# fhgyuanshen/HybridGL

Hardware: AMD Instinct MI355X
Metric: images/sec (whole node) (higher is better)
Workload: dtype f32 via fp16x3 split MFMA (fp32 accumulate)

## Files before the change

### hybridgl_amd/_lib.py

```python
import ctypes as C
import os

_HERE = os.path.dirname(os.path.abspath(__file__))
LIB_PATH = os.path.join(_HERE, "libhybridgl.so")

c_float_p = C.POINTER(C.c_float)
c_u8_p = C.POINTER(C.c_uint8)
c_i32_p = C.POINTER(C.c_int32)
c_i64_p = C.POINTER(C.c_int64)


class HybridGLError(RuntimeError):
    pass


class HglSentence(C.Structure):
    _fields_ = [("sentence_row", C.c_int), ("noun_phrase_row", C.c_int), ("other_row0", C.c_int), ("n_other", C.c_int),
                ("dirflag", C.c_int), ("relaword", C.c_int), ("has_other_nouns", C.c_int), ("black", C.c_float),
                ("imgattn", C.c_void_p), ("target", C.c_void_p)]


class HglGroupRef(C.Structure):
    _fields_ = [("hybrid", C.c_void_p), ("text", C.c_void_p), ("T", C.c_int), ("boxes", C.c_void_p), ("masks", C.c_void_p),
                ("N", C.c_int), ("H", C.c_int), ("W", C.c_int), ("sentences", C.POINTER(HglSentence)), ("S", C.c_int),
# ... 104 lines not shown
    "hgl_clip_text_workspace_bytes": (_SZ, [C.POINTER(HglClipTextW), _I]),
    "hgl_clip_encode_text": (_I, [C.POINTER(HglClipTextW), _VP, _I, _VP, _VP, _SZ, _VP]),
    "hgl_clip_encode_text_prefix": (_I, [C.POINTER(HglClipTextW), _VP, _I, _I, _VP, _VP, _SZ, _VP]),
    "hgl_clip_encode_text_ex": (_I, [C.POINTER(HglClipTextW), _VP, _I, _I, _VP, _VP, _I, _I, _VP, _VP, _SZ, _VP]),
    "hgl_gem_workspace_bytes": (_SZ, [C.POINTER(HglClipVisionW)]),
    "hgl_gem_image_features": (_I, [C.POINTER(HglClipVisionW), _VP, _I, _I, _F, _VP, _VP, _VP, _SZ, _VP]),
    "hgl_gem_batch_workspace_bytes": (_SZ, [C.POINTER(HglClipVisionW), _I]),
    "hgl_gem_image_features_batch": (_I, [C.POINTER(HglClipVisionW), _VP, _I, _I, _I, _F, _VP, _VP, _VP, _SZ, _VP]),
    "hgl_gem_heatmap_workspace_bytes": (_SZ, [_I, _I, _I]),
    "hgl_gem_heatmap": (_I, [_VP, _I, _I, _VP, _I, _I, _I, _VP, _VP, _SZ, _VP]),
    "hgl_resize_bilinear_aa": (_I, [_VP, _I, _I, _I, _VP, _I, _I, _VP]),
    "hgl_resize_bilinear": (_I, [_VP, _I, _I, _I, _VP, _I, _I, _VP]),
    "hgl_mask_resize": (_I, [_VP, _I, _I, _I, _I, _VP, _VP]),
    "hgl_calculate_score": (_I, [_VP, _VP, _I, _I, _I, _F, _VP, _VP]),
    "hgl_coherence_workspace_bytes": (_SZ, [_I, _I, _I]),
    "hgl_coherence_scores": (_I, [_VP, _VP, _I, _I, _I, _I, _F, _VP, _VP, _SZ, _VP]),
    "hgl_iou": (_I, [_VP, _VP, _LL, _VP, _VP]),
    "hgl_iou_select": (_I, [_VP, _VP, _I, _VP, _LL, _VP, _VP]),
    "hgl_score_sentence_workspace_bytes": (_SZ, [_I, _I]),
    "hgl_score_sentence": (_I, [_VP, _VP, _VP, _VP, _I, _F, _VP, _VP, _I, _I, _F, _I, _I, _F, _I, _I,
                                _VP, _VP, _VP, _VP, _SZ, _VP]),
    "hgl_synthesize_views": (_I, [_VP, _VP, _VP, _VP, _I, _I, _I, _I, _VP, _VP, _VP]),
    "hgl_resize_pil_bilinear_workspace_bytes": (_SZ, [_I, _I, _I]),
    "hgl_resize_pil_bilinear": (_I, [_VP, _I, _I, _I, _I, _I, _VP, _VP, _I, _VP, _VP, _I, _VP, _VP, _SZ, _VP]),
    "hgl_sam_encode_workspace_bytes": (_SZ, [C.POINTER(HglSamEncoderW)]),
    "hgl_sam_encode": (_I, [C.POINTER(HglSamEncoderW), _VP, _I, _I, _VP, _VP, _SZ, _VP]),
    "hgl_sam_encode_batch_workspace_bytes": (_SZ, [C.POINTER(HglSamEncoderW), _I]),
    "hgl_sam_encode_batch": (_I, [C.POINTER(HglSamEncoderW), C.POINTER(C.c_void_p), C.POINTER(C.c_int), C.POINTER(C.c_int), _I,
                                  _VP, _VP, _SZ, _VP]),
    "hgl_sam_dense_pe": (_I, [C.POINTER(HglSamDecoderW), _VP, _VP, _VP]),
    "hgl_sam_decode_workspace_bytes": (_SZ, [C.POINTER(HglSamDecoderW), _I]),
    "hgl_sam_decode_points": (_I, [C.POINTER(HglSamDecoderW), _VP, _VP, _I, _VP, _VP, _VP, _SZ, _VP]),
    "hgl_sam_decode_points_gated": (_I, [C.POINTER(HglSamDecoderW), _VP, _VP, _I, C.c_float, _VP, _VP, _VP, _SZ, _VP]),
    "hgl_sam_decode_prompts": (_I, [C.POINTER(HglSamDecoderW), _VP, _VP, _VP, _I, _VP, _I, _I, _VP, _VP, _VP, _SZ, _VP]),
    "hgl_sam_embed_masks": (_I, [C.POINTER(HglSamDecoderW), _VP, _I, _VP, _VP]),
    "hgl_sam_decoder_fusion": (_I, [_I]),
    "hgl_attention_presplit": (_I, [_I]),
    "hgl_attention_presplit_f32": (_I, [_VP, _I, _I, _I, _I, _I, _VP, _I, C.c_float, _I, _VP, _I, _I, _VP, C.c_size_t, _VP]),
    "hgl_sam_postprocess_workspace_bytes": (_SZ, [_I]),
    "hgl_sam_postprocess": (_I, [_VP, _VP, _I, _I, _I, _I, _I, _I, _I, _I, _F, _F, _F, _F, _VP, _VP, _VP, _VP, _VP,
                                 _VP, _SZ, _VP]),
    "hgl_nms": (_I, [_VP, _VP, _VP, _I, _F, _VP, _VP, _VP]),
    "hgl_nms_large_workspace_bytes": (_SZ, [_I]),
    "hgl_nms_large": (_I, [_VP, _VP, _VP, _I, _F, _VP, _VP, _VP, _SZ, _VP]),
    "hgl_box_near_crop_edge": (_I, [_VP, _I, C.POINTER(C.c_int32), C.POINTER(C.c_int32), _F, _VP, _VP]),
    "hgl_remove_small_regions_workspace_bytes": (_SZ, [_I, _I, _I]),
    "hgl_remove_small_regions": (_I, [_VP, _I, _I, _I, _I, _I, _VP, _VP, _VP, _SZ, _VP]),
    "hgl_remove_small_regions_boxes": (_I, [_VP, _I, _I, _I, _I, _I, _VP, _VP, _VP, _VP, _SZ, _VP]),
    "hgl_mask_boxes": (_I, [_VP, _I, _I, _I, _VP, _VP]),
    "hgl_gather_masks": (_I, [_VP, _VP, _VP, _I, _LL, _VP, _VP]),
    "hgl_gen_dir_mask": (_I, [_I, _I, _I, _VP, _VP]),
    "hgl_relation_boxes": (_I, [_VP, _VP, _VP, _VP, _I, _I, _VP, _VP]),
    "hgl_gaussian_blur_u8_workspace_bytes": (_SZ, [_I, _I, _I]),
    "hgl_gaussian_blur_u8": (_I, [_VP, _I, _I, _I, C.POINTER(C.c_double), _I, _VP, _VP, _SZ, _VP]),
    "hgl_cv_gaussian_kernel_q8": (_I, [_I, C.c_double, C.POINTER(C.c_uint16)]),
    "hgl_gaussian_blur_u8_q8": (_I, [_VP, _I, _I, _I, C.POINTER(C.c_uint16), C.POINTER(C.c_uint16), _I, _VP, _VP, _SZ, _VP]),
    "hgl_score_ref_workspace_bytes": (_SZ, [_I, _I, _I, _I, _I]),
    "hgl_score_ref": (_I, [_VP, _VP, _I, _VP, _VP, _I, _I, _I, _I, C.POINTER(HglSentence), _I, C.c_float, C.c_float, _I, _I, C.c_float,
                           _VP, _VP, _VP, _VP, _VP, _VP, _VP, _SZ, _VP]),
    "hgl_score_group_workspace_bytes": (_SZ, [C.POINTER(HglGroupRef), _I, _I]),
    "hgl_score_group": (_I, [C.POINTER(HglGroupRef), _I, _I, C.c_float, C.c_float, C.c_float, _VP, _VP, _SZ, _VP]),
    "hgl_u8_to_chw_lut": (_I, [_VP, _I, _I, _I, _VP, _VP, _VP]),
    "hgl_gt_mask_from_polygons": (_I, [_VP, _VP, _I, _I, _I, _VP, _VP]),
    "hgl_gt_mask_from_rle_counts": (_I, [_VP, _I, _I, _I, _VP, _VP]),
    "hgl_gt_mask_from_rle_string": (_I, [C.c_char_p, _I, _I, _VP, _VP]),
    "hgl_rle_encode_mask": (_I, [_VP, _I, _I, _VP, _LL, C.POINTER(C.c_longlong)]),
    "hgl_rle_to_string": (_I, [_VP, _LL, C.c_char_p, _SZ, C.POINTER(C.c_size_t)]),
}

_lib = None
ABI_VERSION = 7


def load():

# ... 26 lines not shown
```

### hybridgl_amd/csrc/attention.hip

```cpp
#include "hgl_common.h"
#include <stdlib.h>

typedef float f32x2 __attribute__((ext_vector_type(2)));

namespace {

constexpr int KV_CHUNK = 64;
constexpr int NEG_BIG_BITS = 0xff800000;

struct AttnArgs {
  const float *q, *k, *v;
  float* out;
  int B, H, Sq, Sk;
  int ldq, ldk, ldv, ldo;
  long long sqb, skb, svb, sob;
  float scale;
  int mask_kind;
  const uint8_t* keep;
  int keep_b0, keep_n;
  const float *rel_h, *rel_w;
  int kh, kw;
  const float *tab_h, *tab_w;
  const _Float16 *tabh_hi = nullptr, *tabh_lo = nullptr, *tabw_hi = nullptr, *tabw_lo = nullptr;
  _Float16 *out_hi, *out_lo;
// ... 1270 lines not shown
        for (int e = 0; e < 4; ++e) o[c][e] += sc[j] * vv[e];
      }
    }
  }
  const long long oo = b * a.sob + (long long)qi * a.ldo + hh * HD;
#pragma unroll
  for (int c = 0; c < 4; ++c) {
    f32x4 r;
#pragma unroll
    for (int e = 0; e < 4; ++e) r[e] = o[c][e] * inv;
    if (a.out) {
      *(f32x4*)(a.out + oo + 4 * c) = r;
    } else {
      h16x4 hi, lo;
#pragma unroll
      for (int e = 0; e < 4; ++e) {
        _Float16 a2, c2;
        hgl_split_hi_lo(r[e], a2, c2);
        hi[e] = a2;
        lo[e] = c2;
      }
      *(h16x4*)(a.out_hi + oo + 4 * c) = hi;
      if (a.out_lo) *(h16x4*)(a.out_lo + oo + 4 * c) = lo;
    }
  }
}

struct FewQArgs {
  const float *q, *k, *v;
  float* out;
  int B, H, Sq, Sk, ldq, ldk, ldv, ldo;
  long long sqb, skb, svb, sob;
  float scale;
};

constexpr int FEWQ_MAX = 8;

__global__ __launch_bounds__(256) void attn_fewq_kernel(FewQArgs a) {
  constexpr int HD = 16;
  __shared__ __attribute__((aligned(16))) float q_s[FEWQ_MAX * HD];
  __shared__ float part[4][FEWQ_MAX][HD + 2];
  int bh;
  {
    const int bid = blockIdx.x, n = gridDim.x;
    const int per = a.H * 8;
    const int full = (n / per) * per;
    if (bid < full) {
      const int grp = bid / per, r = bid - grp * per;
      const int xcd = r & 7, j = r >> 3;
      bh = (grp * 8 + xcd) * a.H + j;
    } else {
      bh = bid;
    }
  }
  const int b = bh / a.H, hh = bh - b * a.H;
  const int t = threadIdx.x, lane = t & 63, wave = t >> 6;
  if (t < a.Sq * HD) q_s[t] = a.q[b * a.sqb + (long long)(t / HD) * a.ldq + hh * HD + (t % HD)] * a.scale;
  else if (t < FEWQ_MAX * HD) q_s[t] = 0.f;
  __syncthreads();
  float m[FEWQ_MAX], l[FEWQ_MAX];
  f32x4 o[FEWQ_MAX][4];
#pragma unroll
  for (int qi = 0; qi < FEWQ_MAX; ++qi) {
    m[qi] = -3.0e38f; l[qi] = 0.f;
#pragma unroll
    for (int c = 0; c < 4; ++c) o[qi][c] = f32x4{0.f, 0.f, 0.f, 0.f};
// ... 64 lines not shown
      const float sc = expf(part[w2][qi][HD] - mm);
      ll += part[w2][qi][HD + 1] * sc;
      oo += part[w2][qi][d] * sc;
    }
    a.out[b * a.sob + (long long)qi * a.ldo + hh * HD + d] = oo / ll;
  }
}

constexpr int FQC_KEYS = 256;
constexpr int FQC_QS = 7 * 16 + 4;
constexpr int FQC_PART = 10;

__global__ __launch_bounds__(256, 4) void attn_fewq_chunk_kernel(FewQArgs a, float* __restrict__ part) {
  constexpr int NQ = 7;
  __shared__ __attribute__((aligned(16))) float q_s[8 * FQC_QS];
  __shared__ __attribute__((aligned(16))) float mrg[4][16][NQ][FQC_PART + 2];
  const int b = blockIdx.y, chunk = blockIdx.x, nchunk = gridDim.x;
  const int t = threadIdx.x, lane = t & 63, wave = t >> 6;
  const int l16 = t & 15, c2 = t & 1, hh = (t >> 1) & 7, ks = t >> 4;
  constexpr float LOG2E = 1.4426950408889634f;
  for (int i = t; i < 8 * NQ * 16; i += 256) {
    const int head = i / (NQ * 16), rem = i - head * (NQ * 16), qi = rem >> 4, d = rem & 15;
    q_s[head * FQC_QS + rem] = qi < a.Sq ? a.q[b * a.sqb + (long long)qi * a.ldq + head * 16 + d] * (a.scale * LOG2E) : 0.f;
  }
  __syncthreads();
  float m[NQ], l[NQ];
  f32x4 o[NQ][2];
#pragma unroll
  for (int qi = 0; qi < NQ; ++qi) {
    m[qi] = -3.0e38f; l[qi] = 0.f;
    o[qi][0] = f32x4{0.f, 0.f, 0.f, 0.f};
    o[qi][1] = f32x4{0.f, 0.f, 0.f, 0.f};
  }
  const float* kp = a.k + b * a.skb + hh * 16 + c2 * 8;
  const float* vp = a.v + b * a.svb + hh * 16 + c2 * 8;
  const float* qs = q_s + hh * FQC_QS + c2 * 8;
  const int k0 = chunk * FQC_KEYS + ks;
  f32x4 kn[2], vn[2];
  {
    const int key = k0 < a.Sk ? k0 : a.Sk - 1;
    kn[0] = *(const f32x4*)(kp + (long long)key * a.ldk); kn[1] = *(const f32x4*)(kp + (long long)key * a.ldk + 4);
    vn[0] = *(const f32x4*)(vp + (long long)key * a.ldv); vn[1] = *(const f32x4*)(vp + (long long)key * a.ldv + 4);
  }
#pragma unroll 2
  for (int pass = 0; pass < FQC_KEYS / 16; ++pass) {
    const int key = k0 + 16 * pass;
    const f32x4 kk0 = kn[0], kk1 = kn[1], vv0 = vn[0], vv1 = vn[1];
    {
      const int nk = key + 16 < a.Sk ? key + 16 : a.Sk - 1;
      kn[0] = *(const f32x4*)(kp + (long long)nk * a.ldk); kn[1] = *(const f32x4*)(kp + (long long)nk * a.ldk + 4);
      vn[0] = *(const f32x4*)(vp + (long long)nk * a.ldv); vn[1] = *(const f32x4*)(vp + (long long)nk * a.ldv + 4);
    }
    if (key < a.Sk) {
#pragma unroll
      for (int qi = 0; qi < NQ; ++qi) {
        const f32x4 q0 = *(const f32x4*)(qs + qi * 16), q1 = *(const f32x4*)(qs + qi * 16 + 4);
        float s = q0[0] * kk0[0];
        s = fmaf(q0[1], kk0[1], s); s = fmaf(q0[2], kk0[2], s); s = fmaf(q0[3], kk0[3], s);
        s = fmaf(q1[0], kk1[0], s); s = fmaf(q1[1], kk1[1], s); s = fmaf(q1[2], kk1[2], s); s = fmaf(q1[3], kk1[3], s);
        s += __shfl_xor(s, 1);
        const float mn = fmaxf(m[qi], s);
        const float al = __builtin_amdgcn_exp2f(m[qi] - mn), p = __builtin_amdgcn_exp2f(s - mn);
        l[qi] = fmaf(l[qi], al, p);
#pragma unroll
        for (int e = 0; e < 4; ++e) {
          o[qi][0][e] = fmaf(o[qi][0][e], al, p * vv0[e]);
          o[qi][1][e] = fmaf(o[qi][1][e], al, p * vv1[e]);
        }
// ... 148 lines not shown
  a.out_hi = (_Float16*)out_hi; a.out_lo = hgl_split_terms() == 1 ? nullptr : (_Float16*)out_lo;
  HglProfScope prof(HGL_PROF_ATTN, 4.0 * B * H * 196.0 * 196.0 * 80, 0.0, st);
  if (hgl_split_terms() == 1) hipLaunchKernelGGL((attn_x3_kernel<80, 14, 8, 1>), dim3(1, (unsigned)(B * H)), dim3(512), 0, st, a);
  else hipLaunchKernelGGL((attn_x3_kernel<80, 14, 8>), dim3(1, (unsigned)(B * H)), dim3(512), 0, st, a);
  return hgl_check_launch("attention_win14");
}

int hgl_launch_attention_smallk(const float* q, const float* k, const float* v, float* out, void* out_hi, void* out_lo,
                                int B, int H, int Sq, int Sk, int hd, int ldq, int ldk, int ldv, int ldo, long long sqb,
                                long long skb, long long svb, long long sob, float scale, hipStream_t st) {
  HGL_REQUIRE(q && k && v && (out || (out_hi && out_lo)), "attention_smallk: null operand");
  HGL_REQUIRE(hd == 16 && Sk >= 1 && Sk <= SMALLK_MAX && H >= 1 && 256 % H == 0, "attention_smallk: unsupported shape (hd %d, Sk %d, H %d)", hd, Sk, H);
  HGL_REQUIRE(((ldq | ldk | ldv | ldo) & 3) == 0 && ((sqb | skb | svb | sob) & 3) == 0, "attention_smallk: strides must be multiples of 4");
  HGL_REQUIRE(B <= 65535, "attention_smallk: B too large");
  SmallKArgs a;
  a.q = q; a.k = k; a.v = v; a.out = out; a.out_hi = (_Float16*)out_hi;
  a.out_lo = hgl_split_terms() == 1 ? nullptr : (_Float16*)out_lo;
  a.B = B; a.H = H; a.Sq = Sq; a.Sk = Sk; a.ldq = ldq; a.ldk = ldk; a.ldv = ldv; a.ldo = ldo;
  a.sqb = sqb; a.skb = skb; a.svb = svb; a.sob = sob; a.scale = scale;
  const int qpb = 256 / H;
  HglProfScope prof(HGL_PROF_ATTN, 4.0 * B * (double)H * Sq * Sk * hd, 0.0, st);
  hipLaunchKernelGGL(attn_smallk_kernel, dim3((unsigned)((Sq + qpb - 1) / qpb), (unsigned)B), dim3(256),
                     (size_t)2 * Sk * H * 16 * sizeof(float), st, a);
  return hgl_check_launch("attention_smallk");
}

int hgl_launch_attention_fewq(const float* q, const float* k, const float* v, float* out, int B, int H, int Sq, int Sk,
                              int hd, int ldq, int ldk, int ldv, int ldo, long long sqb, long long skb, long long svb,
                              long long sob, float scale, hipStream_t st) {
  HGL_REQUIRE(q && k && v && out, "attention_fewq: null operand");
  HGL_REQUIRE(hd == 16 && Sq >= 1 && Sq <= FEWQ_MAX, "attention_fewq: unsupported shape (hd %d, Sq %d)", hd, Sq);
  HGL_REQUIRE(((ldk | ldv) & 3) == 0 && ((skb | svb) & 3) == 0, "attention_fewq: K/V strides must be multiples of 4");
  FewQArgs a;
  a.q = q; a.k = k; a.v = v; a.out = out; a.B = B; a.H = H; a.Sq = Sq; a.Sk = Sk;
  a.ldq = ldq; a.ldk = ldk; a.ldv = ldv; a.ldo = ldo; a.sqb = sqb; a.skb = skb; a.svb = svb; a.sob = sob; a.scale = scale;
  HglProfScope prof(HGL_PROF_ATTN, 4.0 * B * (double)H * Sq * Sk * hd, 0.0, st);
  hipLaunchKernelGGL(attn_fewq_kernel, dim3((unsigned)(B * H)), dim3(256), 0, st, a);
  return hgl_check_launch("attention_fewq");
}

size_t hgl_attention_fewq_part_bytes(int B, int Sk) {
  return (size_t)B * ((Sk + FQC_KEYS - 1) / FQC_KEYS) * 16 * 7 * FQC_PART * sizeof(float);
}

int hgl_launch_attention_fewq_chunked(const float* q, const float* k, const float* v, float* out, int B, int H, int Sq, int Sk,
                                      int hd, int ldq, int ldk, int ldv, int ldo, long long sqb, long long skb, long long svb,
                                      long long sob, float scale, float* part, size_t part_bytes, hipStream_t st) {
  HGL_REQUIRE(q && k && v && out && part, "attention_fewq_chunked: null operand");
  HGL_REQUIRE(hd == 16 && H == 8 && Sq >= 1 && Sq <= 7 && Sk >= 1 && B >= 1 && B <= 65535,
              "attention_fewq_chunked: unsupported shape (hd %d, H %d, Sq %d)", hd, H, Sq);
  HGL_REQUIRE(((ldk | ldv) & 3) == 0 && ((skb | svb) & 3) == 0 && (((uintptr_t)k | (uintptr_t)v) & 15) == 0,
              "attention_fewq_chunked: K/V strides must be multiples of 4");
  HGL_REQUIRE(part_bytes >= hgl_attention_fewq_part_bytes(B, Sk), "attention_fewq_chunked: partial buffer too small");
  FewQArgs a;
  a.q = q; a.k = k; a.v = v; a.out = out; a.B = B; a.H = H; a.Sq = Sq; a.Sk = Sk;
  a.ldq = ldq; a.ldk = ldk; a.ldv = ldv; a.ldo = ldo; a.sqb = sqb; a.skb = skb; a.svb = svb; a.sob = sob; a.scale = scale;
  const int nchunk = (Sk + FQC_KEYS - 1) / FQC_KEYS;
  HglProfScope prof(HGL_PROF_ATTN, 4.0 * B * (double)H * Sq * Sk * hd, 0.0, st);
  hipLaunchKernelGGL(attn_fewq_chunk_kernel, dim3((unsigned)nchunk, (unsigned)B), dim3(256), 0, st, a, part);
  hipLaunchKernelGGL(attn_fewq_combine_kernel, dim3(7, (unsigned)B), dim3(128), 0, st, (const float*)part, nchunk, Sq, out, ldo, sob);
  return hgl_check_launch("attention_fewq_chunked");
}

int hgl_launch_attention(const float* q, const float* k, const float* v, float* out, int B, int H,
                         int Sq, int Sk, int hd, int ldq, int ldk, int ldv, int ldo, long long sqb,
                         long long skb, long long svb, long long sob, float scale, int mask_kind,
                         const uint8_t* keep, int keep_b0, int keep_n, const float* rel_h,
                         const float* rel_w, int kh, int kw, hipStream_t st) {
  return hgl_launch_attention_split(q, k, v, out, nullptr, nullptr, B, H, Sq, Sk, hd, ldq, ldk, ldv, ldo, sqb, skb, svb, sob,
                                    scale, mask_kind, keep, keep_b0, keep_n, rel_h, rel_w, kh, kw, st);
}

int hgl_launch_attention_split(const float* q, const float* k, const float* v, float* out, void* out_hi, void* out_lo, int B,
                               int H, int Sq, int Sk, int hd, int ldq, int ldk, int ldv, int ldo, long long sqb,
                               long long skb, long long svb, long long sob, float scale, int mask_kind,
                               const uint8_t* keep, int keep_b0, int keep_n, const float* rel_h,
                               const float* rel_w, int kh, int kw, hipStream_t st) {
  HGL_REQUIRE(q && k && v && (out || (out_hi && out_lo)), "attention: null operand");
  HGL_REQUIRE(out || hgl_split_layout(), "attention: split output exists in the split-fp16 modes only");
  HGL_REQUIRE(B > 0 && H > 0 && Sq > 0 && Sk > 0, "attention: bad shape");
  HGL_REQUIRE((ldq & 3) == 0 && (ldk & 3) == 0 && (ldv & 3) == 0 && (ldo & 3) == 0, "attention: leading dims must be multiples of 4");
  HGL_REQUIRE((((uintptr_t)q | (uintptr_t)k | (uintptr_t)v | (uintptr_t)out | (uintptr_t)out_hi | (uintptr_t)out_lo) & 15) == 0,
              "attention: operands must be 16-byte aligned");
  HGL_REQUIRE(((sqb | skb | svb | sob) & 3) == 0, "attention: batch strides must be multiples of 4");
  HGL_REQUIRE(mask_kind >= 0 && mask_kind <= 2, "attention: bad mask kind %d", mask_kind);
  HGL_REQUIRE(mask_kind != HGL_MASK_CLS_KEEP || keep, "attention: HGL_MASK_CLS_KEEP needs keep bytes");
  HGL_REQUIRE((rel_h == nullptr) == (rel_w == nullptr), "attention: rel_h and rel_w go together");
// ... 30 lines not shown
```

### hybridgl_amd/csrc/hgl_common.h

```cpp
#pragma once
#include <hip/hip_runtime.h>
#include <stdint.h>
#include <stddef.h>
#include <atomic>
#include "../../include/hybridgl.h"

typedef float f32x16 __attribute__((ext_vector_type(16)));
typedef float f32x4 __attribute__((ext_vector_type(4)));

#ifdef __HIPCC__
static __device__ __attribute__((unused)) unsigned int hgl_tu_split_overflow;
__device__ __forceinline__ void hgl_split_hi_lo(float x, _Float16& hi, _Float16& lo) {
  asm volatile("" : "+v"(x));
  hi = (_Float16)x;
  lo = (_Float16)(x - (float)hi);
}
__device__ __forceinline__ void hgl_split_hi_lo(float x, _Float16& hi, _Float16& lo, float& amax) {
  asm volatile("" : "+v"(x));
  amax = fmaxf(amax, fabsf(x));
  hi = (_Float16)x;
  lo = (_Float16)(x - (float)hi);
}
__device__ __forceinline__ void hgl_split_commit(float amax) {
  if (__builtin_expect(amax > 65504.0f, 0)) atomicAdd(&hgl_tu_split_overflow, 1u);
// ... 92 lines not shown
    if (dry) return nullptr;
    return (T*)(base + o);
  }
  bool ok() const { return dry || off <= cap; }
};

int hgl_launch_gemm(const float* A, const float* W, const float* bias, const float* R, float* C,
                    int M, int N, int K, int lda, int ldw, int ldr, int ldc, int batch,
                    long long sA, long long sW, long long sR, long long sC, int act,
                    hipStream_t st);
int hgl_launch_layernorm(const float* x, const float* w, const float* b, float* y, int rows, int D,
                         float eps, hipStream_t st);
int hgl_launch_attention_split(const float* q, const float* k, const float* v, float* out, void* out_hi, void* out_lo, int B,
                               int H, int Sq, int Sk, int hd, int ldq, int ldk, int ldv, int ldo, long long sqb,
                               long long skb, long long svb, long long sob, float scale, int mask_kind,
                               const uint8_t* keep, int keep_b0, int keep_n, const float* rel_h,
                               const float* rel_w, int kh, int kw, hipStream_t st);
int hgl_launch_attention_win14(const float* q, const float* k, const float* v, void* out_hi, void* out_lo, int B, int H, int hd,
                               int ldq, int ldk, int ldv, int ldo, long long sqb, long long skb, long long svb, long long sob,
                               float scale, const float* Rh, const float* Rw, hipStream_t st);
bool hgl_attention_ps_enabled();
int hgl_attention_ps_serves(long long plane_delta, int ld, int B, int H, int S, int hd, int mask_kind, int rel_kh, int rel_kw,
                            const float* tab_h, const float* tab_w);
int hgl_launch_attention_ps(const void* qkv_hi, const void* qkv_lo, int ld, int qcol, int kcol, int vcol, long long sb, int B,
                            int H, int S, int hd, float* out, void* out_hi, void* out_lo, int ldo, long long sob, float scale,
                            int mask_kind, const uint8_t* keep, int keep_b0, int keep_n, const float* rel_h, const float* rel_w,
                            int kh, int kw, const float* tab_h, const float* tab_w, hipStream_t st);
int hgl_launch_attention_smallk(const float* q, const float* k, const float* v, float* out, void* out_hi, void* out_lo,
                                int B, int H, int Sq, int Sk, int hd, int ldq, int ldk, int ldv, int ldo, long long sqb,
                                long long skb, long long svb, long long sob, float scale, hipStream_t st);
size_t hgl_attention_fewq_part_bytes(int B, int Sk);
int hgl_launch_attention_fewq_chunked(const float* q, const float* k, const float* v, float* out, int B, int H, int Sq, int Sk,
                                      int hd, int ldq, int ldk, int ldv, int ldo, long long sqb, long long skb, long long svb,
                                      long long sob, float scale, float* part, size_t part_bytes, hipStream_t st);
int hgl_launch_attention(const float* q, const float* k, const float* v, float* out, int B, int H,
                         int Sq, int Sk, int hd, int ldq, int ldk, int ldv, int ldo, long long sqb,
                         long long skb, long long svb, long long sob, float scale, int mask_kind,
                         const uint8_t* keep, int keep_b0, int keep_n, const float* rel_h,
                         const float* rel_w, int kh, int kw, hipStream_t st);

int hgl_launch_im2col_patch(const float* img, int N, int res, int patch, float* cols, hipStream_t st);
int hgl_launch_im2col_patch_split(const float* img, int N, int res, int patch, void* hi, void* lo, hipStream_t st);
int hgl_launch_assemble_lnpre(const float* tok, const float* cls, const float* pos, const float* lw,
                              const float* lb, float* x, int B, int S, int D, hipStream_t st);
int hgl_launch_mask_resize(const uint8_t* masks, int N, int Hm, int Wm, int g, float* pm,
                           uint8_t* keep, hipStream_t st);
int hgl_launch_mix(float* out, const float* a, float ca, const float* b, float cb, const float* pm,
                   int N, int S, int D, hipStream_t st);
int hgl_launch_gather_rows(const float* x, long long row_stride, int rows, int D, float* y,
                           hipStream_t st);
int hgl_launch_add_inplace(float* y, const float* x, long long n, hipStream_t st);
int hgl_launch_text_embed(const int32_t* tokens, const float* emb, const float* pos, float* x, int B,
                          int S, int ctx, int D, int vocab, int32_t* eot, hipStream_t st);
int hgl_launch_gather_eot(const float* x, const int32_t* eot, int B, int S, int D, float* y,
                          hipStream_t st);
int hgl_launch_zero_positions(float* x, int B, int S, int D, const int32_t* pos, int n, hipStream_t st);

struct HglBlockBufs {
  float* H;
  float* QKV;
  float* F;
};
int hgl_clip_run_block(const HglResBlockW& w, float* X, int B, int S, int D, int heads, const HglBlockBufs& bf,
                       int mask_kind, const uint8_t* keep, int keep_b0, int keep_n, hipStream_t st);
bool hgl_clip_block_uses_x3(const HglResBlockW& w, int M, int D);
bool hgl_clip_block_presplit(const HglResBlockW& w, int B, int S, int D, int heads, int mask_kind);
int hgl_clip_block_qkv(const HglResBlockW& w, const float* X, int M, int D, const HglBlockBufs& bf, hipStream_t st,
// ... 29 lines not shown
                            float* tokens, hipStream_t st);
int hgl_launch_mask_downscaling(const float* in, int P, int g, const float* c1w, const float* c1b, const float* n1w, const float* n1b,
                                const float* c2w, const float* c2b, const float* n2w, const float* n2b, const float* c3w,
                                const float* c3b, float* out, hipStream_t st);
int hgl_launch_win_maps(int g, int ws, int nw, int nb, int* pad_of, int* tok_of, int* pad_list, int* pad_count, hipStream_t st);
int hgl_launch_fill_rows(float* dst, int ld, const int* rows, const int* nrows, int max_rows, const float* v, int N,
                         hipStream_t st);
int hgl_launch_fill_rows_split(void* hi, void* lo, int ld, const int* rows, const int* nrows, int max_rows, const float* v,
                               int N, hipStream_t st);
int hgl_launch_ln_gelu64(float* x, const float* w, const float* b, long long rows, float eps, void* hi, void* lo,
                         hipStream_t st);
int hgl_launch_ln256_pe_split(float* x, const float* w, const float* b, const float* pe, int pe_rows, long long rows,
                              float eps, int write_f32, void* kh, void* kl, void* ph, void* pl, hipStream_t st);
int hgl_launch_hyper_logits(const float* u2, const float* hyper, int P, int g, int row0, float* low_res, hipStream_t st);
int hgl_launch_pe_labeled(const float* coords01, const int32_t* labels, const float* G, int n, int F, const float* not_a_point,
                          const float* const* point_embed, float* out, hipStream_t st);
int hgl_launch_t2i_fold_q(const float* q1, const float* Wk, float scale, float* Qk, int P, hipStream_t st);
int hgl_t2i_key_ranges(int P, int HW);
size_t hgl_t2i_part_bytes(int P, int HW);
int hgl_launch_t2i_raw_attn(const void* Qh, const void* Ql, const float* bias, const void* Kh, const void* Kl, int P, int HW,
                            float* out, int ns, hipStream_t st);
int hgl_launch_i2t_prep(const float* k1, const float* v1, const float* Wq, const float* bq, const float* Wo, float scale, void* Kh,
                        void* Kl, float* cb, void* Uh, void* Ul, int P, hipStream_t st);
unsigned long long hgl_split_overflow_decoder(int reset);
int hgl_launch_dec_i2t_fold(const void* Xh, const void* Xl, const void* Kh, const void* Kl, const float* pek, const float* cb,
                            const void* Uh, const void* Ul, const float* bo, const float* ln_w, const float* ln_b, float eps, int P,
                            int HW, void* out_hi, void* out_lo, hipStream_t st);
int hgl_launch_t2i_unfold_v(const float* A, int ns, const float* Wv, const float* bv, float* att, int P, hipStream_t st);
int hgl_launch_dec_tail(const void* src_hi, const void* src_lo, const float* up0_w, const float* up0_b, const float* ln_w,
                        const float* ln_b, const float* up3_w, const float* up3_b, const float* hyper, int row0, int P, int g,
                        float eps, float* low_res, const uint8_t* skip, hipStream_t st);
int hgl_launch_dec_i2t(const float* q, int ldq, long long q_bstride, const float* k1, const float* v1, const float* out_w,
                       const float* out_b, const float* R, long long r_bstride, const float* ln_w, const float* ln_b, float eps,
                       float scale, int P, int HW, float* out32, void* out_hi, void* out_lo, hipStream_t st);

int hgl_precision();
bool hgl_split_layout();
int hgl_split_terms();
struct HglSplitTermsScope {
  explicit HglSplitTermsScope(int terms);
  ~HglSplitTermsScope();
  int prev;
};
bool hgl_has_split_weight(const float* W);
bool hgl_get_split_weight(const float* W, const void** hi, const void** lo, int* scale_log2, int* N, int* K);
int hgl_launch_split_f16(const float* x, float scale, void* hi, void* lo, long long n, hipStream_t st);
int hgl_launch_layernorm_split(const float* x, const float* w, const float* b, void* hi, void* lo, int rows, int D,
                               float eps, hipStream_t st);
int hgl_launch_layernorm_split_maps(const float* x, const float* w, const float* b, void* hi, void* lo, int rows, int D,
                                    float eps, const int* smap, const int* dmap, hipStream_t st);
bool hgl_gemm_skinny_applicable(const float* W32, int M, int N, int K, int lda, int ldw, int batch, int max_m = 1024);
int hgl_launch_gemm_x3_skinny(const float* A, int lda, const float* W32, const float* bias, const float* R, int ldr,
                              float* C, int ldc, int M, int N, int K, int act, hipStream_t st);
int hgl_gemm_f16x3_splitk_factor(int M, int N, int K);
int hgl_launch_gemm_f16x3_splitk(const void* Ah, const void* Al, int lda, const int* amap, const float* W32, const float* bias,
                                 const float* R, int ldr, const int* cmap, float* C, int ldc, int M, int N, int K, int act,
                                 int ksplit, float* part, size_t part_bytes, hipStream_t st);
int hgl_launch_gemm_f16x3_balanced(const void* Ah, const void* Al, int lda, const int* amap, const float* W32, const float* bias,
                                   const float* R, int ldr, const int* cmap, float* C, int ldc, int M, int N, int K, int act,
                                   float* part, size_t part_bytes, hipStream_t st);
int hgl_launch_gemm_f16x3_maps(const void* Ah, const void* Al, int lda, const int* amap, const float* W32, const float* bias,
                               const float* R, int ldr, int rmod, const int* cmap, float* C, void* Ch, void* Cl, int ldc,
                               int M, int N, int K, int act, hipStream_t st);
int hgl_launch_gemm_f16x3_rmod(const void* Ah, const void* Al, int lda, const float* W32, const float* bias, const float* R,
                               int ldr, int rmod, float* C, void* Ch, void* Cl, int ldc, int M, int N, int K, int act, hipStream_t st);
int hgl_launch_gemm_f16x3(const void* Ah, const void* Al, int lda, const float* W32, const float* bias, const float* R,
                          int ldr, float* C, void* Ch, void* Cl, int ldc, int M, int N, int K, int act, hipStream_t st);
// ... 3 lines not shown
```

### hybridgl_amd/csrc/sam_api.hip

```cpp
#include "hgl_common.h"
#include <stdlib.h>
#include <math.h>

namespace {

struct EncPlan {
  float *img, *cols, *X, *H, *Hw, *QKV, *O, *P, *F, *Th, *Tw, *relh, *relw, *neckA, *neckB, *cols3;
  int *pad_of, *tok_of, *pad_list, *pad_count;
  int n_pad_max;
  int nb;
};

bool carve_enc(HglArena& ar, const HglSamEncoderW* w, int nb, EncPlan& p) {
  const int D = w->embed_dim, S = w->img_size, g = S / w->patch, C = w->out_chans;
  const size_t T = (size_t)nb * g * g;
  size_t Tw_max = T;
  int rl_max = 0;
  for (int i = 0; i < w->depth; ++i) {
    const int ws = w->blocks[i].window;
    if (ws > 0) {
      const size_t nw = (g + ws - 1) / ws;
      Tw_max = Tw_max > nb * nw * nw * ws * ws ? Tw_max : nb * nw * nw * ws * ws;
    }
    rl_max = rl_max > w->blocks[i].rel_len ? rl_max : w->blocks[i].rel_len;
// ... 173 lines not shown
    const size_t qkv_bytes = (size_t)M * 3 * D * sizeof(float);
    if (ks > 1 && (size_t)ks * T * D * sizeof(float) <= qkv_bytes) {
      HGL_TRY(hgl_launch_gemm_f16x3_splitk(Fh, Fl, 4 * D, nullptr, b.lin2_w, b.lin2_b, p.X, D, nullptr, p.X, D, T, D, 4 * D,
                                           HGL_ACT_NONE, ks, p.QKV, qkv_bytes, st));
    } else {
      HGL_TRY(hgl_launch_gemm_f16x3_balanced(Fh, Fl, 4 * D, nullptr, b.lin2_w, b.lin2_b, p.X, D, nullptr, p.X, D, T, D, 4 * D, HGL_ACT_NONE,
                                             p.QKV, qkv_bytes, st));
    }
    return HGL_OK;
  }
  if (ws > 0) {
    HGL_TRY(hgl_launch_gemm(p.O, b.proj_w, b.proj_b, nullptr, p.P, M, D, D, D, D, 0, D, 1, 0, 0, 0, 0,
                            HGL_ACT_NONE, st));
    for (int i = 0; i < p.nb; ++i)
      HGL_TRY(hgl_launch_win_unpartition_add(p.X + (size_t)i * T1 * D, g, ws, nw, D, p.P + (size_t)i * M1 * D, st));
  } else {
    HGL_TRY(hgl_launch_gemm(p.O, b.proj_w, b.proj_b, p.X, p.X, T, D, D, D, D, D, D, 1, 0, 0, 0, 0,
                            HGL_ACT_NONE, st));
  }
  HGL_TRY(hgl_launch_layernorm(p.X, b.norm2_w, b.norm2_b, p.H, T, D, 1e-6f, st));
  HGL_TRY(hgl_launch_gemm(p.H, b.lin1_w, b.lin1_b, nullptr, p.F, T, 4 * D, D, D, D, 0, 4 * D, 1, 0, 0, 0, 0,
                          HGL_ACT_GELU, st));
  HGL_TRY(hgl_launch_gemm(p.F, b.lin2_w, b.lin2_b, p.X, p.X, T, D, 4 * D, 4 * D, 4 * D, D, D, 1, 0, 0, 0, 0,
                          HGL_ACT_NONE, st));
  return HGL_OK;
}

struct DecPlan {
  float *coords, *sparse, *tokens, *queries, *qpe, *q1, *k1, *v1, *att, *keys0, *kpe0, *keys, *kpe, *kp, *vp,
      *qi, *atti, *mlp, *u1, *u2, *hy_a, *hy_b, *hyper, *iou_a, *iou_b, *keysS;
  uint8_t* skip;
};

bool carve_dec(HglArena& ar, const HglSamDecoderW* w, int P, DecPlan& p) {
  const size_t C = w->C, HW = (size_t)w->grid * w->grid, T = 16;
  p.sparse = ar.take<float>((size_t)P * (T - 5) * C);
  p.tokens = ar.take<float>(P * T * C);
  p.queries = ar.take<float>(P * T * C);
  p.qpe = ar.take<float>(P * T * C);
  p.q1 = ar.take<float>(P * T * C);
  p.k1 = ar.take<float>(P * T * C);
  p.v1 = ar.take<float>(P * T * C);
  p.att = ar.take<float>(P * T * C);
  p.keys0 = ar.take<float>(HW * C);
  p.kpe0 = ar.take<float>(HW * C);
  p.keys = ar.take<float>(P * HW * C);
  p.kpe = ar.take<float>(P * HW * C);
  p.kp = ar.take<float>(3 * (P * HW * C / 2));
  p.vp = p.kp ? p.kp + P * HW * C / 2 : nullptr;
  p.qi = p.kp ? p.kp + 2 * (P * HW * C / 2) : nullptr;
  p.atti = ar.take<float>(P * HW * C / 2);
  p.mlp = ar.take<float>(P * T * w->mlp_dim);
  p.u1 = ar.take<float>(P * HW * C);
  p.u2 = ar.take<float>(P * HW * 16 * (C / 8));
  p.hy_a = ar.take<float>((size_t)P * C);
  p.hy_b = ar.take<float>((size_t)P * C);
  p.hyper = ar.take<float>((size_t)P * 4 * (C / 8));
  p.keysS = ar.take<float>(P * HW * C);
  p.iou_a = ar.take<float>((size_t)P * C);
  p.iou_b = ar.take<float>((size_t)P * C);
  p.skip = ar.take<uint8_t>((size_t)P);
  return ar.ok();
}

bool valid_lin(const HglLinearW& l) { return l.w && l.b; }
bool valid_attn(const HglSamAttnW& a) {
  return valid_lin(a.q) && valid_lin(a.k) && valid_lin(a.v) && valid_lin(a.out) && a.internal > 0;
}
bool valid_dec(const HglSamDecoderW* w) {
  if (!w || w->C <= 0 || w->grid <= 0 || w->heads <= 0 || w->mlp_dim <= 0 || (w->C & 31)) return false;
  if (!w->pe_gauss || !w->point_embed_pos || !w->not_a_point || !w->no_mask || !w->iou_token || !w->mask_tokens) return false;
  for (int i = 0; i < 2; ++i) {
    const auto& l = w->layer[i];
    if (!valid_attn(l.self_attn) || !valid_attn(l.t2i) || !valid_attn(l.i2t) || !valid_lin(l.lin1) || !valid_lin(l.lin2) ||
        !l.n1.w || !l.n2.w || !l.n3.w || !l.n4.w) return false;
  }
  if (!valid_attn(w->final_t2i) || !w->norm_final.w || !w->up0_w || !w->up0_b || !w->up1.w || !w->up3_w || !w->up3_b) return false;
  for (int i = 0; i < 4; ++i) for (int j = 0; j < 3; ++j) if (!valid_lin(w->hyper[i][j])) return false;
  for (int j = 0; j < 3; ++j) if (!valid_lin(w->iou_head[j])) return false;
  return true;
}

inline int lin(const float* A, int lda, const HglLinearW& l, const float* R, int ldr, float* Cc, int ldc, int M,
               int N, int K, int act, hipStream_t st) {
  if (M > 1024 && hgl_gemm_skinny_applicable(l.w, M, N, K, lda, K, 1, 8192))
    return hgl_launch_gemm_x3_skinny(A, lda, l.w, l.b, R, ldr, Cc, ldc, M, N, K, act, st);
  return hgl_launch_gemm(A, l.w, l.b, R, Cc, M, N, K, lda, K, ldr, ldc, 1, 0, 0, 0, 0, act, st);
}

int g_dec_fusion = -1;
int dec_fusion_mask() {
  if (g_dec_fusion < 0) g_dec_fusion = HGL_DIAG_SWITCH("HGL_SAM_DEC_FUSED", 0x7fffffff);
  return g_dec_fusion;
}

int dec_fewq(const float* q, const float* k, const float* v, float* att, int B, int heads, int Nq, int Nk, int hd, int ldq,
             int ldk, int ldv, int ldo, long long sqb, long long skb, long long svb, long long sob, float* scratch,
             size_t scratch_bytes, hipStream_t st) {
  const float scale = 1.0f / sqrtf((float)hd);
  if ((dec_fusion_mask() & 16) && scratch && heads == 8 && hd == 16 && Nk >= 256 && B <= 65535 &&
      scratch_bytes >= hgl_attention_fewq_part_bytes(B, Nk)) {
    for (int q0 = 0; q0 < Nq; q0 += 7)
      HGL_TRY(hgl_launch_attention_fewq_chunked(q + (long long)q0 * ldq, k, v, att + (long long)q0 * ldo, B, heads,
                                                Nq - q0 < 7 ? Nq - q0 : 7, Nk, hd, ldq, ldk, ldv, ldo, sqb, skb, svb, sob, scale,
                                                scratch, scratch_bytes, st));
    return HGL_OK;
  }
  return hgl_launch_attention(q, k, v, att, B, heads, Nq, Nk, hd, ldq, ldk, ldv, ldo, sqb, skb, svb, sob, scale, HGL_MASK_NONE,
                              nullptr, 0, 0, nullptr, nullptr, 0, 0, st);
}

int dec_attn(const HglSamDecoderW* w, const HglSamAttnW& a, const float* q, bool q_shared, int Nq, const float* k,
             const float* v, bool kv_shared, int Nk, int B, float* qp, float* kp, float* vp, float* att,
             const float* R, long long sR, float* out, hipStream_t st, float* scratch = nullptr, size_t scratch_bytes = 0) {
  const int C = w->C, I = a.internal, heads = w->heads, hd = I / heads;
  const int Bq = q_shared ? 1 : B, Bk = kv_shared ? 1 : B;
  HGL_TRY(lin(q, C, a.q, nullptr, 0, qp, I, Bq * Nq, I, C, HGL_ACT_NONE, st));
  HGL_TRY(lin(k, C, a.k, nullptr, 0, kp, I, Bk * Nk, I, C, HGL_ACT_NONE, st));
  HGL_TRY(lin(v, C, a.v, nullptr, 0, vp, I, Bk * Nk, I, C, HGL_ACT_NONE, st));
  HGL_TRY(dec_fewq(qp, kp, vp, att, B, heads, Nq, Nk, hd, I, I, I, I, q_shared ? 0 : (long long)Nq * I,
                   kv_shared ? 0 : (long long)Nk * I, kv_shared ? 0 : (long long)Nk * I, (long long)Nq * I, scratch,
                   scratch_bytes, st));
  if (!R || sR == (long long)Nq * C)
    return lin(att, I, a.out, R, C, out, C, B * Nq, C, I, HGL_ACT_NONE, st);
  return hgl_launch_gemm(att, a.out.w, a.out.b, R, out, Nq, C, I, I, I, C, C, B, (long long)Nq * I, 0, sR,
                         (long long)Nq * C, HGL_ACT_NONE, st);
}

struct SplitPair { uint16_t *hi, *lo; };
inline SplitPair split_view(float* buf, size_t elems) { return SplitPair{(uint16_t*)buf, (uint16_t*)buf + elems}; }

bool dec_x3_ready(const HglSamDecoderW* w) {
  if (!hgl_split_layout() || w->C != 256) return false;
  const float* need[] = {w->layer[0].i2t.out.w, w->layer[1].i2t.out.w, w->layer[1].i2t.q.w, w->layer[1].t2i.k.w,
                         w->layer[1].t2i.v.w, w->final_t2i.k.w, w->final_t2i.v.w, w->up0_w, w->up3_w};
  for (const float* x : need) if (!hgl_has_split_weight(x)) return false;
  return true;
}

int dec_i2t_x3(const HglSamDecoderW* w, const HglSamAttnW& a, bool shared, const float* kpe0, const SplitPair& kpeS,
               const float* tok_k, const float* tok_v, int P, int HW, int T, float* qi, float* k1, float* v1, float* atti,
               const float* R, int rmod, float* keys_out, hipStream_t st) {
  const int C = w->C, I = a.internal, heads = w->heads, hd = I / heads;
  if (shared) {
    HGL_TRY(lin(kpe0, C, a.q, nullptr, 0, qi, I, HW, I, C, HGL_ACT_NONE, st));
  } else {
    HGL_TRY(hgl_launch_gemm_f16x3(kpeS.hi, kpeS.lo, C, a.q.w, a.q.b, nullptr, 0, qi, nullptr, nullptr, I, P * HW, I, C,
                                  HGL_ACT_NONE, st));
  }
  HGL_TRY(lin(tok_k, C, a.k, nullptr, 0, k1, I, P * T, I, C, HGL_ACT_NONE, st));
  HGL_TRY(lin(tok_v, C, a.v, nullptr, 0, v1, I, P * T, I, C, HGL_ACT_NONE, st));
  const SplitPair at = split_view(atti, (size_t)P * HW * I);
  HGL_TRY(hgl_launch_attention_split(qi, k1, v1, nullptr, at.hi, at.lo, P, heads, HW, T, hd, I, I, I, I,
                                     shared ? 0 : (long long)HW * I, (long long)T * I, (long long)T * I, (long long)HW * I,
                                     1.0f / sqrtf((float)hd), HGL_MASK_NONE, nullptr, 0, 0, nullptr, nullptr, 0, 0, st));
// ... 5 lines not shown
               int P, int HW, int T, float* q1, float* kp, float* vp, float* att, float* queries, float* scratch,
               size_t scratch_bytes, hipStream_t st) {
  const int C = w->C, I = a.internal, heads = w->heads, hd = I / heads;
  HGL_TRY(lin(qpe, C, a.q, nullptr, 0, q1, I, P * T, I, C, HGL_ACT_NONE, st));
  HGL_TRY(hgl_launch_gemm_f16x3(kpeS.hi, kpeS.lo, C, a.k.w, a.k.b, nullptr, 0, kp, nullptr, nullptr, I, P * HW, I, C,
                                HGL_ACT_NONE, st));
  HGL_TRY(hgl_launch_gemm_f16x3(keysS.hi, keysS.lo, C, a.v.w, a.v.b, nullptr, 0, vp, nullptr, nullptr, I, P * HW, I, C,
                                HGL_ACT_NONE, st));
  HGL_TRY(dec_fewq(q1, kp, vp, att, P, heads, T, HW, hd, I, I, I, I, (long long)T * I, (long long)HW * I, (long long)HW * I,
                   (long long)T * I, scratch, scratch_bytes, st));
  return lin(att, I, a.out, queries, C, queries, C, P * T, C, I, HGL_ACT_NONE, st);
}

bool dec_merged_ready(const HglSamDecoderW* w) {
  return (dec_fusion_mask() & 2) && w->kvq1_w && w->kvq1_b && w->kvq1_pe && w->kvf_w && w->kvf_b && w->kvf_pe &&
         hgl_has_split_weight(w->kvq1_w) && hgl_has_split_weight(w->kvf_w);
}

int dec_project_merged(const SplitPair& keysS, const float* W, const float* b, const float* pe_tab, int P, int HW, int C, int N,
                       float* kvq, hipStream_t st) {
  return hgl_launch_gemm_f16x3_rmod(keysS.hi, keysS.lo, C, W, b, pe_tab, N, HW, kvq, nullptr, nullptr, N, P * HW, N, C,
                                    HGL_ACT_NONE, st);
}

int dec_t2i_merged(const HglSamDecoderW* w, const HglSamAttnW& a, const float* qpe, const float* kvq, int ld, int P, int HW,
                   int T, float* q1, float* att, float* queries, float* scratch, size_t scratch_bytes, hipStream_t st) {
  const int C = w->C, I = a.internal, heads = w->heads, hd = I / heads;
  HGL_TRY(lin(qpe, C, a.q, nullptr, 0, q1, I, P * T, I, C, HGL_ACT_NONE, st));
  HGL_TRY(dec_fewq(q1, kvq, kvq + I, att, P, heads, T, HW, hd, I, ld, ld, I, (long long)T * I, (long long)HW * ld,
                   (long long)HW * ld, (long long)T * I, scratch, scratch_bytes, st));
  return lin(att, I, a.out, queries, C, queries, C, P * T, C, I, HGL_ACT_NONE, st);
}

int dec_t2i_raw(const HglSamDecoderW* w, const HglSamAttnW& a, const float* qpe, const SplitPair& keysS, int P, int HW, int T,
                float* q1, float* small, float* bias, float* att, float* queries, hipStream_t st) {
  const int C = w->C, I = a.internal, heads = w->heads, hd = I / heads;
  HGL_TRY(lin(qpe, C, a.q, nullptr, 0, q1, I, P * T, I, C, HGL_ACT_NONE, st));
  uint16_t* Qh = (uint16_t*)small;
  uint16_t* Ql = Qh + (size_t)P * 56 * C;
  float* A = (float*)(Ql + (size_t)P * 56 * C);
  HGL_TRY(hgl_launch_t2i_fold_q(q1, a.k.w, 1.0f / sqrtf((float)hd), A, P, st));
  HGL_TRY(hgl_launch_split_f16(A, 1.0f, Qh, Ql, (long long)P * 56 * C, st));
  HGL_TRY(hgl_launch_gemm_f16x3(Qh, Ql, C, w->dense_pe, nullptr, nullptr, 0, bias, nullptr, nullptr, HW, P * 56, HW, C,
                                HGL_ACT_NONE, st));
  const int ns = hgl_t2i_key_ranges(P, HW);
  float* const rows = ns > 1 ? A + (size_t)P * 56 * C : A;
  HGL_TRY(hgl_launch_t2i_raw_attn(Qh, Ql, bias, keysS.hi, keysS.lo, P, HW, rows, ns, st));
  HGL_TRY(hgl_launch_t2i_unfold_v(rows, ns, a.v.w, a.v.b, att, P, st));
  return lin(att, I, a.out, queries, C, queries, C, P * T, C, I, HGL_ACT_NONE, st);
}

int dec_i2t_merged(const HglSamDecoderW* w, const HglSamAttnW& a, const float* kvq, int ld, const float* tok_k, const float* tok_v,
                   int P, int HW, int T, float* k1, float* v1, float* atti, const float* R, float* keys_out, hipStream_t st) {
  const int C = w->C, I = a.internal, heads = w->heads, hd = I / heads;
  HGL_TRY(lin(tok_k, C, a.k, nullptr, 0, k1, I, P * T, I, C, HGL_ACT_NONE, st));
  HGL_TRY(lin(tok_v, C, a.v, nullptr, 0, v1, I, P * T, I, C, HGL_ACT_NONE, st));
  const SplitPair at = split_view(atti, (size_t)P * HW * I);
  HGL_TRY(hgl_launch_attention_split(kvq + 2 * I, k1, v1, nullptr, at.hi, at.lo, P, heads, HW, T, hd, ld, I, I, I,
                                     (long long)HW * ld, (long long)T * I, (long long)T * I, (long long)HW * I,
                                     1.0f / sqrtf((float)hd), HGL_MASK_NONE, nullptr, 0, 0, nullptr, nullptr, 0, 0, st));
  return hgl_launch_gemm_f16x3_rmod(at.hi, at.lo, I, a.out.w, a.out.b, R, C, 0, keys_out, nullptr, nullptr, C, P * HW, C, I,
                                    HGL_ACT_NONE, st);
}

}

extern "C" {

size_t hgl_sam_encode_batch_workspace_bytes(const HglSamEncoderW* w, int nb) {
  if (!valid_enc(w) || nb < 1) return 0;
  HglArena ar(nullptr, 0);
  EncPlan p;
  carve_enc(ar, w, nb, p);
  return ar.off;
}

size_t hgl_sam_encode_workspace_bytes(const HglSamEncoderW* w) { return hgl_sam_encode_batch_workspace_bytes(w, 1); }

// ... 68 lines not shown
  return hgl_sam_encode_batch(w, &resized_img, &in_h, &in_w, 1, emb, workspace, workspace_bytes, stream);
}

int hgl_sam_dense_pe(const HglSamDecoderW* w, const float* grid_coords01, float* dense_pe, void* stream) {
  HGL_TRY(hgl_require_device());
  HGL_REQUIRE(w && w->pe_gauss && grid_coords01 && dense_pe && w->grid > 0 && w->C > 0, "sam_dense_pe: bad arguments");
  return hgl_launch_pe(grid_coords01, w->pe_gauss, w->grid * w->grid, w->C / 2, 0, nullptr, nullptr, dense_pe,
                       (hipStream_t)stream);
}

size_t hgl_sam_decode_workspace_bytes(const HglSamDecoderW* w, int P) {
  if (!valid_dec(w) || P <= 0) return 0;
  HglArena ar(nullptr, 0);
  DecPlan p;
  carve_dec(ar, w, P, p);
  return ar.off;
}

int hgl_sam_decoder_fusion(int mask) {
  const int old = dec_fusion_mask();
  if (mask >= 0) g_dec_fusion = mask;
  return old;
}

__global__ void iou_gate_kernel(const float* __restrict__ iou, int P, float gate, uint8_t* __restrict__ skip) {
  const int p = blockIdx.x * blockDim.x + threadIdx.x;
  if (p >= P) return;
  skip[p] = (iou[3 * p] > gate || iou[3 * p + 1] > gate || iou[3 * p + 2] > gate) ? 0 : 1;
}

static int decode_impl(const HglSamDecoderW* w, const float* emb, const float* points01, const float* coords01,
                       const int32_t* labels, int n_sparse, const float* dense, int first_mask, int P, float* low_res,
                       float* iou_pred, void* workspace, size_t workspace_bytes, void* stream, bool gated = false,
                       float iou_gate = 0.f) {
  const HglSplitTermsScope three_terms(3);
  HGL_TRY(hgl_require_device());
  HGL_REQUIRE(valid_dec(w) && w->dense_pe, "sam_decode: invalid weight struct (dense_pe missing?)");
  HGL_REQUIRE(emb && (points01 || (coords01 && labels)) && low_res && iou_pred && P > 0, "sam_decode: null input");
  HGL_REQUIRE(first_mask == 0 || first_mask == 1, "sam_decode: first_mask must be 0 or 1");
  HGL_REQUIRE(n_sparse >= 2 && n_sparse <= 11, "sam_decode: %d sparse tokens per prompt (2 .. 11 supported)", n_sparse);
  HGL_REQUIRE(n_sparse <= 3 || (long long)P * w->heads <= 65535, "sam_decode: %d prompts of more than 3 sparse tokens in one call", P);
  HglArena ar(workspace, workspace_bytes);
  DecPlan p;
  if (!workspace || !carve_dec(ar, w, P, p)) {
    hgl_set_error("sam_decode: workspace too small (%zu bytes given)", workspace_bytes);
    return HGL_EWORKSPACE;
  }
  hipStream_t st = (hipStream_t)stream;
  const int C = w->C, g = w->grid, HW = g * g, T = 5 + n_sparse;
  const bool perprompt = dense != nullptr;
  const long long sQ = (long long)T * C, sK = (long long)HW * C;
  const size_t atti_bytes = (size_t)P * HW * (C / 2) * sizeof(float);

  if (points01) {
    HGL_TRY(hgl_launch_pe(points01, w->pe_gauss, 2 * P, C / 2, 1, w->point_embed_pos, w->not_a_point, p.sparse, st));
  } else {
    const float* pe4[4] = {w->point_embed_neg, w->point_embed_pos, w->point_embed_box0, w->point_embed_box1};
    HGL_REQUIRE(pe4[0] && pe4[2] && pe4[3], "sam_decode_prompts: the weight struct lacks point_embeddings 0 / 2 / 3");
    HGL_TRY(hgl_launch_pe_labeled(coords01, labels, w->pe_gauss, n_sparse * P, C / 2, w->not_a_point, pe4, p.sparse, st));
  }
  HGL_TRY(hgl_launch_build_tokens(w->iou_token, w->mask_tokens, p.sparse, P, C, T, p.tokens, st));
  if (perprompt) {
    HGL_TRY(hgl_launch_add_rows_bcast(dense, sK, emb, sK, P, p.keys, st));
    HGL_TRY(hgl_launch_add_rows_bcast(p.keys, sK, w->dense_pe, sK, P, p.kpe, st));
  } else {
    HGL_TRY(hgl_launch_add_rows_bcast(emb, C, w->no_mask, C, HW, p.keys0, st));
    HGL_TRY(hgl_launch_add_rows_bcast(p.keys0, 0, w->dense_pe, (long long)HW * C, 1, p.kpe0, st));
  }
  (void)hipMemcpyAsync(p.queries, p.tokens, sizeof(float) * P * sQ, hipMemcpyDeviceToDevice, st);

  const bool x3 = dec_x3_ready(w);
  const bool merged = x3 && dec_merged_ready(w) && w->layer[1].t2i.internal == w->layer[1].i2t.internal &&
                      w->layer[1].t2i.internal == w->final_t2i.internal && 2 * w->final_t2i.internal == C;
  const int I1 = w->layer[1].t2i.internal;
  const SplitPair keysS = split_view(p.keysS, (size_t)P * HW * C), kpeS = split_view(p.kpe, (size_t)P * HW * C);
  const bool raw_t2i = merged && (dec_fusion_mask() & 32) && (dec_fusion_mask() & 4) && T == 7 && I1 == 128 && w->heads == 8 &&
                       C == 256 && HW % 128 == 0 && P <= 65535 && !perprompt && hgl_has_split_weight(w->dense_pe) &&
                       (size_t)P * (56 * C * 8) + hgl_t2i_part_bytes(P, HW) <= atti_bytes &&
                       (size_t)P * (56 * C * 4 + 16384 * 4 + 256) <= atti_bytes;
  for (int li = 0; li < 2; ++li) {
    const auto& L = w->layer[li];
    const bool shared = li == 0 && !perprompt;
    const bool plain0 = li == 0 && perprompt;
    const float* keys = shared ? p.keys0 : p.keys;
    const float* kpe = shared ? p.kpe0 : p.kpe;
    if (li == 0) {
      HGL_TRY(dec_attn(w, L.self_attn, p.queries, false, T, p.queries, p.queries, false, T, P, p.q1, p.k1, p.v1, p.att,
                       nullptr, 0, p.qpe, st));
      (void)hipMemcpyAsync(p.queries, p.qpe, sizeof(float) * P * sQ, hipMemcpyDeviceToDevice, st);
    } else {
      HGL_TRY(hgl_launch_add_rows_bcast(p.queries, P * sQ, p.tokens, P * sQ, 1, p.qpe, st));
      HGL_TRY(dec_attn(w, L.self_attn, p.qpe, false, T, p.qpe, p.queries, false, T, P, p.q1, p.k1, p.v1, p.att,
                       p.queries, sQ, p.queries, st));
    }
    HGL_TRY(hgl_launch_layernorm(p.queries, L.n1.w, L.n1.b, p.queries, P * T, C, 1e-5f, st));
    HGL_TRY(hgl_launch_add_rows_bcast(p.queries, P * sQ, p.tokens, P * sQ, 1, p.qpe, st));
    if (raw_t2i && !shared && !plain0) {
      HGL_TRY(dec_t2i_raw(w, L.t2i, p.qpe, keysS, P, HW, T, p.q1, p.atti, p.kp, p.att, p.queries, st));
    } else if (merged && !shared && !plain0) {
      HGL_TRY(dec_project_merged(keysS, w->kvq1_w, w->kvq1_b, w->kvq1_pe, P, HW, C, 3 * I1, p.kp, st));
      HGL_TRY(dec_t2i_merged(w, L.t2i, p.qpe, p.kp, 3 * I1, P, HW, T, p.q1, p.att, p.queries, p.atti, atti_bytes, st));
    } else if (x3 && !shared && !plain0) {
      HGL_TRY(dec_t2i_x3(w, L.t2i, p.qpe, kpeS, keysS, P, HW, T, p.q1, p.kp, p.vp, p.att, p.queries, p.atti, atti_bytes, st));
    } else {
      HGL_TRY(dec_attn(w, L.t2i, p.qpe, false, T, kpe, keys, shared, HW, P, p.q1, p.kp, p.vp, p.att, p.queries, sQ,
                       p.queries, st, p.atti, atti_bytes));
    }
    HGL_TRY(hgl_launch_layernorm(p.queries, L.n2.w, L.n2.b, p.queries, P * T, C, 1e-5f, st));
    HGL_TRY(lin(p.queries, C, L.lin1, nullptr, 0, p.mlp, w->mlp_dim, P * T, w->mlp_dim, C, HGL_ACT_RELU, st));
    HGL_TRY(lin(p.mlp, w->mlp_dim, L.lin2, p.queries, C, p.queries, C, P * T, C, w->mlp_dim, HGL_ACT_NONE, st));
    HGL_TRY(hgl_launch_layernorm(p.queries, L.n3.w, L.n3.b, p.queries, P * T, C, 1e-5f, st));
    HGL_TRY(hgl_launch_add_rows_bcast(p.queries, P * sQ, p.tokens, P * sQ, 1, p.qpe, st));
    const bool fuse_i2t = merged && (dec_fusion_mask() & 4) && L.i2t.internal == I1 && I1 == 128 && w->heads == 8 &&
                          HW % 64 == 0 && P <= 65535 && T == 7 && !plain0;
    if (fuse_i2t && raw_t2i && !shared) {
      HGL_TRY(lin(p.qpe, C, L.i2t.k, nullptr, 0, p.k1, I1, P * T, I1, C, HGL_ACT_NONE, st));
      HGL_TRY(lin(p.queries, C, L.i2t.v, nullptr, 0, p.v1, I1, P * T, I1, C, HGL_ACT_NONE, st));
      uint16_t* Kh = (uint16_t*)p.atti;
      uint16_t* Kl = Kh + (size_t)P * 56 * C;
      uint16_t* Uh = Kl + (size_t)P * 56 * C;
      uint16_t* Ul = Uh + (size_t)P * 16384;
      float* cbv = (float*)(Ul + (size_t)P * 16384);
      HGL_TRY(hgl_launch_i2t_prep(p.k1, p.v1, L.i2t.q.w, L.i2t.q.b, L.i2t.out.w, 1.0f / sqrtf((float)(I1 / w->heads)), Kh, Kl, cbv, Uh,
                                  Ul, P, st));
      HGL_TRY(hgl_launch_gemm_f16x3(Kh, Kl, C, w->dense_pe, nullptr, nullptr, 0, p.kp, nullptr, nullptr, HW, P * 56, HW, C,
                                    HGL_ACT_NONE, st));
      HGL_TRY(hgl_launch_dec_i2t_fold(keysS.hi, keysS.lo, Kh, Kl, p.kp, cbv, Uh, Ul, L.i2t.out.b, L.n4.w, L.n4.b, 1e-5f, P, HW,
                                      keysS.hi, keysS.lo, st));
    } else if (fuse_i2t) {
      HGL_TRY(lin(p.qpe, C, L.i2t.k, nullptr, 0, p.k1, I1, P * T, I1, C, HGL_ACT_NONE, st));
      HGL_TRY(lin(p.queries, C, L.i2t.v, nullptr, 0, p.v1, I1, P * T, I1, C, HGL_ACT_NONE, st));
      if (shared) HGL_TRY(lin(p.kpe0, C, L.i2t.q, nullptr, 0, p.qi, I1, HW, I1, C, HGL_ACT_NONE, st));
      HGL_TRY(hgl_launch_dec_i2t(shared ? p.qi : p.kp + 2 * I1, shared ? I1 : 3 * I1, shared ? 0 : (long long)HW * 3 * I1, p.k1,
                                 p.v1, L.i2t.out.w, L.i2t.out.b, keys, shared ? 0 : sK, L.n4.w, L.n4.b, 1e-5f,
                                 1.0f / sqrtf((float)(I1 / w->heads)), P, HW, (li == 0 && !raw_t2i) ? p.keys : nullptr, keysS.hi,
                                 keysS.lo, st));
    } else if (x3 && plain0) {
      HGL_TRY(dec_attn(w, L.i2t, kpe, false, HW, p.qpe, p.queries, false, T, P, p.qi, p.k1, p.v1, p.atti, keys, sK, p.keys, st));
      HGL_TRY(hgl_launch_ln256_pe_split(p.keys, L.n4.w, L.n4.b, w->dense_pe, HW, (long long)P * HW, 1e-5f, 1, keysS.hi, keysS.lo,
                                        merged ? nullptr : kpeS.hi, merged ? nullptr : kpeS.lo, st));
    } else if (x3) {
      if (merged && !shared) {
        HGL_TRY(dec_i2t_merged(w, L.i2t, p.kp, 3 * I1, p.qpe, p.queries, P, HW, T, p.k1, p.v1, p.atti, keys, p.keys, st));
      } else {
        HGL_TRY(dec_i2t_x3(w, L.i2t, shared, p.kpe0, kpeS, p.qpe, p.queries, P, HW, T, p.qi, p.k1, p.v1, p.atti, keys,
                           shared ? HW : 0, p.keys, st));
      }
      HGL_TRY(hgl_launch_ln256_pe_split(p.keys, L.n4.w, L.n4.b, w->dense_pe, HW, (long long)P * HW, 1e-5f, li == 0 ? 1 : 0,
                                        keysS.hi, keysS.lo, merged ? nullptr : kpeS.hi, merged ? nullptr : kpeS.lo, st));
    } else {
      HGL_TRY(dec_attn(w, L.i2t, kpe, shared, HW, p.qpe, p.queries, false, T, P, p.qi, p.k1, p.v1, p.atti, keys,
                       shared ? 0 : sK, p.keys, st));
      HGL_TRY(hgl_launch_layernorm(p.keys, L.n4.w, L.n4.b, p.keys, P * HW, C, 1e-5f, st));
      HGL_TRY(hgl_launch_add_rows_bcast(p.keys, sK, w->dense_pe, sK, P, p.kpe, st));
    }
  }
  HGL_TRY(hgl_launch_add_rows_bcast(p.queries, P * sQ, p.tokens, P * sQ, 1, p.qpe, st));
  if (raw_t2i) {
    HGL_TRY(dec_t2i_raw(w, w->final_t2i, p.qpe, keysS, P, HW, T, p.q1, p.atti, p.kp, p.att, p.queries, st));
  } else if (merged) {
    HGL_TRY(dec_project_merged(keysS, w->kvf_w, w->kvf_b, w->kvf_pe, P, HW, C, 2 * I1, p.kp, st));
    HGL_TRY(dec_t2i_merged(w, w->final_t2i, p.qpe, p.kp, 2 * I1, P, HW, T, p.q1, p.att, p.queries, p.atti, atti_bytes, st));
  } else if (x3) {
    HGL_TRY(dec_t2i_x3(w, w->final_t2i, p.qpe, kpeS, keysS, P, HW, T, p.q1, p.kp, p.vp, p.att, p.queries, p.atti, atti_bytes, st));
  } else {
    HGL_TRY(dec_attn(w, w->final_t2i, p.qpe, false, T, p.kpe, p.keys, false, HW, P, p.q1, p.kp, p.vp, p.att, p.queries,
                     sQ, p.queries, st, p.atti, atti_bytes));
  }
  HGL_TRY(hgl_launch_layernorm(p.queries, w->norm_final.w, w->norm_final.b, p.queries, P * T, C, 1e-5f, st));

  HGL_TRY(lin(p.queries, T * C, w->iou_head[0], nullptr, 0, p.iou_a, C, P, C, C, HGL_ACT_RELU, st));
  HGL_TRY(lin(p.iou_a, C, w->iou_head[1], nullptr, 0, p.iou_b, C, P, C, C, HGL_ACT_RELU, st));
  HGL_TRY(lin(p.iou_b, C, w->iou_head[2], nullptr, 0, p.iou_a, 4, P, 4, C, HGL_ACT_NONE, st));
  HGL_TRY(hgl_launch_gather_rows(p.iou_a + first_mask, 4, P, 3, iou_pred, st));
  const uint8_t* skip = nullptr;
  if (gated) {
    hipLaunchKernelGGL(iou_gate_kernel, dim3((P + 255) / 256), dim3(256), 0, st, (const float*)iou_pred, P, iou_gate, p.skip);
    skip = p.skip;
  }

  const int C4 = C / 4, C8 = C / 8;
  HGL_REQUIRE(C4 == 64, "sam_decode: LayerNorm2d width %d unsupported (64 expected)", C4);
  HGL_REQUIRE(C8 == 32, "sam_decode: hyper-network width %d unsupported (32 expected)", C8);
  for (int i = 0; i < 4; ++i) {
    HGL_TRY(lin(p.queries + (1 + i) * C, T * C, w->hyper[i][0], nullptr, 0, p.hy_a, C, P, C, C, HGL_ACT_RELU, st));
    HGL_TRY(lin(p.hy_a, C, w->hyper[i][1], nullptr, 0, p.hy_b, C, P, C, C, HGL_ACT_RELU, st));
    HGL_TRY(lin(p.hy_b, C, w->hyper[i][2], nullptr, 0, p.hyper + i * C8, 4 * C8, P, C8, C, HGL_ACT_NONE, st));
  }
  const bool fused_tail = x3 && (dec_fusion_mask() & 1) && (HW % 64) == 0 && (g % 64 == 0 || 64 % g == 0) && P <= 65535;
  if (fused_tail) {
    HGL_TRY(hgl_launch_dec_tail(keysS.hi, keysS.lo, w->up0_w, w->up0_b, w->up1.w, w->up1.b, w->up3_w, w->up3_b, p.hyper, first_mask,
                                P, g, 1e-6f, low_res, skip, st));
  } else {
    if (x3) {
      HGL_TRY(hgl_launch_gemm_f16x3(keysS.hi, keysS.lo, C, w->up0_w, w->up0_b, nullptr, 0, p.u1, nullptr, nullptr, 4 * C4,
                                    P * HW, 4 * C4, C, HGL_ACT_NONE, st));
      const SplitPair u1S = split_view(p.kpe, (size_t)P * HW * 4 * C4);
      HGL_TRY(hgl_launch_ln_gelu64(p.u1, w->up1.w, w->up1.b, (long long)P * HW * 4, 1e-6f, u1S.hi, u1S.lo, st));
      HGL_TRY(hgl_launch_gemm_f16x3(u1S.hi, u1S.lo, C4, w->up3_w, w->up3_b, nullptr, 0, p.u2, nullptr, nullptr, 4 * C8,
                                    P * HW * 4, 4 * C8, C4, HGL_ACT_GELU, st));
    } else {
      HGL_TRY(hgl_launch_gemm(p.keys, w->up0_w, w->up0_b, nullptr, p.u1, P * HW, 4 * C4, C, C, C, 0, 4 * C4, 1, 0, 0, 0, 0,
                              HGL_ACT_NONE, st));
      HGL_TRY(hgl_launch_ln_gelu64(p.u1, w->up1.w, w->up1.b, (long long)P * HW * 4, 1e-6f, nullptr, nullptr, st));
      HGL_TRY(hgl_launch_gemm(p.u1, w->up3_w, w->up3_b, nullptr, p.u2, P * HW * 4, 4 * C8, C4, C4, C4, 0, 4 * C8, 1, 0, 0,
                              0, 0, HGL_ACT_GELU, st));
    }
    HGL_TRY(hgl_launch_hyper_logits(p.u2, p.hyper, P, g, first_mask, low_res, st));
  }
  return HGL_OK;
}

int hgl_sam_decode_points(const HglSamDecoderW* w, const float* emb, const float* points01, int P, float* low_res,
                          float* iou_pred, void* workspace, size_t workspace_bytes, void* stream) {
  HGL_REQUIRE(points01, "sam_decode: null input");
  return decode_impl(w, emb, points01, nullptr, nullptr, 2, nullptr, 1, P, low_res, iou_pred, workspace, workspace_bytes, stream);
}

int hgl_sam_decode_points_gated(const HglSamDecoderW* w, const float* emb, const float* points01, int P, float iou_gate,
                                float* low_res, float* iou_pred, void* workspace, size_t workspace_bytes, void* stream) {
  HGL_REQUIRE(points01, "sam_decode: null input");
  return decode_impl(w, emb, points01, nullptr, nullptr, 2, nullptr, 1, P, low_res, iou_pred, workspace, workspace_bytes, stream, true,
                     iou_gate);
}

int hgl_sam_decode_prompts(const HglSamDecoderW* w, const float* emb, const float* coords01, const int32_t* labels, int n_sparse,
                           const float* dense, int first_mask, int P, float* low_res, float* iou_pred, void* workspace,
                           size_t workspace_bytes, void* stream) {
  HGL_REQUIRE(coords01 && labels, "sam_decode_prompts: null input");
  return decode_impl(w, emb, nullptr, coords01, labels, n_sparse, dense, first_mask, P, low_res, iou_pred, workspace,
                     workspace_bytes, stream);
}

int hgl_sam_embed_masks(const HglSamDecoderW* w, const float* mask_input, int P, float* dense, void* stream) {
  HGL_TRY(hgl_require_device());
  HGL_REQUIRE(w && mask_input && dense && P > 0 && P <= 65535, "sam_embed_masks: bad arguments");
  HGL_REQUIRE(w->md_c1_w && w->md_c1_b && w->md_n1_w && w->md_n1_b && w->md_c2_w && w->md_c2_b && w->md_n2_w && w->md_n2_b &&
              w->md_c3_w && w->md_c3_b, "sam_embed_masks: the weight struct lacks mask_downscaling");
  HGL_REQUIRE(w->C == 256, "sam_embed_masks: embedding width %d unsupported", w->C);
  return hgl_launch_mask_downscaling(mask_input, P, w->grid, w->md_c1_w, w->md_c1_b, w->md_n1_w, w->md_n1_b, w->md_c2_w, w->md_c2_b,
                                     w->md_n2_w, w->md_n2_b, w->md_c3_w, w->md_c3_b, dense, (hipStream_t)stream);
}

}
```

### hybridgl_amd/csrc/sam_decoder_fused.hip

```cpp
#include "hgl_common.h"

bool hgl_get_split_weight(const float* W, const void** hi, const void** lo, int* scale_log2, int* N, int* K);

namespace {

typedef _Float16 f16x8 __attribute__((ext_vector_type(8)));
typedef _Float16 f16x4 __attribute__((ext_vector_type(4)));
typedef unsigned u32x4 __attribute__((ext_vector_type(4)));

struct TailArgs {
  const _Float16 *Ah, *Al;
  const _Float16 *W0h, *W0l;
  const _Float16 *W3h, *W3l;
  const float *b0, *ln_w, *ln_b, *b3;
  const float* hyper;
  float s0, s3, eps;
  int g, HW;
  int hrow0;
  float* out;
  const uint8_t* skip;
};

__device__ __forceinline__ unsigned frag_off(int kstep, int nmb, int mb, int r, int chunk) {
  const int sw = (0x78 >> (2 * ((r >> 2) & 3))) & 3;
// ... 233 lines not shown
        const float send = up1 ? k12[ii][m] : k12[2 + ii][m];
        const float keep = up1 ? k12[2 + ii][m] : k12[ii][m];
        const float res = keep + __shfl_xor(send, 16);
        const int i = 2 * (h & 1) + ii;
        const int sub = 2 * pass + (h >> 1);
        const int dy = 2 * (pos >> 1) + (sub >> 1), dx = 2 * (pos & 1) + (sub & 1);
        stage[(m * TAIL_ROWS + 16 * i + r) * 16 + dy * 4 + dx] = res;
      }
  }
  __syncthreads();

  const int g = a.g, S4 = 4 * g;
  const int gw = g < TAIL_ROWS ? g : TAIL_ROWS;
  const int lrow = 31 - __clz(4 * gw);
  const int lnr = 31 - __clz(TAIL_ROWS / gw);
  const int pix0 = tile * TAIL_ROWS, y0 = pix0 / g, x0 = pix0 - y0 * g;
#pragma unroll
  for (int o = t; o < 3 * TAIL_ROWS * 16; o += 512) {
    const int xx = o & ((1 << lrow) - 1);
    int q = o >> lrow;
    const int dy = q & 3;
    q >>= 2;
    const int yl = q & ((1 << lnr) - 1), m = q >> lnr;
    const int xl = xx >> 2, dx = xx & 3;
    const float v = stage[(m * TAIL_ROWS + yl * gw + xl) * 16 + dy * 4 + dx];
    a.out[(((long long)p * 3 + m) * S4 + 4 * (y0 + yl) + dy) * S4 + 4 * (x0 + xl) + dx] = v;
  }
}


struct I2TArgs {
  const float* q;
  long long sqb;
  int ldq;
  const float *k1, *v1;
  const _Float16 *Wh, *Wl;
  const float* bo;
  const float* R;
  long long srb;
  const float *ln_w, *ln_b;
  float so, eps, scale;
  float* out32;
  _Float16 *oh, *ol;
  int HW;
};

constexpr int I2T_ROWS = 64;
constexpr int I2T_TOK = 7;
constexpr int I2T_HS = 20;
constexpr int I2T_A_PLANE = I2T_ROWS * 128 * 2;

__global__ __launch_bounds__(512, 2) void dec_i2t_kernel(I2TArgs a) {
  __shared__ __attribute__((aligned(16))) unsigned char img[2 * I2T_A_PLANE];
  __shared__ __attribute__((aligned(16))) float kv_s[2 * I2T_TOK * 8 * I2T_HS];
  __shared__ __attribute__((aligned(16))) float red[2][I2T_ROWS][8];
  const int t = threadIdx.x, lane = t & 63, wave = t >> 6;
  const int r = lane & 15, h = lane >> 4;
  const int p = blockIdx.y, tile = blockIdx.x;
  const int n0 = tile * I2T_ROWS;
  const long long row0 = (long long)p * a.HW + n0;

  const _Float16* const wh = a.Wh + (long long)(wave * 32 + r) * 128 + 8 * h;
  const _Float16* const wl = a.Wl + (long long)(wave * 32 + r) * 128 + 8 * h;
  f16x8 bh[2][2], bl[2][2];
#pragma unroll
  for (int pre = 0; pre < 2; ++pre)
#pragma unroll
    for (int j = 0; j < 2; ++j) {
      bh[pre][j] = *(const f16x8*)(wh + j * 16 * 128 + pre * 32);
      bl[pre][j] = *(const f16x8*)(wl + j * 16 * 128 + pre * 32);
    }

  if (t < I2T_TOK * 32) {
    const int j = t >> 5, c = t & 31;
    const int dst = (j * 8 + (c >> 2)) * I2T_HS + 4 * (c & 3);
    *(f32x4*)(kv_s + dst) = ((const f32x4*)(a.k1 + (long long)p * I2T_TOK * 128))[t];
    *(f32x4*)(kv_s + I2T_TOK * 8 * I2T_HS + dst) = ((const f32x4*)(a.v1 + (long long)p * I2T_TOK * 128))[t];
  }
  const int hh = t & 7, arow = t >> 3;
  f32x4 qv[4];
  {
    const float* qp = a.q + p * a.sqb + (long long)(n0 + arow) * a.ldq + hh * 16;
#pragma unroll
    for (int c = 0; c < 4; ++c) qv[c] = *(const f32x4*)(qp + 4 * c);
  }
  __syncthreads();

  {
    float sc[I2T_TOK];
    float mx = -3.0e38f;
#pragma unroll
    for (int j = 0; j < I2T_TOK; ++j) {
      const float* kr = kv_s + (j * 8 + hh) * I2T_HS;
      float d = 0.f;
#pragma unroll
      for (int c = 0; c < 4; ++c) {
        const f32x4 kk = *(const f32x4*)(kr + 4 * c);
        d += qv[c][0] * kk[0]; d += qv[c][1] * kk[1]; d += qv[c][2] * kk[2]; d += qv[c][3] * kk[3];
      }
      sc[j] = d * a.scale;
      mx = fmaxf(mx, sc[j]);
    }
    float l = 0.f;
#pragma unroll
    for (int j = 0; j < I2T_TOK; ++j) {
      sc[j] = expf(sc[j] - mx);
      l += sc[j];
    }
    const float inv = 1.0f / l;
    f32x4 o[4];
#pragma unroll
    for (int c = 0; c < 4; ++c) o[c] = f32x4{0.f, 0.f, 0.f, 0.f};
#pragma unroll
    for (int j = 0; j < I2T_TOK; ++j) {
      const float* vr = kv_s + I2T_TOK * 8 * I2T_HS + (j * 8 + hh) * I2T_HS;
// ... 34 lines not shown
#pragma unroll
    for (int i = 0; i < 4; ++i) {
      const unsigned off = frag_off(ks, 4, i, r, h);
      ah[i] = *(const f16x8*)(img + off);
      al[i] = *(const f16x8*)(img + I2T_A_PLANE + off);
    }
#pragma unroll
    for (int term = 0; term < 3; ++term)
#pragma unroll
      for (int i = 0; i < 4; ++i)
#pragma unroll
        for (int j = 0; j < 2; ++j) {
          const f16x8 av = term == 0 ? al[i] : ah[i];
          const f16x8 bv = term == 1 ? bl[cb][j] : bh[cb][j];
          acc[i][j] = __builtin_amdgcn_mfma_f32_16x16x32_f16(bv, av, acc[i][j], 0, 0, 0);
        }
    if (ks + 2 < 4) {
#pragma unroll
      for (int j = 0; j < 2; ++j) {
        bh[cb][j] = *(const f16x8*)(wh + j * 16 * 128 + (ks + 2) * 32);
        bl[cb][j] = *(const f16x8*)(wl + j * 16 * 128 + (ks + 2) * 32);
      }
    }
  }

  const int colw = wave * 32 + 4 * h;
  f32x4 bov[2], lw[2], lb[2];
#pragma unroll
  for (int j = 0; j < 2; ++j) {
    bov[j] = *(const f32x4*)(a.bo + colw + 16 * j);
    lw[j] = *(const f32x4*)(a.ln_w + colw + 16 * j);
    lb[j] = *(const f32x4*)(a.ln_b + colw + 16 * j);
  }
  const float* Rp = a.R + p * a.srb + (long long)n0 * 256 + colw;
#pragma unroll
  for (int i = 0; i < 4; ++i)
#pragma unroll
    for (int j = 0; j < 2; ++j) {
      const f32x4 rv = *(const f32x4*)(Rp + (long long)(16 * i + r) * 256 + 16 * j);
#pragma unroll
      for (int e = 0; e < 4; ++e) acc[i][j][e] = (acc[i][j][e] * a.so + bov[j][e]) + rv[e];
    }
  auto row_sum = [&](const f32x4 (&x)[2]) {
    float u = ((x[0][0] + x[0][1]) + (x[0][2] + x[0][3])) + ((x[1][0] + x[1][1]) + (x[1][2] + x[1][3]));
    u += __shfl_xor(u, 16);
    u += __shfl_xor(u, 32);
    return u;
  };
  auto tile_sum = [&](const float* s8) {
    const f32x4 s = *(const f32x4*)s8, u = *(const f32x4*)(s8 + 4);
    return ((s[0] + s[1]) + (s[2] + s[3])) + ((u[0] + u[1]) + (u[2] + u[3]));
  };
#pragma unroll
  for (int i = 0; i < 4; ++i) {
    const float u = row_sum(acc[i]);
    if (h == 0) red[0][16 * i + r][wave] = u;
  }
  __syncthreads();
  float mean[4], rstd[4];
#pragma unroll
  for (int i = 0; i < 4; ++i) {
    mean[i] = tile_sum(red[0][16 * i + r]) * (1.f / 256.f);
    f32x4 q[2];
#pragma unroll
    for (int j = 0; j < 2; ++j)
#pragma unroll
      for (int e = 0; e < 4; ++e) { const float d = acc[i][j][e] - mean[i]; q[j][e] = d * d; }
// ... 39 lines not shown
        *(f32x4*)(a.out32 + ob + row * 256 + c4 * 4) = *(const f32x4*)(st32 + row * 256 + ((c4 ^ row) * 4));
      }
    }
  }
}

}

int hgl_launch_dec_tail(const void* src_hi, const void* src_lo, const float* up0_w, const float* up0_b, const float* ln_w,
                        const float* ln_b, const float* up3_w, const float* up3_b, const float* hyper, int row0, int P, int g,
                        float eps, float* low_res, const uint8_t* skip, hipStream_t st) {
  const void *w0h, *w0l, *w3h, *w3l;
  int s0 = 0, s3 = 0, n0 = 0, k0 = 0, n3 = 0, k3 = 0;
  const int HW = g * g;
  HGL_REQUIRE(hgl_get_split_weight(up0_w, &w0h, &w0l, &s0, &n0, &k0) && hgl_get_split_weight(up3_w, &w3h, &w3l, &s3, &n3, &k3),
              "dec_tail: the upscaling weights have no registered fp16 split");
  HGL_REQUIRE(n0 == 256 && k0 == 256 && n3 == 128 && k3 == 64, "dec_tail: upscaling geometry [%d,%d] / [%d,%d] unsupported", n0, k0, n3, k3);
  HGL_REQUIRE(HW % TAIL_ROWS == 0 && (g % TAIL_ROWS == 0 || TAIL_ROWS % g == 0) && P > 0 && P <= 65535,
              "dec_tail: grid %d / %d prompts unsupported", g, P);
  TailArgs a;
  a.Ah = (const _Float16*)src_hi; a.Al = (const _Float16*)src_lo;
  a.W0h = (const _Float16*)w0h; a.W0l = (const _Float16*)w0l; a.W3h = (const _Float16*)w3h; a.W3l = (const _Float16*)w3l;
  a.b0 = up0_b; a.ln_w = ln_w; a.ln_b = ln_b; a.b3 = up3_b; a.hyper = hyper;
  a.s0 = ldexpf(1.0f, -s0); a.s3 = ldexpf(1.0f, -s3); a.eps = eps;
  a.g = g; a.HW = HW; a.hrow0 = row0; a.out = low_res; a.skip = skip;
  HGL_RESERVE_LDS((dec_tail_kernel), TAIL_LDS, "dec_tail");
  HglProfScope prof(HGL_PROF_OTHER, 2.0 * P * HW * (256.0 * 256 + 4 * 64.0 * 128), 0.0, st);
  hipLaunchKernelGGL(dec_tail_kernel, dim3((unsigned)(HW / TAIL_ROWS), (unsigned)P), dim3(512), TAIL_LDS, st, a);
  return hgl_check_launch("dec_tail");
}

int hgl_launch_dec_i2t(const float* q, int ldq, long long q_bstride, const float* k1, const float* v1, const float* out_w,
                       const float* out_b, const float* R, long long r_bstride, const float* ln_w, const float* ln_b, float eps,
                       float scale, int P, int HW, float* out32, void* out_hi, void* out_lo, hipStream_t st) {
  const void *wh, *wl;
  int s = 0, n = 0, k = 0;
  HGL_REQUIRE(hgl_get_split_weight(out_w, &wh, &wl, &s, &n, &k), "dec_i2t: the out-projection weight has no registered fp16 split");
  HGL_REQUIRE(n == 256 && k == 128, "dec_i2t: out-projection geometry [%d,%d] unsupported", n, k);
  HGL_REQUIRE(q && k1 && v1 && R && out_hi && out_lo, "dec_i2t: null operand");
  HGL_REQUIRE(HW % I2T_ROWS == 0 && P > 0 && P <= 65535 && (ldq & 3) == 0 && (q_bstride & 3) == 0 && (r_bstride & 3) == 0,
              "dec_i2t: %d tokens / %d prompts / strides unsupported", HW, P);
  I2TArgs a;
  a.q = q; a.sqb = q_bstride; a.ldq = ldq; a.k1 = k1; a.v1 = v1;
  a.Wh = (const _Float16*)wh; a.Wl = (const _Float16*)wl; a.bo = out_b; a.R = R; a.srb = r_bstride;
  a.ln_w = ln_w; a.ln_b = ln_b; a.so = ldexpf(1.0f, -s); a.eps = eps; a.scale = scale;
  a.out32 = out32; a.oh = (_Float16*)out_hi; a.ol = (_Float16*)out_lo; a.HW = HW;
  HglProfScope prof(HGL_PROF_OTHER, 2.0 * P * HW * (128.0 * 256 + 2 * 7 * 128), 0.0, st);
  hipLaunchKernelGGL(dec_i2t_kernel, dim3((unsigned)(HW / I2T_ROWS), (unsigned)P), dim3(512), 0, st, a);
  return hgl_check_launch("dec_i2t");
}
```

### hybridgl_amd/csrc/sam_glue.hip

```cpp
#include "hgl_common.h"
#include <math.h>

typedef float f32x2 __attribute__((ext_vector_type(2)));
typedef _Float16 f16x4g __attribute__((ext_vector_type(4)));
typedef unsigned u32x4g __attribute__((ext_vector_type(4)));

namespace {

inline unsigned grid1(long long n, int block = 256) { return (unsigned)((n + block - 1) / block); }

__global__ __launch_bounds__(256) void sam_preprocess_kernel(const uint8_t* __restrict__ img, int h, int w,
                                                             int S, float* __restrict__ out) {
  const long long i = blockIdx.x * 256ll + threadIdx.x;
  if (i >= 3ll * S * S) return;
  const int x = (int)(i % S), y = (int)((i / S) % S), c = (int)(i / ((long long)S * S));
  const float mean[3] = {123.675f, 116.28f, 103.53f};
  const float stdv[3] = {58.395f, 57.12f, 57.375f};
  float v = 0.f;
  if (y < h && x < w) v = ((float)img[((long long)y * w + x) * 3 + c] - mean[c]) / stdv[c];
  out[i] = v;
}

__global__ __launch_bounds__(256) void pil_resample_kernel(const uint8_t* __restrict__ in, uint8_t* __restrict__ out,
                                                           const int* __restrict__ kk, const int* __restrict__ bounds,
// ... 932 lines not shown
  return true;
}

__global__ void init_counters_kernel(unsigned* c, int K) {
  const int k = blockIdx.x * blockDim.x + threadIdx.x;
  if (k >= K) return;
  c[k * 6 + 0] = 0; c[k * 6 + 1] = 0;
  c[k * 6 + 2] = 0x7fffffff; c[k * 6 + 3] = 0x7fffffff;
  c[k * 6 + 4] = 0; c[k * 6 + 5] = 0;
}

__global__ void sam_finalize_kernel(const unsigned* __restrict__ c, const float* __restrict__ iou, int K,
                                    float iou_thresh, float stab_thresh, float* __restrict__ stab,
                                    int* __restrict__ boxes, uint8_t* __restrict__ keep) {
  const int k = blockIdx.x * blockDim.x + threadIdx.x;
  if (k >= K) return;
  const bool pass_iou = !iou || !(iou_thresh > 0.f) || iou[k] > iou_thresh;
  const float s = (float)c[k * 6 + 0] / (float)c[k * 6 + 1];
  stab[k] = pass_iou ? s : 0.f;
  const bool empty = c[k * 6 + 2] == 0x7fffffff;
  boxes[k * 4 + 0] = empty ? 0 : (int)c[k * 6 + 2];
  boxes[k * 4 + 1] = empty ? 0 : (int)c[k * 6 + 3];
  boxes[k * 4 + 2] = empty ? 0 : (int)c[k * 6 + 4];
  boxes[k * 4 + 3] = empty ? 0 : (int)c[k * 6 + 5];
  keep[k] = (pass_iou && (!(stab_thresh > 0.f) || s >= stab_thresh)) ? 1 : 0;
}

__device__ __forceinline__ bool nms_before(float sj, int j, float si, int i) {
  const bool nj = sj != sj, ni = si != si;
  if (nj || ni) return nj && (!ni || j < i);
  return sj > si || (sj == si && j < i);
}

__global__ __launch_bounds__(1024) void nms_kernel(const int* __restrict__ boxes,
                                                   const float* __restrict__ scores,
                                                   const uint8_t* __restrict__ keep, int K, float thr,
                                                   int* __restrict__ out_idx, int* __restrict__ out_n) {
  __shared__ int order[1024];
  __shared__ unsigned char alive[1024];
  __shared__ int cur, nkept;
  const int t = threadIdx.x;
  int valid = 0;
  float sc = 0.f;
  if (t < K && keep[t]) { valid = 1; sc = scores[t]; }
  if (t < 1024) order[t] = -1;
  __syncthreads();
  if (valid) {
    int rank = 0;
    for (int j = 0; j < K; ++j) {
      if (!keep[j]) continue;
      const float sj = scores[j];
      if (nms_before(sj, j, sc, t)) ++rank;
    }
    order[rank] = t;
  }
  if (t < 1024) alive[t] = 1;
  if (t == 0) nkept = 0;
  __syncthreads();
  int nvalid = 0;
  for (int j = 0; j < K; ++j) nvalid += keep[j] ? 1 : 0;
  for (int r = 0; r < nvalid; ++r) {
    if (t == 0) cur = alive[r] ? order[r] : -1;
    __syncthreads();
    const int ci = cur;
    if (ci >= 0) {
      if (t == 0) { out_idx[nkept] = ci; ++nkept; }
      const int me = (t > r && t < nvalid) ? order[t] : -1;
      if (me >= 0 && alive[t]) {
        const float ax0 = boxes[ci * 4], ay0 = boxes[ci * 4 + 1], ax1 = boxes[ci * 4 + 2], ay1 = boxes[ci * 4 + 3];
        const float bx0 = boxes[me * 4], by0 = boxes[me * 4 + 1], bx1 = boxes[me * 4 + 2], by1 = boxes[me * 4 + 3];
        const float iw = fmaxf(fminf(ax1, bx1) - fmaxf(ax0, bx0), 0.f);
        const float ih = fmaxf(fminf(ay1, by1) - fmaxf(ay0, by0), 0.f);
        const float inter = iw * ih;
        const float iou = inter / ((ax1 - ax0) * (ay1 - ay0) + (bx1 - bx0) * (by1 - by0) - inter);
        if (iou > thr) alive[t] = 0;
      }
    }
    __syncthreads();
  }
  if (t == 0) *out_n = nkept;
}

__global__ __launch_bounds__(256) void nms_rank_kernel(const float* __restrict__ scores, const uint8_t* __restrict__ keep,
                                                       int K, int* __restrict__ order, int* __restrict__ nvalid) {
  const int i = blockIdx.x * 256 + threadIdx.x;
  if (i >= K || !keep[i]) return;
  const float sc = scores[i];
  int rank = 0;
  for (int j = 0; j < K; ++j) {
    if (!keep[j]) continue;
    const float sj = scores[j];
    rank += nms_before(sj, j, sc, i) ? 1 : 0;
  }
  order[rank] = i;
  atomicAdd(nvalid, 1);
}

__device__ __forceinline__ bool nms_overlap(const int4 a, const int4 b, float thr) {
  const float ax0 = (float)a.x, ay0 = (float)a.y, ax1 = (float)a.z, ay1 = (float)a.w;
  const float bx0 = (float)b.x, by0 = (float)b.y, bx1 = (float)b.z, by1 = (float)b.w;
  const float iw = fmaxf(fminf(ax1, bx1) - fmaxf(ax0, bx0), 0.f);
  const float ih = fmaxf(fminf(ay1, by1) - fmaxf(ay0, by0), 0.f);
  const float inter = iw * ih;
  const float iou = inter / ((ax1 - ax0) * (ay1 - ay0) + (bx1 - bx0) * (by1 - by0) - inter);
  return iou > thr;
}

__global__ __launch_bounds__(512) void nms_bits_kernel(const int* __restrict__ boxes, const float* __restrict__ scores,
                                                       const uint8_t* __restrict__ keep, int K, float thr,
                                                       int* __restrict__ out_idx, int* __restrict__ out_n) {
  __shared__ int4 sbox[512];
  __shared__ int order[512];
  __shared__ float ssc[512];
  __shared__ unsigned char skeep[512];
  __shared__ unsigned long long mask[512][8];
  __shared__ unsigned long long removed[8];
  __shared__ unsigned long long kept_word;
  __shared__ int nv, nkept_s;
  const int t = threadIdx.x, lane = t & 63;
  const bool valid = t < K && keep[t];
  const float sc = valid ? scores[t] : 0.f;
  ssc[t] = sc;
  skeep[t] = valid ? 1 : 0;
  order[t] = -1;
  if (t < 8) removed[t] = 0;
  if (t == 0) { nv = 0; nkept_s = 0; }
  __syncthreads();
  if (valid) {
    int rank = 0;
#pragma unroll 8
    for (int j = 0; j < K; ++j) {
      const float sj = ssc[j];
      rank += (skeep[j] && nms_before(sj, j, sc, t)) ? 1 : 0;
    }
    order[rank] = t;
    atomicAdd(&nv, 1);
  }
  __syncthreads();
  const int n = nv;
  if (t < n) sbox[t] = ((const int4*)boxes)[order[t]];
  __syncthreads();
  const int nw = (n + 63) >> 6;
  for (int w = 0, q0 = 0; w < nw; ++w) {
// ... 12 lines not shown
  }
  __syncthreads();
  for (int rb = 0; rb < nw; ++rb) {
    if (t < 64) {
      const int a = rb * 64 + lane;
      const unsigned long long d = a < n ? mask[a][rb] : 0ull;
      unsigned long long rem = removed[rb], km = 0;
      for (int s2 = 0; s2 < 64; ++s2) {
        const unsigned lo = __shfl((unsigned)(d & 0xffffffffull), s2), hi = __shfl((unsigned)(d >> 32), s2);
        if (rb * 64 + s2 < n && !((rem >> s2) & 1ull)) {
          km |= 1ull << s2;
          rem |= ((unsigned long long)hi << 32) | lo;
        }
      }
      const int base = nkept_s;
      if ((km >> lane) & 1ull) out_idx[base + __popcll(km & ((1ull << lane) - 1ull))] = order[a];
      if (lane == 0) { kept_word = km; nkept_s = base + __popcll(km); }
    }
    __syncthreads();
    const unsigned long long km = kept_word;
    if (t > rb && t < nw) {
      unsigned long long acc = removed[t];
      unsigned long long bits = km;
      while (bits) {
        const int s2 = __ffsll((long long)bits) - 1;
        bits &= bits - 1;
        acc |= mask[rb * 64 + s2][t];
      }
      removed[t] = acc;
    }
    __syncthreads();
  }
  if (t == 0) *out_n = nkept_s;
}

__global__ __launch_bounds__(64) void nms_mask_kernel(const int* __restrict__ boxes, const int* __restrict__ order,
                                                      const int* __restrict__ nvalid, int W, float thr,
                                                      unsigned long long* __restrict__ mask) {
  const int cb = blockIdx.x, rb = blockIdx.y, t = threadIdx.x;
  const int n = *nvalid;
  if (cb < rb || rb * 64 >= n) return;
  __shared__ int4 colbox[64];
  const int b = cb * 64 + t;
  colbox[t] = b < n ? ((const int4*)boxes)[order[b]] : make_int4(0, 0, 0, 0);
  __syncthreads();
  const int a = rb * 64 + t;
  unsigned long long w = 0;
  if (a < n) {
    const int4 me = ((const int4*)boxes)[order[a]];
    const int jmax = min(64, n - cb * 64);
    for (int j = 0; j < jmax; ++j) {
      if (cb * 64 + j > a && nms_overlap(me, colbox[j], thr)) w |= 1ull << j;
    }
  }
  mask[(long long)a * W + cb] = w;
}

__global__ __launch_bounds__(256) void nms_scan_kernel(const unsigned long long* __restrict__ mask,
                                                       const int* __restrict__ order, const int* __restrict__ nvalid,
                                                       int W, int* __restrict__ out_idx, int* __restrict__ out_n) {
  __shared__ unsigned long long removed[1024];
  __shared__ unsigned long long kept_word;
  __shared__ int nkept_s;
  const int t = threadIdx.x, lane = t & 63;
  const int n = *nvalid;
  for (int w = t; w < W; w += 256) removed[w] = 0;
// ... 260 lines not shown
  }
  hipStream_t st = (hipStream_t)stream;
  unsigned* counters = (unsigned*)workspace;
  hipLaunchKernelGGL(init_counters_kernel, dim3((K + 255) / 256), dim3(256), 0, st, counters, K);
  PostArgs a;
  a.low = low_res; a.iou = iou_pred; a.iou_thresh = pred_iou_thresh;
  a.K = K; a.hl = hl; a.wl = wl; a.S = img_size; a.hi = in_h; a.wi = in_w; a.H = H; a.W = W;
  a.thr = mask_threshold; a.off = stability_offset;
  a.masks = masks; a.counters = counters; a.full_logits = full_logits;
  const char* sep_env = hgl_env_str("HGL_SAM_POST_SEP");
  const bool sep_on = !(sep_env && sep_env[0] == '0');
  const dim3 grid((W + PTW - 1) / PTW, (H + PTH - 1) / PTH, K);
  if (sep_on && postprocess_sep_fits(W, in_w, wl, img_size) && postprocess_sep_fits(H, in_h, hl, img_size))
    hipLaunchKernelGGL(sam_postprocess_sep_kernel, grid, dim3(256), 0, st, a);
  else
    hipLaunchKernelGGL(sam_postprocess_kernel, grid, dim3(256), 0, st, a);
  hipLaunchKernelGGL(sam_finalize_kernel, dim3((K + 255) / 256), dim3(256), 0, st, counters, iou_pred, K,
                     pred_iou_thresh, stability_thresh, stability, (int*)boxes_xyxy, keep);
  return hgl_check_launch("sam_postprocess");
}

int hgl_nms(const int32_t* boxes_xyxy, const float* scores, const uint8_t* keep, int K, float iou_threshold,
            int32_t* out_idx, int32_t* out_n, void* stream) {
  HGL_TRY(hgl_require_device());
  HGL_REQUIRE(boxes_xyxy && scores && keep && out_idx && out_n, "nms: null argument");
  HGL_REQUIRE(K > 0 && K <= 1024, "nms: K must be in [1,1024] (got %d)", K);
  if (K <= 512 && ((uintptr_t)boxes_xyxy & 15) == 0)
    hipLaunchKernelGGL(nms_bits_kernel, dim3(1), dim3(512), 0, (hipStream_t)stream, (const int*)boxes_xyxy, scores, keep, K, iou_threshold, (int*)out_idx, (int*)out_n);
  else
    hipLaunchKernelGGL(nms_kernel, dim3(1), dim3(1024), 0, (hipStream_t)stream, (const int*)boxes_xyxy, scores, keep, K, iou_threshold, (int*)out_idx, (int*)out_n);
  return hgl_check_launch("nms");
}

size_t hgl_nms_large_workspace_bytes(int K) {
  const size_t W = ((size_t)K + 63) / 64;
  return hgl_align_up((size_t)K * sizeof(int), 256) + hgl_align_up(sizeof(int), 256) + hgl_align_up((size_t)K * W * 8, 256);
}

int hgl_nms_large(const int32_t* boxes_xyxy, const float* scores, const uint8_t* keep, int K, float iou_threshold,
                  int32_t* out_idx, int32_t* out_n, void* workspace, size_t workspace_bytes, void* stream) {
  HGL_TRY(hgl_require_device());
  HGL_REQUIRE(boxes_xyxy && scores && keep && out_idx && out_n, "nms_large: null argument");
  HGL_REQUIRE(K > 0 && K <= 32768, "nms_large: K must be in [1,32768] (got %d)", K);
  HGL_REQUIRE(((uintptr_t)boxes_xyxy & 15) == 0, "nms_large: boxes must be 16-byte aligned");
  if (!workspace || workspace_bytes < hgl_nms_large_workspace_bytes(K)) {
    hgl_set_error("nms_large: workspace too small");
    return HGL_EWORKSPACE;
  }
  hipStream_t st = (hipStream_t)stream;
  const int W = (K + 63) / 64;
  HglArena ar(workspace, workspace_bytes);
  int* order = ar.take<int>((size_t)K);
  int* nvalid = ar.take<int>(1);
  unsigned long long* mask = ar.take<unsigned long long>((size_t)K * W);
  if (hipMemsetAsync(nvalid, 0, sizeof(int), st) != hipSuccess) {
    hgl_set_error("nms_large: memset failed");
    return HGL_ELAUNCH;
  }
  hipLaunchKernelGGL(nms_rank_kernel, dim3((K + 255) / 256), dim3(256), 0, st, scores, keep, K, order, nvalid);
  hipLaunchKernelGGL(nms_mask_kernel, dim3(W, W), dim3(64), 0, st, (const int*)boxes_xyxy, order, nvalid, W, iou_threshold, mask);
  hipLaunchKernelGGL(nms_scan_kernel, dim3(1), dim3(256), 0, st, mask, order, nvalid, W, (int*)out_idx, (int*)out_n);
  return hgl_check_launch("nms_large");
}

int hgl_box_near_crop_edge(const int32_t* boxes_xyxy, int K, const int32_t* crop_box_xyxy, const int32_t* orig_box_xyxy,
                           float atol, uint8_t* keep, void* stream) {
// ... 18 lines not shown
```

### hybridgl_amd/sam.py

```python
import ctypes as C
import os

import numpy as np
import torch

from . import _lib, ops, weights
from ._lib import check


from ._lib import (HglLinearW, HglNormW, HglSamAttnW, HglSamBlockW, HglSamDecoderW,
                   HglSamEncoderW)


def _dev(a, device):
    if isinstance(a, torch.Tensor):
        t = a.detach().to(torch.float32)
    else:
        t = torch.from_numpy(np.ascontiguousarray(a, dtype=np.float32))
    return t.contiguous().to(device)


def load_sam_state_dict(path):
    sd = torch.load(path, map_location="cpu")
    return {k: v.float().numpy() for k, v in sd.items()}
# ... 179 lines not shown
        nb = len(resized_list)
        imgs = [r.contiguous() for r in resized_list]
        ptrs = (C.c_void_p * nb)(*[ops._dev(r, torch.uint8, "resized_img") for r in imgs])
        hs = (C.c_int * nb)(*[int(r.shape[0]) for r in imgs])
        wsz = (C.c_int * nb)(*[int(r.shape[1]) for r in imgs])
        need = lib.hgl_sam_encode_batch_workspace_bytes(C.byref(self.enc_w), nb)
        ws = ops.workspace(need, self.device, "sam_encode")
        emb = torch.empty((nb, self.grid * self.grid, self.cfg["out_chans"]), dtype=torch.float32, device=self.device)
        check(lib.hgl_sam_encode_batch(C.byref(self.enc_w), ptrs, hs, wsz, nb, emb.data_ptr(), ws.data_ptr(), ws.numel(),
                                       ops._stream()), "hgl_sam_encode_batch")
        return emb

    def decode_points(self, emb, points01, iou_gate=None):
        lib = _lib.load()
        ops.use_precision(self.precision)
        P = points01.shape[0]
        need = lib.hgl_sam_decode_workspace_bytes(C.byref(self.dec_w), P)
        ws = ops.workspace(need, self.device, "sam_decode")
        g4 = 4 * self.grid
        low = torch.empty((P, 3, g4, g4), dtype=torch.float32, device=self.device)
        iou = torch.empty((P, 3), dtype=torch.float32, device=self.device)
        if iou_gate is not None:
            check(lib.hgl_sam_decode_points_gated(C.byref(self.dec_w), ops._dev(emb, torch.float32, "emb"),
                                                  ops._dev(points01, torch.float32, "points01"), P, float(iou_gate), low.data_ptr(),
                                                  iou.data_ptr(), ws.data_ptr(), ws.numel(), ops._stream()),
                  "hgl_sam_decode_points_gated")
            return low, iou
        check(lib.hgl_sam_decode_points(C.byref(self.dec_w), ops._dev(emb, torch.float32, "emb"),
                                        ops._dev(points01, torch.float32, "points01"), P, low.data_ptr(),
                                        iou.data_ptr(), ws.data_ptr(), ws.numel(), ops._stream()),
              "hgl_sam_decode_points")
        return low, iou

    def decode_prompts(self, emb, coords01, labels, first_mask=1, dense=None):
        lib = _lib.load()
        ops.use_precision(self.precision)
        P, n = int(coords01.shape[0]), int(coords01.shape[1])
        need = lib.hgl_sam_decode_workspace_bytes(C.byref(self.dec_w), P)
        ws = ops.workspace(need, self.device, "sam_decode")
        g4 = 4 * self.grid
        low = torch.empty((P, 3, g4, g4), dtype=torch.float32, device=self.device)
        iou = torch.empty((P, 3), dtype=torch.float32, device=self.device)
        check(lib.hgl_sam_decode_prompts(C.byref(self.dec_w), ops._dev(emb, torch.float32, "emb"),
                                         ops._dev(coords01, torch.float32, "coords01"), ops._dev(labels, torch.int32, "labels"), n,
                                         None if dense is None else ops._dev(dense, torch.float32, "dense"),
                                         int(first_mask), P, low.data_ptr(), iou.data_ptr(), ws.data_ptr(), ws.numel(),
                                         ops._stream()), "hgl_sam_decode_prompts")
        return low, iou

    def embed_masks(self, mask_input):
        lib = _lib.load()
        P = int(mask_input.shape[0])
        g4 = 4 * self.grid
        if tuple(mask_input.shape) != (P, 1, g4, g4):
            raise ValueError(f"mask_input must be [P,1,{g4},{g4}], got {tuple(mask_input.shape)}")
        dense = torch.empty((P, self.grid * self.grid, self.dec_w.C), dtype=torch.float32, device=self.device)
        check(lib.hgl_sam_embed_masks(C.byref(self.dec_w), ops._dev(mask_input, torch.float32, "mask_input"), P, dense.data_ptr(),
                                      ops._stream()), "hgl_sam_embed_masks")
        return dense

    def postprocess(self, low_res, iou_pred, input_size, original_size, pred_iou_thresh=-1e30,
                    stability_thresh=0.0, stability_offset=1.0, return_logits=False):
        lib = _lib.load()
        K, hl, wl = low_res.shape
        H, W = original_size
        dev = self.device
        masks = torch.empty((K, H, W), dtype=torch.uint8, device=dev)
        boxes = torch.empty((K, 4), dtype=torch.int32, device=dev)
        stab = torch.empty((K,), dtype=torch.float32, device=dev)
        keep = torch.empty((K,), dtype=torch.uint8, device=dev)
        full = torch.empty((K, H, W), dtype=torch.float32, device=dev) if return_logits else None
        need = lib.hgl_sam_postprocess_workspace_bytes(K)
        ws = ops.workspace(need, dev, "sam_post")
        check(lib.hgl_sam_postprocess(ops._dev(low_res, torch.float32, "low_res"),
                                      ops._dev(iou_pred, torch.float32, "iou_pred"), K, hl, wl, self.img_size,
                                      int(input_size[0]), int(input_size[1]), H, W, float(self.mask_threshold),
                                      float(stability_offset), float(pred_iou_thresh), float(stability_thresh),
                                      masks.data_ptr(), boxes.data_ptr(), stab.data_ptr(), keep.data_ptr(),
                                      full.data_ptr() if full is not None else None, ws.data_ptr(), ws.numel(),
                                      ops._stream()), "hgl_sam_postprocess")
        return masks, boxes, stab, keep, full


def nms(boxes_xyxy, scores, keep, iou_threshold):
    lib = _lib.load()
    K = boxes_xyxy.shape[0]
    idx = torch.empty((K,), dtype=torch.int32, device=boxes_xyxy.device)
    n = torch.empty((1,), dtype=torch.int32, device=boxes_xyxy.device)
    if K <= 1024:
        check(lib.hgl_nms(ops._dev(boxes_xyxy, torch.int32, "boxes"), ops._dev(scores, torch.float32, "scores"),
                          ops._dev(keep, torch.uint8, "keep"), K, float(iou_threshold), idx.data_ptr(), n.data_ptr(),
                          ops._stream()), "hgl_nms")
    else:
        need = lib.hgl_nms_large_workspace_bytes(K)
        ws = ops.workspace(need, boxes_xyxy.device, "nms_large")
        check(lib.hgl_nms_large(ops._dev(boxes_xyxy, torch.int32, "boxes"), ops._dev(scores, torch.float32, "scores"),
                                ops._dev(keep, torch.uint8, "keep"), K, float(iou_threshold), idx.data_ptr(),
                                n.data_ptr(), ws.data_ptr(), ws.numel(), ops._stream()), "hgl_nms_large")
    return idx, n


def nms_large(boxes_xyxy, scores, keep, iou_threshold):
    lib = _lib.load()
    K = boxes_xyxy.shape[0]
    idx = torch.empty((K,), dtype=torch.int32, device=boxes_xyxy.device)
    n = torch.empty((1,), dtype=torch.int32, device=boxes_xyxy.device)
    ws = ops.workspace(lib.hgl_nms_large_workspace_bytes(K), boxes_xyxy.device, "nms_large")
    check(lib.hgl_nms_large(ops._dev(boxes_xyxy, torch.int32, "boxes"), ops._dev(scores, torch.float32, "scores"),
                            ops._dev(keep, torch.uint8, "keep"), K, float(iou_threshold), idx.data_ptr(), n.data_ptr(),
                            ws.data_ptr(), ws.numel(), ops._stream()), "hgl_nms_large")
    return idx, n


def box_near_crop_edge(boxes_xyxy, keep, crop_box, orig_box, atol=20.0):
    import ctypes as C
    lib = _lib.load()
    cb = (C.c_int32 * 4)(*[int(v) for v in crop_box])
    ob = (C.c_int32 * 4)(*[int(v) for v in orig_box])
    check(lib.hgl_box_near_crop_edge(ops._dev(boxes_xyxy, torch.int32, "boxes"), boxes_xyxy.shape[0], cb, ob, float(atol),
                                     ops._dev(keep, torch.uint8, "keep"), ops._stream()), "hgl_box_near_crop_edge")
    return keep


def _build(cfg_name, checkpoint=None, state_dict=None, seed=0, device="cuda", precision=None):
    checkpoint = checkpoint or os.environ.get("HYBRIDGL_SAM_CHECKPOINT")
    if state_dict is None and checkpoint:
        state_dict = load_sam_state_dict(checkpoint)
    if state_dict is None:
        state_dict = weights.sam_state_dict(cfg_name, seed)
    return Sam(state_dict, weights.SAM_CONFIGS[cfg_name], device, precision)

# ... 222 lines not shown
                 point_grids=None, min_mask_region_area=0, output_mode="binary_mask"):
        assert (points_per_side is None) != (point_grids is None), \
            "Exactly one of points_per_side or point_grid must be provided."
        assert output_mode in ["binary_mask", "uncompressed_rle", "coco_rle"], f"Unknown output_mode {output_mode}."
        self.output_mode = output_mode
        self.model = model
        self.predictor = SamPredictor(model)
        if point_grids is None:
            self.point_grids = build_all_layer_point_grids(points_per_side, crop_n_layers, crop_n_points_downscale_factor)
        else:
            self.point_grids = point_grids
        assert len(self.point_grids) >= crop_n_layers + 1, "one point grid per crop layer"
        self.crop_n_layers = crop_n_layers
        self.crop_overlap_ratio = crop_overlap_ratio
        self.points_per_batch = points_per_batch
        self.pred_iou_thresh = pred_iou_thresh
        self.stability_score_thresh = stability_score_thresh
        self.stability_score_offset = stability_score_offset
        self.box_nms_thresh = box_nms_thresh
        self.crop_nms_thresh = crop_nms_thresh
        self.min_mask_region_area = min_mask_region_area

    def propose(self, image, resized=None, layer_idx=0, crop_box=None, orig_size=None):
        m = self.model
        H, W = image.shape[:2]
        nh, nw = get_preprocess_shape(H, W, m.img_size)
        if resized is None:
            dev_img = image if isinstance(image, torch.Tensor) else torch.from_numpy(np.ascontiguousarray(image)).to(m.device)
            resized = resize_longest_side(dev_img.contiguous(), m.img_size)
        emb = m.encode(resized)
        return self._propose_from_embedding(emb, H, W, nh, nw, layer_idx, crop_box, orig_size)

    def propose_batch(self, images, encoded_event=None):
        m = self.model
        sizes, resized = [], []
        for image in images:
            H, W = image.shape[:2]
            dev_img = image if isinstance(image, torch.Tensor) else torch.from_numpy(np.ascontiguousarray(image)).to(m.device)
            sizes.append((H, W) + get_preprocess_shape(H, W, m.img_size))
            resized.append(resize_longest_side(dev_img.contiguous(), m.img_size))
        emb = m.encode_batch(resized)
        if encoded_event is not None:
            encoded_event.record(torch.cuda.current_stream(m.device))
        return [self._propose_from_embedding(emb[i], *sizes[i], 0, None, None) for i in range(len(images))]

    def _propose_from_embedding(self, emb, H, W, nh, nw, layer_idx, crop_box, orig_size):
        m = self.model
        pts = self.point_grids[layer_idx] * np.array([[W, H]], dtype=np.float64)
        tp = pts.copy()
        tp[:, 0] *= nw / W
        tp[:, 1] *= nh / H
        key = (H, W, layer_idx)
        cache = self.__dict__.setdefault("_p01_cache", {})
        p01 = cache.get(key)
        if p01 is None:
            if len(cache) >= 64:
                cache.clear()
            p01 = cache[key] = torch.from_numpy(((tp + 0.5) / float(m.img_size)).astype(np.float32)).to(m.device)
        lows, ious = [], []
        gate = float(self.pred_iou_thresh) if self.pred_iou_thresh > 0 and getattr(self, "iou_gate", True) else None
        for s in range(0, len(pts), self.points_per_batch):
            low, iou = m.decode_points(emb, p01[s:s + self.points_per_batch].contiguous(), iou_gate=gate)
            lows.append(low.flatten(0, 1))
            ious.append(iou.flatten())
        low = lows[0] if len(lows) == 1 else torch.cat(lows)
        iou = ious[0] if len(ious) == 1 else torch.cat(ious)
        masks, boxes, stab, keep, _ = m.postprocess(low, iou, (nh, nw), (H, W), self.pred_iou_thresh,
                                                    self.stability_score_thresh, self.stability_score_offset)
        if crop_box is not None and orig_size is not None and list(crop_box) != [0, 0, orig_size[1], orig_size[0]]:
            box_near_crop_edge(boxes, keep, crop_box, [0, 0, orig_size[1], orig_size[0]])
        order, n = nms(boxes, iou, keep, self.box_nms_thresh)
        return masks, boxes, iou, stab, order, n, np.repeat(pts, 3, axis=0)

    def generate_device_crops(self, image):
        m = self.model
        dev_img = image if isinstance(image, torch.Tensor) else torch.from_numpy(np.ascontiguousarray(image)).to(m.device)
        H, W = dev_img.shape[:2]
        crop_boxes, layer_idxs = generate_crop_boxes((H, W), self.crop_n_layers, self.crop_overlap_ratio)
        all_m, all_b, all_iou, all_stab, all_pts, all_cb = [], [], [], [], [], []
        embs = []
        for c0 in range(0, len(crop_boxes), 8):
            res = [resize_longest_side(dev_img[y0:y1, x0:x1, :].contiguous(), m.img_size) for x0, y0, x1, y1 in crop_boxes[c0:c0 + 8]]
            e = m.encode_batch(res) if len(res) > 1 else [m.encode(res[0])]
            embs.extend(e[i] for i in range(len(res)))
        for ci, (crop_box, layer_idx) in enumerate(zip(crop_boxes, layer_idxs)):
            x0, y0, x1, y1 = crop_box
            ch, cw = y1 - y0, x1 - x0
            masks, boxes, iou, stab, order, n, pts = self._propose_from_embedding(embs[ci], ch, cw, *get_preprocess_shape(ch, cw, m.img_size),
                                                                                   layer_idx, crop_box, (H, W))
            n = int(n.item())
            if n == 0:
# ... 178 lines not shown
        return out

    def generate_crops_group(self, images):
        return self.crops_finish(self.crops_post(self.crops_mid(self.crops_begin(images))))

    def generate_device(self, image, resized=None, fixed_n=None):
        masks, boxes, iou, stab, order, n, points = self.propose(image, resized)
        if fixed_n is not None:
            idx = order[:fixed_n].long()
            m = masks.index_select(0, idx).contiguous()
            m, nb = self.cleanup_fixed(m)
            return m, nb, iou.index_select(0, idx), stab.index_select(0, idx), idx
        n = int(n.item())
        idx = order[:n].long()
        m = masks.index_select(0, idx).contiguous()
        bx = boxes.index_select(0, idx).contiguous()
        if self.min_mask_region_area > 0 and n > 0:
            m1, c1 = remove_small_regions(m, self.min_mask_region_area, "holes")
            m2, c2, nb = remove_small_regions_boxes(m1, self.min_mask_region_area, "islands")
            unchanged = ((c1 | c2) == 0).to(torch.float32)
            keep_all = torch.ones(n, dtype=torch.uint8, device=m.device)
            order2, n2 = nms(nb, unchanged, keep_all, max(self.box_nms_thresh, self.crop_nms_thresh))
            k = order2[: int(n2.item())].long()
            m, bx, idx = m2.index_select(0, k), nb.index_select(0, k), idx.index_select(0, k)
        b = bx.long()
        xywh = torch.stack([b[:, 0], b[:, 1], b[:, 2] - b[:, 0], b[:, 3] - b[:, 1]], 1) if n > 0 else b
        return m, xywh, iou.index_select(0, idx), stab.index_select(0, idx), idx

    def group_begin(self, images, cap=None, encoded_event=None):
        assert self.crop_n_layers == 0, "crop layers take generate_device_crops (one crop at a time)"
        st = _GroupState()
        st.cap = cap
        st.sizes = [tuple(int(v) for v in im.shape[:2]) for im in images]
        st.cand = self.propose_batch(images, encoded_event)
        dev = self.model.device
        st.n1_dev = torch.cat([c[5] for c in st.cand])
        st.n1 = torch.empty(len(images), dtype=torch.int32).pin_memory()
        st.n1.copy_(st.n1_dev, non_blocking=True)
        st.overflow = 0
        st.ovf = torch.zeros(2, dtype=torch.int32).pin_memory()
        ops.split_overflow_peek(st.ovf)
        st.ev1 = torch.cuda.Event()
        st.ev1.record(torch.cuda.current_stream(dev))
        return st

    def group_cleanup(self, st):
        st.ev1.synchronize()
        if st.ovf is not None:
            st.overflow = int(st.ovf[0]) + int(st.ovf[1])
        dev = self.model.device
        n1 = [int(v) for v in st.n1.tolist()]
        if st.cap is not None:
            n1 = [min(v, st.cap) for v in n1]
        st.n1_list = n1
        st.stage = []
        n2_dev = []
        for (masks, boxes, iou, stab, order, _n, _pts), n in zip(st.cand, n1):
            if n == 0:
                st.stage.append(None)
                n2_dev.append(torch.zeros(1, dtype=torch.int32, device=dev))
                continue
            idx = order[:n].long()
            m = masks.index_select(0, idx)
            bx = boxes.index_select(0, idx)
            if self.min_mask_region_area > 0:
                m1, c1 = remove_small_regions(m, self.min_mask_region_area, "holes")
                m2, c2, nb = remove_small_regions_boxes(m1, self.min_mask_region_area, "islands")
                unchanged = ((c1 | c2) == 0).to(torch.float32)
                order2, n2 = nms(nb, unchanged, torch.ones(n, dtype=torch.uint8, device=dev),
                                 max(self.box_nms_thresh, self.crop_nms_thresh))
                st.stage.append((m2, nb, idx, order2, iou, stab))
                n2_dev.append(n2)
            else:
                st.stage.append((m, bx, idx, None, iou, stab))
                n2_dev.append(torch.full((1,), n, dtype=torch.int32, device=dev))
        st.cand = None
        st.n2 = None
        if self.min_mask_region_area > 0:
            st.n2 = torch.empty(len(n1), dtype=torch.int32).pin_memory()
            st.n2.copy_(torch.cat(n2_dev), non_blocking=True)
            st.ev2 = torch.cuda.Event()
            st.ev2.record(torch.cuda.current_stream(dev))
        return st

    def group_finish(self, st):
        if st.n2 is not None:
            st.ev2.synchronize()
            n2 = [int(v) for v in st.n2.tolist()]
        else:
            n2 = list(st.n1_list)
        out = []
        dev = self.model.device
        for stg, n, hw in zip(st.stage, n2, st.sizes):
            if stg is None or n == 0:
                e = torch.empty
                out.append((e((0,) + hw, dtype=torch.uint8, device=dev), e((0, 4), dtype=torch.int64, device=dev),
                            e((0,), device=dev), e((0,), device=dev), e((0,), dtype=torch.int64, device=dev)))
                continue
            m, bx, idx, order2, iou, stab = stg
            if order2 is not None:
                k = order2[:n].long()
                m, bx, idx = m.index_select(0, k), bx.index_select(0, k), idx.index_select(0, k)
            b = bx.long()
            xywh = torch.stack([b[:, 0], b[:, 1], b[:, 2] - b[:, 0], b[:, 3] - b[:, 1]], 1)
            out.append((m, xywh, iou.index_select(0, idx), stab.index_select(0, idx), idx))
        st.stage = None
        return out

    def generate_group(self, images, cap=None):
        return self.group_finish(self.group_cleanup(self.group_begin(images, cap)))

    def cleanup_fixed(self, m):
        if self.min_mask_region_area <= 0:
            return m, mask_boxes(m)
        m1, c1 = remove_small_regions(m, self.min_mask_region_area, "holes")
        m2, c2, nb = remove_small_regions_boxes(m1, self.min_mask_region_area, "islands")
        nms(nb, ((c1 | c2) == 0).to(torch.float32), torch.ones(m.shape[0], dtype=torch.uint8, device=m.device),
            max(self.box_nms_thresh, self.crop_nms_thresh))
        return m2, nb

    def _segmentation(self, mask):
        if self.output_mode == "binary_mask":
            return mask
        rle = mask_to_rle(mask)
        return coco_encode_rle(rle) if self.output_mode == "coco_rle" else rle

    def generate(self, image):
        if self.crop_n_layers > 0:
            m, xywh, iou, stab, pts, cbs = self.generate_device_crops(image)
            masks = m.bool().cpu().numpy()
            xywh, iou, stab = xywh.cpu().numpy(), iou.cpu().numpy(), stab.cpu().numpy()
            out = []
            for i in range(len(masks)):
                cb = cbs[i]
                out.append({"segmentation": self._segmentation(masks[i]), "area": int(masks[i].sum()), "bbox": [int(v) for v in xywh[i]],
                            "predicted_iou": float(iou[i]), "point_coords": [pts[i].tolist()],
                            "stability_score": float(stab[i]),
                            "crop_box": [int(cb[0]), int(cb[1]), int(cb[2] - cb[0]), int(cb[3] - cb[1])]})
            return out
        m, xywh, iou, stab, idx = self.generate_device(image)
# ... 14 lines not shown
    lib = _lib.load()
    mk = np.ascontiguousarray(np.asarray(mask).astype(np.uint8))
    H, W = mk.shape
    m = C.c_longlong(0)
    check(lib.hgl_rle_encode_mask(mk.ctypes.data, H, W, None, 0, C.byref(m)), "hgl_rle_encode_mask")
    counts = np.empty(m.value, dtype=np.uint32)
    check(lib.hgl_rle_encode_mask(mk.ctypes.data, H, W, counts.ctypes.data, m.value, C.byref(m)), "hgl_rle_encode_mask")
    return {"size": [H, W], "counts": [int(v) for v in counts]}


def rle_to_mask(rle):
    lib = _lib.load()
    h, w = rle["size"]
    counts = np.ascontiguousarray(np.asarray(rle["counts"], dtype=np.uint32))
    out = np.empty((h, w), dtype=np.uint8)
    check(lib.hgl_gt_mask_from_rle_counts(counts.ctypes.data, len(counts), h, w, out.ctypes.data, None), "hgl_gt_mask_from_rle_counts")
    return out.astype(bool)


def area_from_rle(rle):
    return sum(rle["counts"][1::2])


def coco_encode_rle(uncompressed_rle):
    lib = _lib.load()
    h, w = uncompressed_rle["size"]
    counts = np.ascontiguousarray(np.asarray(uncompressed_rle["counts"], dtype=np.uint32))
    buf = C.create_string_buffer(7 * len(counts) + 1)
    n = C.c_size_t(0)
    check(lib.hgl_rle_to_string(counts.ctypes.data, len(counts), buf, len(buf), C.byref(n)), "hgl_rle_to_string")
    return {"size": [h, w], "counts": buf.raw[:n.value].decode("utf-8")}


def remove_small_regions(masks, area_thresh, mode):
    lib = _lib.load()
    n, H, W = masks.shape
    out = torch.empty_like(masks)
    changed = torch.empty((n,), dtype=torch.uint8, device=masks.device)
    need = lib.hgl_remove_small_regions_workspace_bytes(n, H, W)
    ws = ops.workspace(need, masks.device, "sam_ccl")
    check(lib.hgl_remove_small_regions(ops._dev(masks, torch.uint8, "masks"), n, H, W, int(area_thresh),
                                       1 if mode == "holes" else 0, out.data_ptr(), changed.data_ptr(),
                                       ws.data_ptr(), ws.numel(), ops._stream()), "hgl_remove_small_regions")
    return out, changed


def remove_small_regions_boxes(masks, area_thresh, mode):
    lib = _lib.load()
    n, H, W = masks.shape
    out = torch.empty_like(masks)
    changed = torch.empty((n,), dtype=torch.uint8, device=masks.device)
    boxes = torch.empty((n, 4), dtype=torch.int32, device=masks.device)
    need = lib.hgl_remove_small_regions_workspace_bytes(n, H, W)
    ws = ops.workspace(need, masks.device, "sam_ccl")
    check(lib.hgl_remove_small_regions_boxes(ops._dev(masks, torch.uint8, "masks"), n, H, W, int(area_thresh),
                                             1 if mode == "holes" else 0, out.data_ptr(), changed.data_ptr(), boxes.data_ptr(),
                                             ws.data_ptr(), ws.numel(), ops._stream()), "hgl_remove_small_regions_boxes")
    return out, changed, boxes


def mask_boxes(masks):
    lib = _lib.load()
    n, H, W = masks.shape
    boxes = torch.empty((n, 4), dtype=torch.int32, device=masks.device)
    check(lib.hgl_mask_boxes(ops._dev(masks, torch.uint8, "masks"), n, H, W, boxes.data_ptr(), ops._stream()),
          "hgl_mask_boxes")
    return boxes
```

### include/hybridgl.h

```cpp
#ifndef HYBRIDGL_H
#define HYBRIDGL_H

#include <stddef.h>
#include <stdint.h>

#ifdef __cplusplus
extern "C" {
#endif

#define HGL_OK 0
#define HGL_EINVAL (-1)
#define HGL_ENODEVICE (-2)
#define HGL_EWORKSPACE (-3)
#define HGL_ELAUNCH (-4)

#define HGL_ABI_VERSION 7

#define HGL_ACT_NONE 0
#define HGL_ACT_QUICKGELU 1
#define HGL_ACT_GELU 2
#define HGL_ACT_RELU 3

#define HGL_FUSION_G2L 0
#define HGL_FUSION_L2G 1
// ... 228 lines not shown
  HglNormW up1;
  const float *up3_w, *up3_b;
  HglLinearW hyper[4][3];
  HglLinearW iou_head[3];
  const float *kvq1_w, *kvq1_b, *kvq1_pe;
  const float *kvf_w, *kvf_b, *kvf_pe;
  const float *point_embed_neg, *point_embed_box0, *point_embed_box1;
  const float *md_c1_w, *md_c1_b, *md_n1_w, *md_n1_b, *md_c2_w, *md_c2_b, *md_n2_w, *md_n2_b, *md_c3_w, *md_c3_b;
} HglSamDecoderW;

size_t hgl_resize_pil_bilinear_workspace_bytes(int H, int out_w, int C);
int hgl_resize_pil_bilinear(const uint8_t* img, int H, int W, int C, int out_h, int out_w, const int32_t* kx,
                            const int32_t* bx, int ksize_x, const int32_t* ky, const int32_t* by, int ksize_y,
                            uint8_t* out, void* workspace, size_t workspace_bytes, void* stream);

int hgl_u8_to_chw_lut(const uint8_t* img, int H, int W, int C, const float* lut, float* out, void* stream);

size_t hgl_sam_encode_workspace_bytes(const HglSamEncoderW* w);
int hgl_sam_encode(const HglSamEncoderW* w, const uint8_t* resized_img, int in_h, int in_w, float* emb,
                   void* workspace, size_t workspace_bytes, void* stream);

size_t hgl_sam_encode_batch_workspace_bytes(const HglSamEncoderW* w, int nb);
int hgl_sam_encode_batch(const HglSamEncoderW* w, const uint8_t* const* resized_imgs, const int* in_h, const int* in_w,
                         int nb, float* emb, void* workspace, size_t workspace_bytes, void* stream);

int hgl_sam_dense_pe(const HglSamDecoderW* w, const float* grid_coords01, float* dense_pe, void* stream);

size_t hgl_sam_decode_workspace_bytes(const HglSamDecoderW* w, int P);
int hgl_sam_decode_points(const HglSamDecoderW* w, const float* emb, const float* points01, int P,
                          float* low_res, float* iou_pred, void* workspace, size_t workspace_bytes,
                          void* stream);
int hgl_sam_decode_points_gated(const HglSamDecoderW* w, const float* emb, const float* points01, int P, float iou_gate,
                                float* low_res, float* iou_pred, void* workspace, size_t workspace_bytes, void* stream);
int hgl_sam_decode_prompts(const HglSamDecoderW* w, const float* emb, const float* coords01, const int32_t* labels, int n_sparse,
                           const float* dense, int first_mask, int P, float* low_res, float* iou_pred, void* workspace,
                           size_t workspace_bytes, void* stream);
int hgl_sam_embed_masks(const HglSamDecoderW* w, const float* mask_input, int P, float* dense, void* stream);

int hgl_sam_decoder_fusion(int mask);

int hgl_attention_presplit(int on);
int hgl_attention_presplit_f32(const float* qkv, int ld, int B, int H, int S, int hd, float* out, int ldo, float scale,
                               int mask_kind, const uint8_t* keep, int keep_b0, int keep_n, void* scratch,
                               size_t scratch_bytes, void* stream);

size_t hgl_sam_postprocess_workspace_bytes(int K);
int hgl_sam_postprocess(const float* low_res, const float* iou_pred, int K, int hl, int wl, int img_size,
                        int in_h, int in_w, int H, int W, float mask_threshold, float stability_offset,
                        float pred_iou_thresh, float stability_thresh, uint8_t* masks, int32_t* boxes_xyxy,
                        float* stability, uint8_t* keep, float* full_logits, void* workspace,
                        size_t workspace_bytes, void* stream);

int hgl_nms(const int32_t* boxes_xyxy, const float* scores, const uint8_t* keep, int K, float iou_threshold,
            int32_t* out_idx, int32_t* out_n, void* stream);

size_t hgl_remove_small_regions_workspace_bytes(int N, int H, int W);
int hgl_remove_small_regions(const uint8_t* masks, int N, int H, int W, int area_thresh, int holes,
                             uint8_t* out, uint8_t* changed, void* workspace, size_t workspace_bytes,
                             void* stream);
int hgl_remove_small_regions_boxes(const uint8_t* masks, int N, int H, int W, int area_thresh, int holes,
                                   uint8_t* out, uint8_t* changed, int32_t* boxes_xyxy, void* workspace,
                                   size_t workspace_bytes, void* stream);
size_t hgl_nms_large_workspace_bytes(int K);
int hgl_nms_large(const int32_t* boxes_xyxy, const float* scores, const uint8_t* keep, int K, float iou_threshold,
                  int32_t* out_idx, int32_t* out_n, void* workspace, size_t workspace_bytes, void* stream);
int hgl_box_near_crop_edge(const int32_t* boxes_xyxy, int K, const int32_t* crop_box_xyxy, const int32_t* orig_box_xyxy,
                           float atol, uint8_t* keep, void* stream);
int hgl_mask_boxes(const uint8_t* masks, int N, int H, int W, int32_t* boxes_xyxy, void* stream);

int hgl_gather_masks(const uint8_t* masks, const int32_t* idx, const int32_t* n, int max_n, long long HW,
                     uint8_t* out, void* stream);

int hgl_gt_mask_from_polygons(const double* xy, const int32_t* n_points, int n_polys, int H, int W, uint8_t* mask,
                              int64_t* area);
int hgl_gt_mask_from_rle_counts(const uint32_t* counts, int m, int H, int W, uint8_t* mask, int64_t* area);
int hgl_gt_mask_from_rle_string(const char* s, int H, int W, uint8_t* mask, int64_t* area);
int hgl_rle_encode_mask(const uint8_t* mask, int H, int W, uint32_t* counts, long long cap, long long* m);
int hgl_rle_to_string(const uint32_t* counts, long long m, char* out, size_t cap, size_t* len);

#ifdef __cplusplus
}
#endif
#endif
```

Before: 33.30.

## Batch SAM mask decoding and NMS across multiple images per launch

Result: faster. 34.14, median of 6 (+2.5%).

```diff
diff --git a/hybridgl_amd/_lib.py b/hybridgl_amd/_lib.py
--- a/hybridgl_amd/_lib.py
+++ b/hybridgl_amd/_lib.py
@@ -160,6 +160,9 @@
     "hgl_sam_decode_workspace_bytes": (_SZ, [C.POINTER(HglSamDecoderW), _I]),
     "hgl_sam_decode_points": (_I, [C.POINTER(HglSamDecoderW), _VP, _VP, _I, _VP, _VP, _VP, _SZ, _VP]),
     "hgl_sam_decode_points_gated": (_I, [C.POINTER(HglSamDecoderW), _VP, _VP, _I, C.c_float, _VP, _VP, _VP, _SZ, _VP]),
+    "hgl_sam_decode_multi_workspace_bytes": (_SZ, [C.POINTER(HglSamDecoderW), _I, _I]),
+    "hgl_sam_decode_points_multi": (_I, [C.POINTER(HglSamDecoderW), _VP, _VP, _I, _I, _VP, _VP, _VP, _SZ, _VP]),
+    "hgl_sam_decode_points_multi_gated": (_I, [C.POINTER(HglSamDecoderW), _VP, _VP, _I, _I, C.c_float, _VP, _VP, _VP, _SZ, _VP]),
     "hgl_sam_decode_prompts": (_I, [C.POINTER(HglSamDecoderW), _VP, _VP, _VP, _I, _VP, _I, _I, _VP, _VP, _VP, _SZ, _VP]),
     "hgl_sam_embed_masks": (_I, [C.POINTER(HglSamDecoderW), _VP, _I, _VP, _VP]),
     "hgl_sam_decoder_fusion": (_I, [_I]),
@@ -169,6 +172,7 @@
     "hgl_sam_postprocess": (_I, [_VP, _VP, _I, _I, _I, _I, _I, _I, _I, _I, _F, _F, _F, _F, _VP, _VP, _VP, _VP, _VP,
                                  _VP, _SZ, _VP]),
     "hgl_nms": (_I, [_VP, _VP, _VP, _I, _F, _VP, _VP, _VP]),
+    "hgl_nms_segments": (_I, [_VP, _VP, _VP, _VP, _I, _I, _F, _VP, _VP, _VP]),
     "hgl_nms_large_workspace_bytes": (_SZ, [_I]),
     "hgl_nms_large": (_I, [_VP, _VP, _VP, _I, _F, _VP, _VP, _VP, _SZ, _VP]),
     "hgl_box_near_crop_edge": (_I, [_VP, _I, C.POINTER(C.c_int32), C.POINTER(C.c_int32), _F, _VP, _VP]),
diff --git a/hybridgl_amd/csrc/attention.hip b/hybridgl_amd/csrc/attention.hip
--- a/hybridgl_amd/csrc/attention.hip
+++ b/hybridgl_amd/csrc/attention.hip
@@ -1326,6 +1326,7 @@
   int B, H, Sq, Sk, ldq, ldk, ldv, ldo;
   long long sqb, skb, svb, sob;
   float scale;
+  int kvdiv;
 };
 
 constexpr int FEWQ_MAX = 8;
@@ -1456,8 +1457,8 @@
     o[qi][0] = f32x4{0.f, 0.f, 0.f, 0.f};
     o[qi][1] = f32x4{0.f, 0.f, 0.f, 0.f};
   }
-  const float* kp = a.k + b * a.skb + hh * 16 + c2 * 8;
-  const float* vp = a.v + b * a.svb + hh * 16 + c2 * 8;
+  const float* kp = a.k + (b / a.kvdiv) * a.skb + hh * 16 + c2 * 8;
+  const float* vp = a.v + (b / a.kvdiv) * a.svb + hh * 16 + c2 * 8;
   const float* qs = q_s + hh * FQC_QS + c2 * 8;
   const int k0 = chunk * FQC_KEYS + ks;
   f32x4 kn[2], vn[2];
@@ -1672,6 +1673,7 @@
   HGL_REQUIRE(hd == 16 && Sq >= 1 && Sq <= FEWQ_MAX, "attention_fewq: unsupported shape (hd %d, Sq %d)", hd, Sq);
   HGL_REQUIRE(((ldk | ldv) & 3) == 0 && ((skb | svb) & 3) == 0, "attention_fewq: K/V strides must be multiples of 4");
   FewQArgs a;
+  a.kvdiv = 1;
   a.q = q; a.k = k; a.v = v; a.out = out; a.B = B; a.H = H; a.Sq = Sq; a.Sk = Sk;
   a.ldq = ldq; a.ldk = ldk; a.ldv = ldv; a.ldo = ldo; a.sqb = sqb; a.skb = skb; a.svb = svb; a.sob = sob; a.scale = scale;
   HglProfScope prof(HGL_PROF_ATTN, 4.0 * B * (double)H * Sq * Sk * hd, 0.0, st);
@@ -1685,14 +1687,16 @@
 
 int hgl_launch_attention_fewq_chunked(const float* q, const float* k, const float* v, float* out, int B, int H, int Sq, int Sk,
                                       int hd, int ldq, int ldk, int ldv, int ldo, long long sqb, long long skb, long long svb,
-                                      long long sob, float scale, float* part, size_t part_bytes, hipStream_t st) {
+                                      long long sob, float scale, float* part, size_t part_bytes, hipStream_t st, int kv_group) {
   HGL_REQUIRE(q && k && v && out && part, "attention_fewq_chunked: null operand");
+  HGL_REQUIRE(kv_group >= 1 && B % kv_group == 0, "attention_fewq_chunked: %d batches in groups of %d", B, kv_group);
   HGL_REQUIRE(hd == 16 && H == 8 && Sq >= 1 && Sq <= 7 && Sk >= 1 && B >= 1 && B <= 65535,
               "attention_fewq_chunked: unsupported shape (hd %d, H %d, Sq %d)", hd, H, Sq);
   HGL_REQUIRE(((ldk | ldv) & 3) == 0 && ((skb | svb) & 3) == 0 && (((uintptr_t)k | (uintptr_t)v) & 15) == 0,
               "attention_fewq_chunked: K/V strides must be multiples of 4");
   HGL_REQUIRE(part_bytes >= hgl_attention_fewq_part_bytes(B, Sk), "attention_fewq_chunked: partial buffer too small");
   FewQArgs a;
+  a.kvdiv = kv_group;
   a.q = q; a.k = k; a.v = v; a.out = out; a.B = B; a.H = H; a.Sq = Sq; a.Sk = Sk;
   a.ldq = ldq; a.ldk = ldk; a.ldv = ldv; a.ldo = ldo; a.sqb = sqb; a.skb = skb; a.svb = svb; a.sob = sob; a.scale = scale;
   const int nchunk = (Sk + FQC_KEYS - 1) / FQC_KEYS;
diff --git a/hybridgl_amd/csrc/hgl_common.h b/hybridgl_amd/csrc/hgl_common.h
--- a/hybridgl_amd/csrc/hgl_common.h
+++ b/hybridgl_amd/csrc/hgl_common.h
@@ -148,7 +148,8 @@
 size_t hgl_attention_fewq_part_bytes(int B, int Sk);
 int hgl_launch_attention_fewq_chunked(const float* q, const float* k, const float* v, float* out, int B, int H, int Sq, int Sk,
                                       int hd, int ldq, int ldk, int ldv, int ldo, long long sqb, long long skb, long long svb,
-                                      long long sob, float scale, float* part, size_t part_bytes, hipStream_t st);
+                                      long long sob, float scale, float* part, size_t part_bytes, hipStream_t st,
+                                      int kv_group = 1);
 int hgl_launch_attention(const float* q, const float* k, const float* v, float* out, int B, int H,
                          int Sq, int Sk, int hd, int ldq, int ldk, int ldv, int ldo, long long sqb,
                          long long skb, long long svb, long long sob, float scale, int mask_kind,
@@ -244,7 +245,8 @@
                         float eps, float* low_res, const uint8_t* skip, hipStream_t st);
 int hgl_launch_dec_i2t(const float* q, int ldq, long long q_bstride, const float* k1, const float* v1, const float* out_w,
                        const float* out_b, const float* R, long long r_bstride, const float* ln_w, const float* ln_b, float eps,
-                       float scale, int P, int HW, float* out32, void* out_hi, void* out_lo, hipStream_t st);
+                       float scale, int P, int HW, float* out32, void* out_hi, void* out_lo, hipStream_t st,
+                       int per_set = 1);
 
 int hgl_precision();
 bool hgl_split_layout();
diff --git a/hybridgl_amd/csrc/sam_api.hip b/hybridgl_amd/csrc/sam_api.hip
--- a/hybridgl_amd/csrc/sam_api.hip
+++ b/hybridgl_amd/csrc/sam_api.hip
@@ -229,7 +229,7 @@
   uint8_t* skip;
 };
 
-bool carve_dec(HglArena& ar, const HglSamDecoderW* w, int P, DecPlan& p) {
+bool carve_dec(HglArena& ar, const HglSamDecoderW* w, int P, DecPlan& p, int n_img = 1) {
   const size_t C = w->C, HW = (size_t)w->grid * w->grid, T = 16;
   p.sparse = ar.take<float>((size_t)P * (T - 5) * C);
   p.tokens = ar.take<float>(P * T * C);
@@ -239,8 +239,8 @@
   p.k1 = ar.take<float>(P * T * C);
   p.v1 = ar.take<float>(P * T * C);
   p.att = ar.take<float>(P * T * C);
-  p.keys0 = ar.take<float>(HW * C);
-  p.kpe0 = ar.take<float>(HW * C);
+  p.keys0 = ar.take<float>(n_img * HW * C);
+  p.kpe0 = ar.take<float>(n_img * HW * C);
   p.keys = ar.take<float>(P * HW * C);
   p.kpe = ar.take<float>(P * HW * C);
   p.kp = ar.take<float>(3 * (P * HW * C / 2));
@@ -285,6 +285,15 @@
   return hgl_launch_gemm(A, l.w, l.b, R, Cc, M, N, K, lda, K, ldr, ldc, 1, 0, 0, 0, 0, act, st);
 }
 
+inline int lin_sets(const float* A, int lda, const HglLinearW& l, float* Cc, int ldc, int M, int n, int N, int K, hipStream_t st) {
+  if (n == 1) return lin(A, lda, l, nullptr, 0, Cc, ldc, M, N, K, HGL_ACT_NONE, st);
+  if (hgl_gemm_skinny_applicable(l.w, M, N, K, lda, K, 1, 8192))
+    return hgl_launch_gemm_x3_skinny(A, lda, l.w, l.b, nullptr, 0, Cc, ldc, n * M, N, K, HGL_ACT_NONE, st);
+  for (int i = 0; i < n; ++i)
+    HGL_TRY(lin(A + (size_t)i * M * lda, lda, l, nullptr, 0, Cc + (size_t)i * M * ldc, ldc, M, N, K, HGL_ACT_NONE, st));
+  return HGL_OK;
+}
+
 int g_dec_fusion = -1;
 int dec_fusion_mask() {
   if (g_dec_fusion < 0) g_dec_fusion = HGL_DIAG_SWITCH("HGL_SAM_DEC_FUSED", 0x7fffffff);
@@ -293,31 +302,40 @@
 
 int dec_fewq(const float* q, const float* k, const float* v, float* att, int B, int heads, int Nq, int Nk, int hd, int ldq,
              int ldk, int ldv, int ldo, long long sqb, long long skb, long long svb, long long sob, float* scratch,
-             size_t scratch_bytes, hipStream_t st) {
+             size_t scratch_bytes, hipStream_t st, int kv_group = 1) {
   const float scale = 1.0f / sqrtf((float)hd);
   if ((dec_fusion_mask() & 16) && scratch && heads == 8 && hd == 16 && Nk >= 256 && B <= 65535 &&
       scratch_bytes >= hgl_attention_fewq_part_bytes(B, Nk)) {
     for (int q0 = 0; q0 < Nq; q0 += 7)
       HGL_TRY(hgl_launch_attention_fewq_chunked(q + (long long)q0 * ldq, k, v, att + (long long)q0 * ldo, B, heads,
                                                 Nq - q0 < 7 ? Nq - q0 : 7, Nk, hd, ldq, ldk, ldv, ldo, sqb, skb, svb, sob, scale,
-                                                scratch, scratch_bytes, st));
+                                                scratch, scratch_bytes, st, kv_group));
     return HGL_OK;
   }
+  HGL_REQUIRE(kv_group == 1, "sam_decode: keys shared by groups of %d prompts need the chunked attention", kv_group);
   return hgl_launch_attention(q, k, v, att, B, heads, Nq, Nk, hd, ldq, ldk, ldv, ldo, sqb, skb, svb, sob, scale, HGL_MASK_NONE,
                               nullptr, 0, 0, nullptr, nullptr, 0, 0, st);
 }
 
 int dec_attn(const HglSamDecoderW* w, const HglSamAttnW& a, const float* q, bool q_shared, int Nq, const float* k,
              const float* v, bool kv_shared, int Nk, int B, float* qp, float* kp, float* vp, float* att,
-             const float* R, long long sR, float* out, hipStream_t st, float* scratch = nullptr, size_t scratch_bytes = 0) {
+             const float* R, long long sR, float* out, hipStream_t st, float* scratch = nullptr, size_t scratch_bytes = 0,
+             int kv_sets = 1) {
   const int C = w->C, I = a.internal, heads = w->heads, hd = I / heads;
   const int Bq = q_shared ? 1 : B, Bk = kv_shared ? 1 : B;
   HGL_TRY(lin(q, C, a.q, nullptr, 0, qp, I, Bq * Nq, I, C, HGL_ACT_NONE, st));
-  HGL_TRY(lin(k, C, a.k, nullptr, 0, kp, I, Bk * Nk, I, C, HGL_ACT_NONE, st));
-  HGL_TRY(lin(v, C, a.v, nullptr, 0, vp, I, Bk * Nk, I, C, HGL_ACT_NONE, st));
-  HGL_TRY(dec_fewq(qp, kp, vp, att, B, heads, Nq, Nk, hd, I, I, I, I, q_shared ? 0 : (long long)Nq * I,
-                   kv_shared ? 0 : (long long)Nk * I, kv_shared ? 0 : (long long)Nk * I, (long long)Nq * I, scratch,
-                   scratch_bytes, st));
+  if (kv_shared && kv_sets > 1) {
+    HGL_TRY(lin_sets(k, C, a.k, kp, I, Nk, kv_sets, I, C, st));
+    HGL_TRY(lin_sets(v, C, a.v, vp, I, Nk, kv_sets, I, C, st));
+    HGL_TRY(dec_fewq(qp, kp, vp, att, B, heads, Nq, Nk, hd, I, I, I, I, (long long)Nq * I, (long long)Nk * I, (long long)Nk * I,
+                     (long long)Nq * I, scratch, scratch_bytes, st, B / kv_sets));
+  } else {
+    HGL_TRY(lin(k, C, a.k, nullptr, 0, kp, I, Bk * Nk, I, C, HGL_ACT_NONE, st));
+    HGL_TRY(lin(v, C, a.v, nullptr, 0, vp, I, Bk * Nk, I, C, HGL_ACT_NONE, st));
+    HGL_TRY(dec_fewq(qp, kp, vp, att, B, heads, Nq, Nk, hd, I, I, I, I, q_shared ? 0 : (long long)Nq * I,
+                     kv_shared ? 0 : (long long)Nk * I, kv_shared ? 0 : (long long)Nk * I, (long long)Nq * I, scratch,
+                     scratch_bytes, st));
+  }
   if (!R || sR == (long long)Nq * C)
     return lin(att, I, a.out, R, C, out, C, B * Nq, C, I, HGL_ACT_NONE, st);
   return hgl_launch_gemm(att, a.out.w, a.out.b, R, out, Nq, C, I, I, I, C, C, B, (long long)Nq * I, 0, sR,
@@ -389,8 +407,8 @@
   return lin(att, I, a.out, queries, C, queries, C, P * T, C, I, HGL_ACT_NONE, st);
 }
 
-int dec_t2i_raw(const HglSamDecoderW* w, const HglSamAttnW& a, const float* qpe, const SplitPair& keysS, int P, int HW, int T,
-                float* q1, float* small, float* bias, float* att, float* queries, hipStream_t st) {
+int dec_t2i_raw(const HglSamDecoderW* w, const HglSamAttnW& a, const float* qpe, const SplitPair& keysS, int P, int ppi, int HW,
+                int T, float* q1, float* small, float* bias, float* att, float* queries, hipStream_t st) {
   const int C = w->C, I = a.internal, heads = w->heads, hd = I / heads;
   HGL_TRY(lin(qpe, C, a.q, nullptr, 0, q1, I, P * T, I, C, HGL_ACT_NONE, st));
   uint16_t* Qh = (uint16_t*)small;
@@ -400,7 +418,7 @@
   HGL_TRY(hgl_launch_split_f16(A, 1.0f, Qh, Ql, (long long)P * 56 * C, st));
   HGL_TRY(hgl_launch_gemm_f16x3(Qh, Ql, C, w->dense_pe, nullptr, nullptr, 0, bias, nullptr, nullptr, HW, P * 56, HW, C,
                                 HGL_ACT_NONE, st));
-  const int ns = hgl_t2i_key_ranges(P, HW);
+  const int ns = hgl_t2i_key_ranges(ppi, HW);
   float* const rows = ns > 1 ? A + (size_t)P * 56 * C : A;
   HGL_TRY(hgl_launch_t2i_raw_attn(Qh, Ql, bias, keysS.hi, keysS.lo, P, HW, rows, ns, st));
   HGL_TRY(hgl_launch_t2i_unfold_v(rows, ns, a.v.w, a.v.b, att, P, st));
@@ -535,7 +553,7 @@
 static int decode_impl(const HglSamDecoderW* w, const float* emb, const float* points01, const float* coords01,
                        const int32_t* labels, int n_sparse, const float* dense, int first_mask, int P, float* low_res,
                        float* iou_pred, void* workspace, size_t workspace_bytes, void* stream, bool gated = false,
-                       float iou_gate = 0.f) {
+                       float iou_gate = 0.f, int n_img = 1) {
   const HglSplitTermsScope three_terms(3);
   HGL_TRY(hgl_require_device());
   HGL_REQUIRE(valid_dec(w) && w->dense_pe, "sam_decode: invalid weight struct (dense_pe missing?)");
@@ -543,9 +561,11 @@
   HGL_REQUIRE(first_mask == 0 || first_mask == 1, "sam_decode: first_mask must be 0 or 1");
   HGL_REQUIRE(n_sparse >= 2 && n_sparse <= 11, "sam_decode: %d sparse tokens per prompt (2 .. 11 supported)", n_sparse);
   HGL_REQUIRE(n_sparse <= 3 || (long long)P * w->heads <= 65535, "sam_decode: %d prompts of more than 3 sparse tokens in one call", P);
+  HGL_REQUIRE(n_img >= 1 && P % n_img == 0 && (n_img == 1 || (points01 && !dense)), "sam_decode: %d prompts for %d images", P, n_img);
+  const int ppi = P / n_img;
   HglArena ar(workspace, workspace_bytes);
   DecPlan p;
-  if (!workspace || !carve_dec(ar, w, P, p)) {
+  if (!workspace || !carve_dec(ar, w, P, p, n_img)) {
     hgl_set_error("sam_decode: workspace too small (%zu bytes given)", workspace_bytes);
     return HGL_EWORKSPACE;
   }
@@ -567,8 +587,8 @@
     HGL_TRY(hgl_launch_add_rows_bcast(dense, sK, emb, sK, P, p.keys, st));
     HGL_TRY(hgl_launch_add_rows_bcast(p.keys, sK, w->dense_pe, sK, P, p.kpe, st));
   } else {
-    HGL_TRY(hgl_launch_add_rows_bcast(emb, C, w->no_mask, C, HW, p.keys0, st));
-    HGL_TRY(hgl_launch_add_rows_bcast(p.keys0, 0, w->dense_pe, (long long)HW * C, 1, p.kpe0, st));
+    HGL_TRY(hgl_launch_add_rows_bcast(emb, C, w->no_mask, C, n_img * HW, p.keys0, st));
+    HGL_TRY(hgl_launch_add_rows_bcast(p.keys0, n_img > 1 ? sK : 0, w->dense_pe, (long long)HW * C, n_img, p.kpe0, st));
   }
   (void)hipMemcpyAsync(p.queries, p.tokens, sizeof(float) * P * sQ, hipMemcpyDeviceToDevice, st);
 
@@ -579,7 +599,7 @@
   const SplitPair keysS = split_view(p.keysS, (size_t)P * HW * C), kpeS = split_view(p.kpe, (size_t)P * HW * C);
   const bool raw_t2i = merged && (dec_fusion_mask() & 32) && (dec_fusion_mask() & 4) && T == 7 && I1 == 128 && w->heads == 8 &&
                        C == 256 && HW % 128 == 0 && P <= 65535 && !perprompt && hgl_has_split_weight(w->dense_pe) &&
-                       (size_t)P * (56 * C * 8) + hgl_t2i_part_bytes(P, HW) <= atti_bytes &&
+                       (size_t)P * (56 * C * 8) + n_img * hgl_t2i_part_bytes(ppi, HW) <= atti_bytes &&
                        (size_t)P * (56 * C * 4 + 16384 * 4 + 256) <= atti_bytes;
   for (int li = 0; li < 2; ++li) {
     const auto& L = w->layer[li];
@@ -599,7 +619,7 @@
     HGL_TRY(hgl_launch_layernorm(p.queries, L.n1.w, L.n1.b, p.queries, P * T, C, 1e-5f, st));
     HGL_TRY(hgl_launch_add_rows_bcast(p.queries, P * sQ, p.tokens, P * sQ, 1, p.qpe, st));
     if (raw_t2i && !shared && !plain0) {
-      HGL_TRY(dec_t2i_raw(w, L.t2i, p.qpe, keysS, P, HW, T, p.q1, p.atti, p.kp, p.att, p.queries, st));
+      HGL_TRY(dec_t2i_raw(w, L.t2i, p.qpe, keysS, P, ppi, HW, T, p.q1, p.atti, p.kp, p.att, p.queries, st));
     } else if (merged && !shared && !plain0) {
       HGL_TRY(dec_project_merged(keysS, w->kvq1_w, w->kvq1_b, w->kvq1_pe, P, HW, C, 3 * I1, p.kp, st));
       HGL_TRY(dec_t2i_merged(w, L.t2i, p.qpe, p.kp, 3 * I1, P, HW, T, p.q1, p.att, p.queries, p.atti, atti_bytes, st));
@@ -607,7 +627,7 @@
       HGL_TRY(dec_t2i_x3(w, L.t2i, p.qpe, kpeS, keysS, P, HW, T, p.q1, p.kp, p.vp, p.att, p.queries, p.atti, atti_bytes, st));
     } else {
       HGL_TRY(dec_attn(w, L.t2i, p.qpe, false, T, kpe, keys, shared, HW, P, p.q1, p.kp, p.vp, p.att, p.queries, sQ,
-                       p.queries, st, p.atti, atti_bytes));
+                       p.queries, st, p.atti, atti_bytes, shared ? n_img : 1));
     }
     HGL_TRY(hgl_launch_layernorm(p.queries, L.n2.w, L.n2.b, p.queries, P * T, C, 1e-5f, st));
     HGL_TRY(lin(p.queries, C, L.lin1, nullptr, 0, p.mlp, w->mlp_dim, P * T, w->mlp_dim, C, HGL_ACT_RELU, st));
@@ -633,11 +653,16 @@
     } else if (fuse_i2t) {
       HGL_TRY(lin(p.qpe, C, L.i2t.k, nullptr, 0, p.k1, I1, P * T, I1, C, HGL_ACT_NONE, st));
       HGL_TRY(lin(p.queries, C, L.i2t.v, nullptr, 0, p.v1, I1, P * T, I1, C, HGL_ACT_NONE, st));
-      if (shared) HGL_TRY(lin(p.kpe0, C, L.i2t.q, nullptr, 0, p.qi, I1, HW, I1, C, HGL_ACT_NONE, st));
-      HGL_TRY(hgl_launch_dec_i2t(shared ? p.qi : p.kp + 2 * I1, shared ? I1 : 3 * I1, shared ? 0 : (long long)HW * 3 * I1, p.k1,
-                                 p.v1, L.i2t.out.w, L.i2t.out.b, keys, shared ? 0 : sK, L.n4.w, L.n4.b, 1e-5f,
+      if (shared) HGL_TRY(lin_sets(p.kpe0, C, L.i2t.q, p.qi, I1, HW, n_img, I1, C, st));
+      const bool sets = shared && n_img > 1;
+      HGL_TRY(hgl_launch_dec_i2t(shared ? p.qi : p.kp + 2 * I1, shared ? I1 : 3 * I1,
+                                 sets ? (long long)HW * I1 : shared ? 0 : (long long)HW * 3 * I1, p.k1,
+                                 p.v1, L.i2t.out.w, L.i2t.out.b, keys, sets ? sK : shared ? 0 : sK, L.n4.w, L.n4.b, 1e-5f,
                                  1.0f / sqrtf((float)(I1 / w->heads)), P, HW, (li == 0 && !raw_t2i) ? p.keys : nullptr, keysS.hi,
-                                 keysS.lo, st));
+                                 keysS.lo, st, sets ? ppi : 1));
+    } else if (shared && n_img > 1) {
+      hgl_set_error("sam_decode: several images in one launch need the fused image -> token step");
+      return HGL_EINVAL;
     } else if (x3 && plain0) {
       HGL_TRY(dec_attn(w, L.i2t, kpe, false, HW, p.qpe, p.queries, false, T, P, p.qi, p.k1, p.v1, p.atti, keys, sK, p.keys, st));
       HGL_TRY(hgl_launch_ln256_pe_split(p.keys, L.n4.w, L.n4.b, w->dense_pe, HW, (long long)P * HW, 1e-5f, 1, keysS.hi, keysS.lo,
@@ -660,7 +685,7 @@
   }
   HGL_TRY(hgl_launch_add_rows_bcast(p.queries, P * sQ, p.tokens, P * sQ, 1, p.qpe, st));
   if (raw_t2i) {
-    HGL_TRY(dec_t2i_raw(w, w->final_t2i, p.qpe, keysS, P, HW, T, p.q1, p.atti, p.kp, p.att, p.queries, st));
+    HGL_TRY(dec_t2i_raw(w, w->final_t2i, p.qpe, keysS, P, ppi, HW, T, p.q1, p.atti, p.kp, p.att, p.queries, st));
   } else if (merged) {
     HGL_TRY(dec_project_merged(keysS, w->kvf_w, w->kvf_b, w->kvf_pe, P, HW, C, 2 * I1, p.kp, st));
     HGL_TRY(dec_t2i_merged(w, w->final_t2i, p.qpe, p.kp, 2 * I1, P, HW, T, p.q1, p.att, p.queries, p.atti, atti_bytes, st));
@@ -679,6 +704,7 @@
   const uint8_t* skip = nullptr;
   if (gated) {
     hipLaunchKernelGGL(iou_gate_kernel, dim3((P + 255) / 256), dim3(256), 0, st, (const float*)iou_pred, P, iou_gate, p.skip);
+    HGL_TRY(hgl_check_launch("iou_gate"));
     skip = p.skip;
   }
 
@@ -727,6 +753,63 @@
                      iou_gate);
 }
 
+static bool dec_multi_fused(const HglSamDecoderW* w, int n_img, int ppi) {
+  const int C = w->C, HW = w->grid * w->grid, I1 = w->layer[1].t2i.internal, heads = w->heads;
+  const long long P = (long long)n_img * ppi;
+  const auto& L0 = w->layer[0];
+  const bool merged = dec_x3_ready(w) && dec_merged_ready(w) && I1 == w->layer[1].i2t.internal && I1 == w->final_t2i.internal &&
+                      2 * w->final_t2i.internal == C;
+  const bool fuse_i2t = merged && (dec_fusion_mask() & 4) && L0.i2t.internal == I1 && I1 == 128 && heads == 8 && HW % 64 == 0;
+  const size_t atti_bytes = (size_t)P * HW * (C / 2) * sizeof(float);
+  const bool chunked = (dec_fusion_mask() & 16) && heads == 8 && L0.t2i.internal == 128 && HW >= 256 &&
+                       atti_bytes >= hgl_attention_fewq_part_bytes((int)P, HW);
+  return P <= 65535 && fuse_i2t && chunked;
+}
+
+static int dec_multi_images(int n_img, int ppi) {
+  const int per = ppi >= 1024 ? 1 : 1024 / ppi;
+  return per < n_img ? per : n_img;
+}
+
+static int decode_multi(const HglSamDecoderW* w, const float* emb, const float* points01, int n_img, int ppi, float* low_res,
+                        float* iou_pred, void* workspace, size_t workspace_bytes, void* stream, bool gated, float iou_gate) {
+  HGL_REQUIRE(points01, "sam_decode: null input");
+  HGL_REQUIRE(valid_dec(w) && w->dense_pe, "sam_decode: invalid weight struct (dense_pe missing?)");
+  HGL_REQUIRE(n_img >= 1 && ppi >= 1 && (long long)n_img * ppi <= 65535, "sam_decode_multi: %d images x %d prompts", n_img, ppi);
+  if (n_img == 1)
+    return decode_impl(w, emb, points01, nullptr, nullptr, 2, nullptr, 1, ppi, low_res, iou_pred, workspace, workspace_bytes, stream,
+                       gated, iou_gate);
+  const int per = dec_multi_fused(w, dec_multi_images(n_img, ppi), ppi) ? dec_multi_images(n_img, ppi) : 1;
+  const size_t HW = (size_t)w->grid * w->grid, lowsz = (size_t)3 * 16 * HW;
+  for (int i = 0; i < n_img; i += per) {
+    const int k = n_img - i < per ? n_img - i : per;
+    HGL_TRY(decode_impl(w, emb + i * HW * w->C, points01 + (size_t)i * ppi * 2, nullptr, nullptr, 2, nullptr, 1, k * ppi,
+                        low_res + (size_t)i * ppi * lowsz, iou_pred + (size_t)i * ppi * 3, workspace, workspace_bytes, stream, gated,
+                        iou_gate, k));
+  }
+  return HGL_OK;
+}
+
+size_t hgl_sam_decode_multi_workspace_bytes(const HglSamDecoderW* w, int n_img, int ppi) {
+  if (!valid_dec(w) || n_img <= 0 || ppi <= 0 || (long long)n_img * ppi > 65535) return 0;
+  const int per = n_img > 1 && dec_multi_fused(w, dec_multi_images(n_img, ppi), ppi) ? dec_multi_images(n_img, ppi) : 1;
+  HglArena ar(nullptr, 0);
+  DecPlan p;
+  carve_dec(ar, w, per * ppi, p, per);
+  return ar.off;
+}
+
+int hgl_sam_decode_points_multi(const HglSamDecoderW* w, const float* emb, const float* points01, int n_img, int ppi,
+                                float* low_res, float* iou_pred, void* workspace, size_t workspace_bytes, void* stream) {
+  return decode_multi(w, emb, points01, n_img, ppi, low_res, iou_pred, workspace, workspace_bytes, stream, false, 0.f);
+}
+
+int hgl_sam_decode_points_multi_gated(const HglSamDecoderW* w, const float* emb, const float* points01, int n_img, int ppi,
+                                      float iou_gate, float* low_res, float* iou_pred, void* workspace, size_t workspace_bytes,
+                                      void* stream) {
+  return decode_multi(w, emb, points01, n_img, ppi, low_res, iou_pred, workspace, workspace_bytes, stream, true, iou_gate);
+}
+
 int hgl_sam_decode_prompts(const HglSamDecoderW* w, const float* emb, const float* coords01, const int32_t* labels, int n_sparse,
                            const float* dense, int first_mask, int P, float* low_res, float* iou_pred, void* workspace,
                            size_t workspace_bytes, void* stream) {
diff --git a/hybridgl_amd/csrc/sam_decoder_fused.hip b/hybridgl_amd/csrc/sam_decoder_fused.hip
--- a/hybridgl_amd/csrc/sam_decoder_fused.hip
+++ b/hybridgl_amd/csrc/sam_decoder_fused.hip
@@ -289,6 +289,7 @@
 struct I2TArgs {
   const float* q;
   long long sqb;
+  int pdiv;
   int ldq;
   const float *k1, *v1;
   const _Float16 *Wh, *Wl;
@@ -337,7 +338,7 @@
   const int hh = t & 7, arow = t >> 3;
   f32x4 qv[4];
   {
-    const float* qp = a.q + p * a.sqb + (long long)(n0 + arow) * a.ldq + hh * 16;
+    const float* qp = a.q + (p / a.pdiv) * a.sqb + (long long)(n0 + arow) * a.ldq + hh * 16;
 #pragma unroll
     for (int c = 0; c < 4; ++c) qv[c] = *(const f32x4*)(qp + 4 * c);
   }
@@ -438,7 +439,7 @@
     lw[j] = *(const f32x4*)(a.ln_w + colw + 16 * j);
     lb[j] = *(const f32x4*)(a.ln_b + colw + 16 * j);
   }
-  const float* Rp = a.R + p * a.srb + (long long)n0 * 256 + colw;
+  const float* Rp = a.R + (p / a.pdiv) * a.srb + (long long)n0 * 256 + colw;
 #pragma unroll
   for (int i = 0; i < 4; ++i)
 #pragma unroll
@@ -544,7 +545,7 @@
 
 int hgl_launch_dec_i2t(const float* q, int ldq, long long q_bstride, const float* k1, const float* v1, const float* out_w,
                        const float* out_b, const float* R, long long r_bstride, const float* ln_w, const float* ln_b, float eps,
-                       float scale, int P, int HW, float* out32, void* out_hi, void* out_lo, hipStream_t st) {
+                       float scale, int P, int HW, float* out32, void* out_hi, void* out_lo, hipStream_t st, int per_set) {
   const void *wh, *wl;
   int s = 0, n = 0, k = 0;
   HGL_REQUIRE(hgl_get_split_weight(out_w, &wh, &wl, &s, &n, &k), "dec_i2t: the out-projection weight has no registered fp16 split");
@@ -552,7 +553,9 @@
   HGL_REQUIRE(q && k1 && v1 && R && out_hi && out_lo, "dec_i2t: null operand");
   HGL_REQUIRE(HW % I2T_ROWS == 0 && P > 0 && P <= 65535 && (ldq & 3) == 0 && (q_bstride & 3) == 0 && (r_bstride & 3) == 0,
               "dec_i2t: %d tokens / %d prompts / strides unsupported", HW, P);
+  HGL_REQUIRE(per_set >= 1 && P % per_set == 0, "dec_i2t: %d prompts in sets of %d", P, per_set);
   I2TArgs a;
+  a.pdiv = per_set;
   a.q = q; a.sqb = q_bstride; a.ldq = ldq; a.k1 = k1; a.v1 = v1;
   a.Wh = (const _Float16*)wh; a.Wl = (const _Float16*)wl; a.bo = out_b; a.R = R; a.srb = r_bstride;
   a.ln_w = ln_w; a.ln_b = ln_b; a.so = ldexpf(1.0f, -s); a.eps = eps; a.scale = scale;
diff --git a/hybridgl_amd/csrc/sam_glue.hip b/hybridgl_amd/csrc/sam_glue.hip
--- a/hybridgl_amd/csrc/sam_glue.hip
+++ b/hybridgl_amd/csrc/sam_glue.hip
@@ -988,10 +988,9 @@
   return sj > si || (sj == si && j < i);
 }
 
-__global__ __launch_bounds__(1024) void nms_kernel(const int* __restrict__ boxes,
-                                                   const float* __restrict__ scores,
-                                                   const uint8_t* __restrict__ keep, int K, float thr,
-                                                   int* __restrict__ out_idx, int* __restrict__ out_n) {
+__device__ __forceinline__ void nms_body(const int* __restrict__ boxes, const float* __restrict__ scores,
+                                         const uint8_t* __restrict__ keep, int K, float thr,
+                                         int* __restrict__ out_idx, int* __restrict__ out_n) {
   __shared__ int order[1024];
   __shared__ unsigned char alive[1024];
   __shared__ int cur, nkept;
@@ -1037,6 +1036,13 @@
   if (t == 0) *out_n = nkept;
 }
 
+__global__ __launch_bounds__(1024) void nms_kernel(const int* __restrict__ boxes,
+                                                   const float* __restrict__ scores,
+                                                   const uint8_t* __restrict__ keep, int K, float thr,
+                                                   int* __restrict__ out_idx, int* __restrict__ out_n) {
+  nms_body(boxes, scores, keep, K, thr, out_idx, out_n);
+}
+
 __global__ __launch_bounds__(256) void nms_rank_kernel(const float* __restrict__ scores, const uint8_t* __restrict__ keep,
                                                        int K, int* __restrict__ order, int* __restrict__ nvalid) {
   const int i = blockIdx.x * 256 + threadIdx.x;
@@ -1062,9 +1068,9 @@
   return iou > thr;
 }
 
-__global__ __launch_bounds__(512) void nms_bits_kernel(const int* __restrict__ boxes, const float* __restrict__ scores,
-                                                       const uint8_t* __restrict__ keep, int K, float thr,
-                                                       int* __restrict__ out_idx, int* __restrict__ out_n) {
+__device__ __forceinline__ void nms_bits_body(const int* __restrict__ boxes, const float* __restrict__ scores,
+                                              const uint8_t* __restrict__ keep, int K, float thr,
+                                              int* __restrict__ out_idx, int* __restrict__ out_n) {
   __shared__ int4 sbox[512];
   __shared__ int order[512];
   __shared__ float ssc[512];
@@ -1143,6 +1149,31 @@
     __syncthreads();
   }
   if (t == 0) *out_n = nkept_s;
+}
+
+__global__ __launch_bounds__(512) void nms_bits_kernel(const int* __restrict__ boxes, const float* __restrict__ scores,
+                                                       const uint8_t* __restrict__ keep, int K, float thr,
+                                                       int* __restrict__ out_idx, int* __restrict__ out_n) {
+  nms_bits_body(boxes, scores, keep, K, thr, out_idx, out_n);
+}
+
+template <bool BITS>
+__global__ __launch_bounds__(BITS ? 512 : 1024) void nms_segments_kernel(const int* __restrict__ boxes,
+                                                                         const float* __restrict__ scores,
+                                                                         const uint8_t* __restrict__ keep,
+                                                                         const int* __restrict__ offsets, float thr,
+                                                                         int* __restrict__ out_idx, int* __restrict__ out_n) {
+  const int s = blockIdx.x, o = offsets[s], K = offsets[s + 1] - o;
+  if (K <= 0 || K > 512) {
+    if (BITS && threadIdx.x == 0) out_n[s] = 0;
+    if (BITS || K <= 0 || K > 1024) return;
+  } else if (!BITS) {
+    return;
+  }
+  if (BITS)
+    nms_bits_body(boxes + 4ll * o, scores + o, keep + o, K, thr, out_idx + o, out_n + s);
+  else
+    nms_body(boxes + 4ll * o, scores + o, keep + o, K, thr, out_idx + o, out_n + s);
 }
 
 __global__ __launch_bounds__(64) void nms_mask_kernel(const int* __restrict__ boxes, const int* __restrict__ order,
@@ -1469,6 +1500,22 @@
   return hgl_check_launch("nms");
 }
 
+int hgl_nms_segments(const int32_t* boxes_xyxy, const float* scores, const uint8_t* keep, const int32_t* offsets, int n_seg,
+                     int max_len, float iou_threshold, int32_t* out_idx, int32_t* out_n, void* stream) {
+  HGL_TRY(hgl_require_device());
+  HGL_REQUIRE(boxes_xyxy && scores && keep && offsets && out_idx && out_n, "nms_segments: null argument");
+  HGL_REQUIRE(n_seg > 0 && n_seg <= 65535, "nms_segments: n_seg must be in [1,65535] (got %d)", n_seg);
+  HGL_REQUIRE(max_len >= 0 && max_len <= 1024, "nms_segments: segments hold up to 1024 candidates (max_len %d)", max_len);
+  HGL_REQUIRE(((uintptr_t)boxes_xyxy & 15) == 0, "nms_segments: boxes must be 16-byte aligned");
+  hipStream_t st = (hipStream_t)stream;
+  hipLaunchKernelGGL(nms_segments_kernel<true>, dim3(n_seg), dim3(512), 0, st, (const int*)boxes_xyxy, scores, keep,
+                     (const int*)offsets, iou_threshold, (int*)out_idx, (int*)out_n);
+  if (max_len > 512)
+    hipLaunchKernelGGL(nms_segments_kernel<false>, dim3(n_seg), dim3(1024), 0, st, (const int*)boxes_xyxy, scores, keep,
+                       (const int*)offsets, iou_threshold, (int*)out_idx, (int*)out_n);
+  return hgl_check_launch("nms_segments");
+}
+
 size_t hgl_nms_large_workspace_bytes(int K) {
   const size_t W = ((size_t)K + 63) / 64;
   return hgl_align_up((size_t)K * sizeof(int), 256) + hgl_align_up(sizeof(int), 256) + hgl_align_up((size_t)K * W * 8, 256);
diff --git a/hybridgl_amd/sam.py b/hybridgl_amd/sam.py
--- a/hybridgl_amd/sam.py
+++ b/hybridgl_amd/sam.py
@@ -235,6 +235,31 @@
               "hgl_sam_decode_points")
         return low, iou
 
+    def decode_points_multi(self, emb, points01, n_img, iou_gate=None):
+        lib = _lib.load()
+        ops.use_precision(self.precision)
+        P = int(points01.shape[0])
+        n_img = int(n_img)
+        if n_img < 1 or P % n_img or tuple(emb.shape[:1]) != (n_img,):
+            raise ValueError(f"{P} prompts / embeddings {tuple(emb.shape)} for {n_img} images")
+        ppi = P // n_img
+        need = lib.hgl_sam_decode_multi_workspace_bytes(C.byref(self.dec_w), n_img, ppi)
+        ws = ops.workspace(need, self.device, "sam_decode")
+        g4 = 4 * self.grid
+        low = torch.empty((P, 3, g4, g4), dtype=torch.float32, device=self.device)
+        iou = torch.empty((P, 3), dtype=torch.float32, device=self.device)
+        if iou_gate is not None:
+            check(lib.hgl_sam_decode_points_multi_gated(C.byref(self.dec_w), ops._dev(emb, torch.float32, "emb"),
+                                                        ops._dev(points01, torch.float32, "points01"), n_img, ppi, float(iou_gate),
+                                                        low.data_ptr(), iou.data_ptr(), ws.data_ptr(), ws.numel(), ops._stream()),
+                  "hgl_sam_decode_points_multi_gated")
+            return low, iou
+        check(lib.hgl_sam_decode_points_multi(C.byref(self.dec_w), ops._dev(emb, torch.float32, "emb"),
+                                              ops._dev(points01, torch.float32, "points01"), n_img, ppi, low.data_ptr(),
+                                              iou.data_ptr(), ws.data_ptr(), ws.numel(), ops._stream()),
+              "hgl_sam_decode_points_multi")
+        return low, iou
+
     def decode_prompts(self, emb, coords01, labels, first_mask=1, dense=None):
         lib = _lib.load()
         ops.use_precision(self.precision)
@@ -300,6 +325,17 @@
         check(lib.hgl_nms_large(ops._dev(boxes_xyxy, torch.int32, "boxes"), ops._dev(scores, torch.float32, "scores"),
                                 ops._dev(keep, torch.uint8, "keep"), K, float(iou_threshold), idx.data_ptr(),
                                 n.data_ptr(), ws.data_ptr(), ws.numel(), ops._stream()), "hgl_nms_large")
+    return idx, n
+
+
+def nms_segments(boxes_xyxy, scores, keep, offsets, max_len, iou_threshold):
+    lib = _lib.load()
+    K, n_seg = boxes_xyxy.shape[0], offsets.shape[0] - 1
+    idx = torch.empty((K,), dtype=torch.int32, device=boxes_xyxy.device)
+    n = torch.empty((n_seg,), dtype=torch.int32, device=boxes_xyxy.device)
+    check(lib.hgl_nms_segments(ops._dev(boxes_xyxy, torch.int32, "boxes"), ops._dev(scores, torch.float32, "scores"),
+                               ops._dev(keep, torch.uint8, "keep"), ops._dev(offsets, torch.int32, "offsets"), n_seg, int(max_len),
+                               float(iou_threshold), idx.data_ptr(), n.data_ptr(), ops._stream()), "hgl_nms_segments")
     return idx, n
 
 
@@ -588,19 +624,55 @@
         return self._propose_from_embedding(emb, H, W, nh, nw, layer_idx, crop_box, orig_size)
 
     def propose_batch(self, images, encoded_event=None):
+        out = [None] * len(images)
+        pts_of = {}
+        for idxs, (masks, boxes, iou, stab, order, cnt), k3, (H, W) in self._propose_classes(images, encoded_event):
+            pts = pts_of.get((H, W))
+            if pts is None:
+                pts = pts_of[(H, W)] = np.repeat(self.point_grids[0] * np.array([[W, H]], dtype=np.float64), 3, axis=0)
+            for j, i in enumerate(idxs):
+                sl = slice(j * k3, (j + 1) * k3)
+                out[i] = (masks[sl], boxes[sl], iou[sl], stab[sl], order[sl], cnt[j:j + 1], pts)
+        return out
+
+    def _propose_classes(self, images, encoded_event=None):
         m = self.model
         sizes, resized = [], []
         for image in images:
             H, W = image.shape[:2]
             dev_img = image if isinstance(image, torch.Tensor) else torch.from_numpy(np.ascontiguousarray(image)).to(m.device)
-            sizes.append((H, W) + get_preprocess_shape(H, W, m.img_size))
+            sizes.append((int(H), int(W)) + get_preprocess_shape(H, W, m.img_size))
             resized.append(resize_longest_side(dev_img.contiguous(), m.img_size))
         emb = m.encode_batch(resized)
         if encoded_event is not None:
             encoded_event.record(torch.cuda.current_stream(m.device))
-        return [self._propose_from_embedding(emb[i], *sizes[i], 0, None, None) for i in range(len(images))]
-
-    def _propose_from_embedding(self, emb, H, W, nh, nw, layer_idx, crop_box, orig_size):
+        npts = len(self.point_grids[0])
+        k3 = 3 * npts
+        classes = {}
+        for i, sz in enumerate(sizes):
+            classes.setdefault(sz, []).append(i)
+        out = []
+        for (H, W, nh, nw), idxs in classes.items():
+            n_max = min(max(1, (2 ** 31 - 1) // (k3 * H * W)), 65535 // k3) if k3 <= 1024 and npts <= self.points_per_batch else 1
+            for c0 in range(0, len(idxs), n_max):
+                part = idxs[c0:c0 + n_max]
+                if len(part) == 1:
+                    c = self._propose_from_embedding(emb[part[0]], H, W, nh, nw, 0, None, None)
+                    out.append((part, c[:6], k3, (H, W)))
+                else:
+                    out.append((part, self._propose_class(emb, part, H, W, nh, nw), k3, (H, W)))
+        return out
+
+    def _dev_const(self, key, make):
+        cache = self.__dict__.setdefault("_const_cache", {})
+        t = cache.get(key)
+        if t is None:
+            if len(cache) >= 256:
+                cache.clear()
+            t = cache[key] = make()
+        return t
+
+    def _prompt_grid(self, H, W, nh, nw, layer_idx):
         m = self.model
         pts = self.point_grids[layer_idx] * np.array([[W, H]], dtype=np.float64)
         tp = pts.copy()
@@ -613,6 +685,32 @@
             if len(cache) >= 64:
                 cache.clear()
             p01 = cache[key] = torch.from_numpy(((tp + 0.5) / float(m.img_size)).astype(np.float32)).to(m.device)
+        return pts, p01
+
+    def _propose_class(self, emb, idxs, H, W, nh, nw):
+        m = self.model
+        dev = m.device
+        n = len(idxs)
+        pts, p01 = self._prompt_grid(H, W, nh, nw, 0)
+        npts = len(pts)
+        k3 = 3 * npts
+        if idxs == list(range(idxs[0], idxs[0] + n)):
+            e = emb[idxs[0]:idxs[0] + n]
+        else:
+            e = emb.index_select(0, self._dev_const(("rows",) + tuple(idxs), lambda: torch.tensor(idxs, dtype=torch.int64, device=dev)))
+        gate = float(self.pred_iou_thresh) if self.pred_iou_thresh > 0 and getattr(self, "iou_gate", True) else None
+        pk = self._dev_const(("p01", H, W, n), lambda: p01.repeat(n, 1).contiguous())
+        low, iou = m.decode_points_multi(e, pk, n, iou_gate=gate)
+        low, iou = low.flatten(0, 1), iou.flatten()
+        masks, boxes, stab, keep, _ = m.postprocess(low, iou, (nh, nw), (H, W), self.pred_iou_thresh,
+                                                    self.stability_score_thresh, self.stability_score_offset)
+        offs = self._dev_const(("offs", n, k3), lambda: torch.arange(0, (n + 1) * k3, k3, dtype=torch.int32, device=dev))
+        order, cnt = nms_segments(boxes, iou, keep, offs, k3, self.box_nms_thresh)
+        return masks, boxes, iou, stab, order, cnt
+
+    def _propose_from_embedding(self, emb, H, W, nh, nw, layer_idx, crop_box, orig_size):
+        m = self.model
+        pts, p01 = self._prompt_grid(H, W, nh, nw, layer_idx)
         lows, ious = [], []
         gate = float(self.pred_iou_thresh) if self.pred_iou_thresh > 0 and getattr(self, "iou_gate", True) else None
         for s in range(0, len(pts), self.points_per_batch):
@@ -857,9 +955,17 @@
         st = _GroupState()
         st.cap = cap
         st.sizes = [tuple(int(v) for v in im.shape[:2]) for im in images]
-        st.cand = self.propose_batch(images, encoded_event)
+        st.cand = self._propose_classes(images, encoded_event)
         dev = self.model.device
-        st.n1_dev = torch.cat([c[5] for c in st.cand])
+        cnts = [c[1][5] for c in st.cand]
+        st.n1_dev = cnts[0] if len(cnts) == 1 else torch.cat(cnts)
+        perm = [i for c in st.cand for i in c[0]]
+        if perm != list(range(len(images))):
+            inv = [0] * len(perm)
+            for pos, i in enumerate(perm):
+                inv[i] = pos
+            st.n1_dev = st.n1_dev.index_select(0, self._dev_const(("rows",) + tuple(inv),
+                                                                  lambda: torch.tensor(inv, dtype=torch.int64, device=dev)))
         st.n1 = torch.empty(len(images), dtype=torch.int32).pin_memory()
         st.n1.copy_(st.n1_dev, non_blocking=True)
         st.overflow = 0
@@ -868,6 +974,20 @@
         st.ev1 = torch.cuda.Event()
         st.ev1.record(torch.cuda.current_stream(dev))
         return st
+
+    def _segment_index(self, counts, stride):
+        total, n = int(sum(counts)), len(counts)
+        host = torch.empty(2 * total + n + 1, dtype=torch.int64, pin_memory=True)
+        h = host.numpy()
+        o = 0
+        h[2 * total] = 0
+        for j, c in enumerate(counts):
+            h[o:o + c] = np.arange(j * stride, j * stride + c)
+            h[total + o:total + o + c] = j * stride
+            o += c
+            h[2 * total + j + 1] = o
+        d = host.to(self.model.device, non_blocking=True)
+        return d[:total], d[total:2 * total], d[2 * total:].to(torch.int32)
 
     def group_cleanup(self, st):
         st.ev1.synchronize()
@@ -880,57 +1000,93 @@
         st.n1_list = n1
         st.stage = []
         n2_dev = []
-        for (masks, boxes, iou, stab, order, _n, _pts), n in zip(st.cand, n1):
-            if n == 0:
+        area = self.min_mask_region_area
+        for idxs, (masks, boxes, iou, stab, order, _cnt), k3, _hw in st.cand:
+            counts = [n1[i] for i in idxs]
+            total = sum(counts)
+            if total == 0:
                 st.stage.append(None)
-                n2_dev.append(torch.zeros(1, dtype=torch.int32, device=dev))
+                if area > 0:
+                    n2_dev.append(torch.zeros(len(idxs), dtype=torch.int32, device=dev))
                 continue
-            idx = order[:n].long()
-            m = masks.index_select(0, idx)
-            bx = boxes.index_select(0, idx)
-            if self.min_mask_region_area > 0:
-                m1, c1 = remove_small_regions(m, self.min_mask_region_area, "holes")
-                m2, c2, nb = remove_small_regions_boxes(m1, self.min_mask_region_area, "islands")
+            pos, base, offs = self._segment_index(counts, k3)
+            idx = order.index_select(0, pos).long()
+            gidx = idx + base
+            m = masks.index_select(0, gidx)
+            bx = boxes.index_select(0, gidx)
+            if area > 0:
+                m1, c1 = torch.empty_like(m), torch.empty((total,), dtype=torch.uint8, device=dev)
+                m2, c2 = torch.empty_like(m), torch.empty((total,), dtype=torch.uint8, device=dev)
+                nb = torch.empty((total, 4), dtype=torch.int32, device=dev)
+                o = 0
+                for c in counts:
+                    if c > 0:
+                        sl = slice(o, o + c)
+                        remove_small_regions(m[sl], area, "holes", out=(m1[sl], c1[sl]))
+                        remove_small_regions_boxes(m1[sl], area, "islands", out=(m2[sl], c2[sl], nb[sl]))
+                    o += c
                 unchanged = ((c1 | c2) == 0).to(torch.float32)
-                order2, n2 = nms(nb, unchanged, torch.ones(n, dtype=torch.uint8, device=dev),
-                                 max(self.box_nms_thresh, self.crop_nms_thresh))
-                st.stage.append((m2, nb, idx, order2, iou, stab))
+                order2, n2 = nms_segments(nb, unchanged, torch.ones(total, dtype=torch.uint8, device=dev), offs, max(counts),
+                                          max(self.box_nms_thresh, self.crop_nms_thresh))
+                st.stage.append((m2, nb, idx, gidx, order2, iou, stab, counts))
                 n2_dev.append(n2)
             else:
-                st.stage.append((m, bx, idx, None, iou, stab))
-                n2_dev.append(torch.full((1,), n, dtype=torch.int32, device=dev))
-        st.cand = None
+                st.stage.append((m, bx, idx, gidx, None, iou, stab, counts))
         st.n2 = None
-        if self.min_mask_region_area > 0:
+        if area > 0:
             st.n2 = torch.empty(len(n1), dtype=torch.int32).pin_memory()
-            st.n2.copy_(torch.cat(n2_dev), non_blocking=True)
+            st.n2.copy_(n2_dev[0] if len(n2_dev) == 1 else torch.cat(n2_dev), non_blocking=True)
             st.ev2 = torch.cuda.Event()
             st.ev2.record(torch.cuda.current_stream(dev))
+        st.cand = [c[0] for c in st.cand]
         return st
 
     def group_finish(self, st):
+        n2_all = None
         if st.n2 is not None:
             st.ev2.synchronize()
-            n2 = [int(v) for v in st.n2.tolist()]
-        else:
-            n2 = list(st.n1_list)
-        out = []
+            n2_all = [int(v) for v in st.n2.tolist()]
+        out = [None] * len(st.sizes)
         dev = self.model.device
-        for stg, n, hw in zip(st.stage, n2, st.sizes):
-            if stg is None or n == 0:
-                e = torch.empty
-                out.append((e((0,) + hw, dtype=torch.uint8, device=dev), e((0, 4), dtype=torch.int64, device=dev),
-                            e((0,), device=dev), e((0,), device=dev), e((0,), dtype=torch.int64, device=dev)))
-                continue
-            m, bx, idx, order2, iou, stab = stg
-            if order2 is not None:
-                k = order2[:n].long()
-                m, bx, idx = m.index_select(0, k), bx.index_select(0, k), idx.index_select(0, k)
-            b = bx.long()
-            xywh = torch.stack([b[:, 0], b[:, 1], b[:, 2] - b[:, 0], b[:, 3] - b[:, 1]], 1)
-            out.append((m, xywh, iou.index_select(0, idx), stab.index_select(0, idx), idx))
+        e = torch.empty
+        k0 = 0
+        for idxs, stg in zip(st.cand, st.stage):
+            n2 = n2_all[k0:k0 + len(idxs)] if n2_all is not None else [st.n1_list[i] for i in idxs]
+            k0 += len(idxs)
+            if stg is not None and sum(n2) > 0:
+                m, bx, idx, gidx, order2, iou, stab, counts = stg
+                if order2 is not None:
+                    pos, base, _ = self._packed_index(n2, counts)
+                    k = order2.index_select(0, pos).long() + base
+                    m, bx, idx, gidx = m.index_select(0, k), bx.index_select(0, k), idx.index_select(0, k), gidx.index_select(0, k)
+                b = bx.long()
+                xywh = torch.stack([b[:, 0], b[:, 1], b[:, 2] - b[:, 0], b[:, 3] - b[:, 1]], 1)
+                iou, stab = iou.index_select(0, gidx), stab.index_select(0, gidx)
+            o = 0
+            for i, n in zip(idxs, n2):
+                if stg is None or n == 0:
+                    hw = st.sizes[i]
+                    out[i] = (e((0,) + hw, dtype=torch.uint8, device=dev), e((0, 4), dtype=torch.int64, device=dev),
+                              e((0,), device=dev), e((0,), device=dev), e((0,), dtype=torch.int64, device=dev))
+                    continue
+                sl = slice(o, o + n)
+                out[i] = (m[sl], xywh[sl], iou[sl], stab[sl], idx[sl])
+                o += n
         st.stage = None
         return out
+
+    def _packed_index(self, counts, seg_lens):
+        total = int(sum(counts))
+        host = torch.empty(2 * total, dtype=torch.int64, pin_memory=True)
+        h = host.numpy()
+        o = s0 = 0
+        for c, ln in zip(counts, seg_lens):
+            h[o:o + c] = np.arange(s0, s0 + c)
+            h[total + o:total + o + c] = s0
+            o += c
+            s0 += ln
+        d = host.to(self.model.device, non_blocking=True)
+        return d[:total], d[total:], None
 
     def generate_group(self, images, cap=None):
         return self.group_finish(self.group_cleanup(self.group_begin(images, cap)))
@@ -1011,11 +1167,15 @@
     return {"size": [h, w], "counts": buf.raw[:n.value].decode("utf-8")}
 
 
-def remove_small_regions(masks, area_thresh, mode):
+def remove_small_regions(masks, area_thresh, mode, out=None):
     lib = _lib.load()
     n, H, W = masks.shape
-    out = torch.empty_like(masks)
-    changed = torch.empty((n,), dtype=torch.uint8, device=masks.device)
+    if out is not None:
+        out, changed = out
+        ops._dev(out, torch.uint8, "out"), ops._dev(changed, torch.uint8, "changed")
+    else:
+        out = torch.empty_like(masks)
+        changed = torch.empty((n,), dtype=torch.uint8, device=masks.device)
     need = lib.hgl_remove_small_regions_workspace_bytes(n, H, W)
     ws = ops.workspace(need, masks.device, "sam_ccl")
     check(lib.hgl_remove_small_regions(ops._dev(masks, torch.uint8, "masks"), n, H, W, int(area_thresh),
@@ -1024,12 +1184,16 @@
     return out, changed
 
 
-def remove_small_regions_boxes(masks, area_thresh, mode):
+def remove_small_regions_boxes(masks, area_thresh, mode, out=None):
     lib = _lib.load()
     n, H, W = masks.shape
-    out = torch.empty_like(masks)
-    changed = torch.empty((n,), dtype=torch.uint8, device=masks.device)
-    boxes = torch.empty((n, 4), dtype=torch.int32, device=masks.device)
+    if out is not None:
+        out, changed, boxes = out
+        ops._dev(out, torch.uint8, "out"), ops._dev(changed, torch.uint8, "changed"), ops._dev(boxes, torch.int32, "boxes")
+    else:
+        out = torch.empty_like(masks)
+        changed = torch.empty((n,), dtype=torch.uint8, device=masks.device)
+        boxes = torch.empty((n, 4), dtype=torch.int32, device=masks.device)
     need = lib.hgl_remove_small_regions_workspace_bytes(n, H, W)
     ws = ops.workspace(need, masks.device, "sam_ccl")
     check(lib.hgl_remove_small_regions_boxes(ops._dev(masks, torch.uint8, "masks"), n, H, W, int(area_thresh),
diff --git a/include/hybridgl.h b/include/hybridgl.h
--- a/include/hybridgl.h
+++ b/include/hybridgl.h
@@ -284,6 +284,12 @@
                           void* stream);
 int hgl_sam_decode_points_gated(const HglSamDecoderW* w, const float* emb, const float* points01, int P, float iou_gate,
                                 float* low_res, float* iou_pred, void* workspace, size_t workspace_bytes, void* stream);
+size_t hgl_sam_decode_multi_workspace_bytes(const HglSamDecoderW* w, int n_img, int ppi);
+int hgl_sam_decode_points_multi(const HglSamDecoderW* w, const float* emb, const float* points01, int n_img, int ppi,
+                                float* low_res, float* iou_pred, void* workspace, size_t workspace_bytes, void* stream);
+int hgl_sam_decode_points_multi_gated(const HglSamDecoderW* w, const float* emb, const float* points01, int n_img, int ppi,
+                                      float iou_gate, float* low_res, float* iou_pred, void* workspace, size_t workspace_bytes,
+                                      void* stream);
 int hgl_sam_decode_prompts(const HglSamDecoderW* w, const float* emb, const float* coords01, const int32_t* labels, int n_sparse,
                            const float* dense, int first_mask, int P, float* low_res, float* iou_pred, void* workspace,
                            size_t workspace_bytes, void* stream);
@@ -305,6 +311,9 @@
 
 int hgl_nms(const int32_t* boxes_xyxy, const float* scores, const uint8_t* keep, int K, float iou_threshold,
             int32_t* out_idx, int32_t* out_n, void* stream);
+
+int hgl_nms_segments(const int32_t* boxes_xyxy, const float* scores, const uint8_t* keep, const int32_t* offsets, int n_seg,
+                     int max_len, float iou_threshold, int32_t* out_idx, int32_t* out_n, void* stream);
 
 size_t hgl_remove_small_regions_workspace_bytes(int N, int H, int W);
 int hgl_remove_small_regions(const uint8_t* masks, int N, int H, int W, int area_thresh, int holes,
```
